# Visual-Behavior/aloception-oss

Hardware: AMD Instinct MI355X
Metric: frames/sec (whole node) DeformableDETR-R50 inference (higher is better)
Workload: dtype bf16; 1 GPU; DeformableDETR-R50 inference bf16, batch 8 synthetic 1333x800 frames per GPU, random-init weights; launch=hip-graph replay + eager inference(), per_gpu_batch=8, global_batch=8, parallelism=batch-sharded x1, no collective

## Files before the change

__graft_entry__.py:

```python
import os
import subprocess
import sys

ROOT = os.path.dirname(os.path.abspath(__file__))
PKG = os.path.join(ROOT, "aloception-oss_amd")
for p in (PKG, os.path.join(ROOT, "oracle")):
    if p not in sys.path:
        sys.path.insert(0, p)


def build():
    if os.path.exists("/opt/rocm/bin/hipcc"):
        subprocess.check_call(["make", "-C", os.path.join(PKG, "csrc"), "-j4"])
    subprocess.check_call(["make", "-C", os.path.join(ROOT, "oracle")])
    import alo_hip

    alo_hip.lib()
    alo_hip.two_stage_lib()
    from alonet.deformable_detr.ops.functions import load_MultiScaleDeformableAttention
    from alonet.raft.corr import CorrBlock

    load_MultiScaleDeformableAttention()


def smoke():
    import numpy as np
    import torch

    import alo_hip
    import oracle as O
    from alonet.deformable_detr.ops.functions import MSDeformAttnFunction
    from alonet.raft.corr import CorrBlock

    assert torch.cuda.is_available(), "smoke() needs a GPU"
    dev = "cuda:0"
    rng = np.random.default_rng(0)
    shapes = np.array([(12, 17), (6, 9), (3, 5), (2, 3)], np.int32)
    start = np.concatenate([[0], np.cumsum(shapes[:, 0] * shapes[:, 1])[:-1]]).astype(np.int32)
    N, M, D, Lq, L, P = 2, 8, 32, 40, 4, 4
    S = int((shapes[:, 0] * shapes[:, 1]).sum())
    value = rng.standard_normal((N, S, M, D)).astype(np.float32)
    loc = rng.uniform(-0.1, 1.1, (N, Lq, M, L, P, 2)).astype(np.float32)
    attn = rng.random((N, Lq, M, L, P)).astype(np.float32)
    attn /= attn.reshape(N, Lq, M, -1).sum(-1)[..., None, None]
    gout = rng.standard_normal((N, Lq, M * D)).astype(np.float32)

    tv = torch.from_numpy(value).to(dev).requires_grad_(True)
    tl = torch.from_numpy(loc).to(dev).requires_grad_(True)
    ta = torch.from_numpy(attn).to(dev).requires_grad_(True)
    out = MSDeformAttnFunction.apply(tv, torch.from_numpy(shapes).to(dev), torch.from_numpy(start).to(dev), tl, ta, 64)
    out.backward(torch.from_numpy(gout).to(dev))
    ref = O.msda_forward(value, shapes, start, loc, attn)
    rgv, rgl, rga = O.msda_backward(value, shapes, start, loc, attn, gout)
    err = {
        "msda_out": float(np.abs(out.detach().cpu().numpy() - ref).max()),
        "msda_grad_value": float(np.abs(tv.grad.cpu().numpy() - rgv).max()),
        "msda_grad_loc": float(np.abs(tl.grad.cpu().numpy() - rgl).max() / max(1.0, np.abs(rgl).max())),
        "msda_grad_attn": float(np.abs(ta.grad.cpu().numpy() - rga).max()),
    }
    refs = np.concatenate([np.stack([(np.tile(np.arange(w), h) + 0.5) / w, (np.repeat(np.arange(h), w) + 0.5) / h], -1) for h, w in shapes])
    eloc = (refs[None, :, None, None, None, :] + rng.uniform(-0.08, 0.08, (N, S, M, L, P, 2))).astype(np.float32)
    eattn = rng.random((N, S, M, L, P)).astype(np.float32)
    eattn /= eattn.reshape(N, S, M, -1).sum(-1)[..., None, None]
    egout = rng.standard_normal((N, S, M * D)).astype(np.float32)
    hint = (__import__("ctypes").c_int32 * 8)(*[int(v) for v in shapes.reshape(-1)])
    assert alo_hip.lib().alo_msda_backward_path(N, S, M, D, L, S, P, alo_hip.ALO_F32, alo_hip.ALO_F32, hint) == 2
    tsh = torch.from_numpy(shapes).to(dev)
    egv, egl, ega = alo_hip.msda_backward(torch.from_numpy(value).to(dev), tsh, torch.from_numpy(start).to(dev), torch.from_numpy(eloc).to(dev),
                                          torch.from_numpy(eattn).to(dev), torch.from_numpy(egout).to(dev))
    wgv, wgl, wga = O.msda_backward(value, shapes, start, eloc, eattn, egout)
    err["msda_wide_grad_value"] = float(np.abs(egv.cpu().numpy() - wgv).max())
    err["msda_wide_grad_loc"] = float(np.abs(egl.cpu().numpy() - wgl).max() / max(1.0, np.abs(wgl).max()))
    err["msda_wide_grad_attn"] = float(np.abs(ega.cpu().numpy() - wga).max())
    f1 = rng.standard_normal((1, 64, 16, 24)).astype(np.float32)
    f2 = rng.standard_normal((1, 64, 16, 24)).astype(np.float32)
    blk = CorrBlock(torch.from_numpy(f1).to(dev), torch.from_numpy(f2).to(dev))
    pyr = O.corr_pyramid(f1, f2)
    err["corr_pyramid"] = max(float(np.abs(blk.corr_pyramid[i].cpu().numpy() - pyr[i]).max()) for i in range(4))
    ys, xs = np.meshgrid(np.arange(16), np.arange(24), indexing="ij")
    coords = (np.stack([xs, ys])[None] + rng.standard_normal((1, 2, 16, 24)) * 2).astype(np.float32)
    got = blk(torch.from_numpy(coords).to(dev)).cpu().numpy()
    err["corr_lookup"] = float(np.abs(got - O.corr_lookup(pyr, coords)).max())
    print("smoke max-abs errors vs oracle:", err)
    assert all(v <= 1e-4 for v in err.values()), err
    assert "libalo_hotpath.so" in open("/proc/self/maps").read()


if __name__ == "__main__":
    build()
    if len(sys.argv) > 1 and sys.argv[1] == "smoke":
        smoke()
```

aloception-oss_amd/alo_hip/__init__.py:

```python
import ctypes
import warnings
import os
import subprocess

import torch

_PKG_ROOT = os.path.dirname(os.path.dirname(os.path.abspath(__file__)))
LIB_PATH = os.path.join(_PKG_ROOT, "libalo_hotpath.so")
CSRC_DIR = os.path.join(_PKG_ROOT, "csrc")

ALO_F32, ALO_F64, ALO_BF16 = 0, 1, 2
RESIDENT_AUTO, RESIDENT_ALWAYS = 0, 1
_DTYPE_CODE = {torch.float32: ALO_F32, torch.float64: ALO_F64, torch.bfloat16: ALO_BF16}

_lib = None
_warned_inference_tensor = False


def tensor_version(t):
    if t.is_inference():
        global _warned_inference_tensor
        if not _warned_inference_tensor:
            _warned_inference_tensor = True
            warnings.warn("alo_hip: a parameter / shape tensor created under torch.inference_mode() carries no version counter, so what is "
                          "derived from it (packed MFMA weights, folded convolutions, the host copy of spatial_shapes) is re-derived on "
                          "every call instead of being cached — results are right, the forward is slower.  Build / load the model outside "
                          "inference_mode() (torch.no_grad() is enough for inference).", RuntimeWarning, stacklevel=3)
        return object()
    return t._version


_DERIVED = "_alo_derived"
_EPOCH = "_alo_cache_epoch"


def derived(owner, name, sources, build, no_grad=True):
    entries = owner.__dict__.setdefault(_DERIVED, {}) if hasattr(owner, "__dict__") else {}
    key = tuple([None if t is None else (tensor_version(t), t.data_ptr(), t.dtype, t.device) for t in sources])
    hit = entries.get(name)
    if hit is None or hit[0] != key:
        with torch.set_grad_enabled(torch.is_grad_enabled() and not no_grad):
            hit = entries[name] = (key, build())
    return hit[1]


class HotpathUnavailable(RuntimeError):
    """libalo_hotpath.so cannot be loaded (not built, or built for another ABI)."""


def build(force=False):
    cmd = ["make", "-C", CSRC_DIR, "-j4"] + (["-B"] if force else [])
    subprocess.check_call(cmd, stdout=subprocess.DEVNULL)
    return LIB_PATH


def _declare(lib):
    c = ctypes
    vp, ip, sz = c.c_void_p, c.c_int, c.c_size_t
    lib.alo_abi_version.restype = ip
    lib.alo_abi_version.argtypes = []
    lib.alo_last_error.restype = c.c_char_p
    lib.alo_last_error.argtypes = []
    lib.alo_msda_forward.restype = ip
    lib.alo_msda_forward.argtypes = [vp] * 6 + [ip] * 9 + [vp]
    lib.alo_msda_forward_fused.restype = ip
    lib.alo_msda_forward_fused.argtypes = [vp] * 7 + [ip] * 9 + [vp]
    lib.alo_msda_backward.restype = ip
    lib.alo_msda_backward.argtypes = [vp] * 9 + [ip] * 9 + [vp]
    lib.alo_msda_backward_hinted.restype = ip
    lib.alo_msda_backward_hinted.argtypes = [vp] * 9 + [ip] * 9 + [c.POINTER(c.c_int32), vp]
    lib.alo_msda_backward_path.restype = ip
    lib.alo_msda_backward_path.argtypes = [ip] * 9 + [c.POINTER(c.c_int32)]
    lib.alo_corr_level_shape.restype = None
    lib.alo_corr_level_shape.argtypes = [ip, ip, ip, c.POINTER(ip), c.POINTER(ip)]
    lib.alo_corr_build_workspace_bytes.restype = sz
    lib.alo_corr_build_workspace_bytes.argtypes = [ip] * 5
    lib.alo_corr_build.restype = ip
    lib.alo_corr_build.argtypes = [vp, vp, c.POINTER(vp), vp, sz] + [ip] * 5 + [vp]
    lib.alo_corr_lookup.restype = ip
    lib.alo_corr_lookup.argtypes = [c.POINTER(vp), vp, vp] + [ip] * 5 + [vp]
    lib.alo_corr_lookup_backward.restype = ip
    lib.alo_corr_lookup_backward.argtypes = [c.POINTER(vp), vp, vp] + [ip] * 5 + [vp]
    lib.alo_corr_lookup_backward_coords.restype = ip
    lib.alo_corr_lookup_backward_coords.argtypes = [c.POINTER(vp), vp, vp, vp] + [ip] * 5 + [vp]
    lib.alo_corr_alt_workspace_bytes.restype = sz
    lib.alo_corr_alt_workspace_bytes.argtypes = [ip] * 5
    lib.alo_corr_alt_prepare.restype = ip
    lib.alo_corr_alt_prepare.argtypes = [vp, c.POINTER(vp), vp, sz] + [ip] * 5 + [vp]
    lib.alo_corr_alt_lookup.restype = ip
    lib.alo_corr_alt_lookup.argtypes = [vp, sz, vp, vp] + [ip] * 6 + [vp]
    lib.alo_msda_forward_fused_hm.restype = ip
    lib.alo_msda_forward_fused_hm_rows.restype = ip
    lib.alo_msda_forward_fused_hm_rows.argtypes = [vp] * 5 + [c.c_long, c.c_long, vp, vp] + [ip] * 9 + [vp]
    lib.alo_msda_forward_fused_hm.argtypes = [vp] * 7 + [ip] * 9 + [vp]
    lib.alo_msda_forward_fused_hm_resident.restype = ip
    lib.alo_msda_forward_fused_hm_resident.argtypes = [vp] * 5 + [c.c_long, c.c_long, vp, vp] + [ip] * 9 + [c.POINTER(c.c_int32), ip, vp]
    lib.alo_msda_resident_levels.restype = ip
    lib.alo_msda_resident_levels.argtypes = [c.POINTER(c.c_int32)] + [ip] * 6
    lib.alo_value_head_major.restype = ip
    lib.alo_value_head_major.argtypes = [vp] * 3 + [ip] * 5 + [vp]
    lib.alo_bias_act_nchw.restype = ip
    lib.alo_bias_act_nchw.argtypes = [vp] * 3 + [ip] * 4 + [vp]
    lib.alo_gru_gate.restype = ip
    lib.alo_gru_gate.argtypes = [vp] * 4 + [ip] * 3 + [c.c_long, c.c_long, vp]
    lib.alo_gru_update.restype = ip
    lib.alo_gru_update.argtypes = [vp] * 5 + [ip] * 3 + [c.c_long, vp]
    lib.alo_pack_mfma_b.restype = ip
    lib.alo_pack_mfma_b.argtypes = [vp, vp, ip, ip, ip, vp]
    lib.alo_value_proj_head_major.restype = ip
    lib.alo_value_proj_head_major.argtypes = [vp] * 5 + [ip] * 5 + [vp]
    lib.alo_conv3x3_nhwc.restype = ip
    lib.alo_conv3x3_nhwc.argtypes = [vp] * 5 + [ip] * 8 + [vp]
    lib.alo_conv3x3_workspace_bytes.restype = c.c_size_t
    lib.alo_conv3x3_workspace_bytes.argtypes = [ip] * 6
    lib.alo_stem_conv_pool.restype = ip
    lib.alo_stem_conv_pool.argtypes = [vp] * 4 + [ip] * 3 + [c.c_long] * 4 + [ip, vp]
    lib.alo_groupnorm_rows_workspace_bytes.restype = c.c_size_t
    lib.alo_groupnorm_rows_workspace_bytes.argtypes = [ip, ip, ip]
    lib.alo_groupnorm_rows.restype = ip
    lib.alo_groupnorm_rows.argtypes = [vp] * 5 + [ip] * 4 + [c.c_float, c.c_long, ip, vp]
    lib.alo_groupnorm_rows_act.restype = ip
    lib.alo_groupnorm_rows_act.argtypes = [vp] * 5 + [ip] * 4 + [c.c_float, c.c_long, ip, ip, vp]
    lib.alo_conv3x3_small_nhwc.restype = ip
    lib.alo_conv3x3_small_nhwc.argtypes = [vp] * 4 + [ip] * 6 + [vp]
    lib.alo_upsample_add_nhwc.restype = ip
    lib.alo_upsample_add_nhwc.argtypes = [vp] * 3 + [ip] * 8 + [vp]
    lib.alo_linear_packed.restype = ip
    lib.alo_linear_packed.argtypes = [vp] * 5 + [c.c_long, ip, ip, ip, ip, vp]
    lib.alo_mask_pyramid.restype = ip
    lib.alo_mask_pyramid.argtypes = [vp, ip, vp, vp, ip, ip, ip, ip, c.POINTER(c.c_int), c.c_uint, vp]
    lib.alo_encoder_reference_points.restype = ip
    lib.alo_encoder_reference_points.argtypes = [vp, vp, ip, ip, c.POINTER(c.c_int), vp]
    lib.alo_conv1x1_nhwc.restype = ip
    lib.alo_conv1x1_nhwc.argtypes = [vp, vp, ip, vp, vp, vp] + [ip] * 8 + [vp]
    lib.alo_panoptic_onehot.restype = ip
    lib.alo_panoptic_onehot.argtypes = [vp, vp] + [ip] * 6 + [c.c_float, vp]
    lib.alo_ffn256.restype = ip
    lib.alo_ffn256.argtypes = [vp] * 6 + [c.c_long, ip, ip, vp]
    lib.alo_linear_shortk.restype = ip
    lib.alo_linear_shortk.argtypes = [vp] * 5 + [c.c_long, ip, ip, ip, ip, vp]
    lib.alo_pos_sine_flat.restype = ip
    lib.alo_pos_sine_flat.argtypes = [vp] * 7 + [ip] * 6 + [c.c_float, c.c_float, ip, vp]
    lib.alo_add_layernorm.restype = ip
    lib.alo_add_layernorm.argtypes = [vp] * 7 + [c.c_long, ip, c.c_float, ip, vp]
    lib.alo_bias_act.restype = ip
    lib.alo_bias_act.argtypes = [vp] * 4 + [c.c_long, ip, ip, ip, vp]


def lib():
    global _lib
    if _lib is None:
        if not os.path.exists(LIB_PATH):
            raise HotpathUnavailable(
                f"{LIB_PATH} is missing: build it with `python -c 'import __graft_entry__ as g; g.build()'` "
                f"or `make -C {CSRC_DIR}` (hipcc, --offload-arch=gfx950). There is no CPU fallback for this path."
            )
        try:
            handle = ctypes.CDLL(LIB_PATH)
        except OSError as e:
            raise HotpathUnavailable(f"cannot load {LIB_PATH}: {e}") from e
        _declare(handle)
        if handle.alo_abi_version() != 2:
            raise HotpathUnavailable(f"{LIB_PATH} has ABI version {handle.alo_abi_version()}, expected 2")
        _lib = handle
    return _lib


def is_available():
    try:
        lib()
        return True
    except HotpathUnavailable:
        return False


def _check(rc):
    if rc != 0:
        raise RuntimeError(lib().alo_last_error().decode() or f"alo_hotpath error {rc}")


def _stream(device):
    return ctypes.c_void_p(torch.cuda.current_stream(device).cuda_stream)


def _ptr(t):
    return ctypes.c_void_p(t.data_ptr())


def _require_cuda_contiguous(named):
    for name, t in named:
        if not t.is_contiguous():
            raise RuntimeError(f"{name} tensor has to be contiguous")
    for name, t in named:
        if not t.is_cuda:
            raise RuntimeError(f"{name} must be a CUDA tensor")


class LaunchTimer:

    def __init__(self, only=None):
        self.records = []
        self.relaunch = {}
        self.only = only

    def __enter__(self):
        global _timer
        self._prev, _timer = _timer, self
        return self

    def __exit__(self, *exc):
        global _timer
        _timer = self._prev

    def replay_ms(self, tag, reps=20):
        fn = self.relaunch[tag]
        fn()
        torch.cuda.synchronize()
        start, stop = torch.cuda.Event(enable_timing=True), torch.cuda.Event(enable_timing=True)
        start.record()
        for _ in range(reps):
            fn()
        stop.record()
        torch.cuda.synchronize()
        return start.elapsed_time(stop) / reps

    def replay_samples(self, tag, reps=7):
        fn = self.relaunch[tag]
        fn()
        torch.cuda.synchronize()
        events = [torch.cuda.Event(enable_timing=True) for _ in range(reps + 1)]
        events[0].record()
        for i in range(reps):
            fn()
            events[i + 1].record()
        torch.cuda.synchronize()
        return [events[i].elapsed_time(events[i + 1]) for i in range(reps)]

    def summary(self):
        torch.cuda.synchronize()
        out = {}
        for tag, start, stop, nbytes, flops in self.records:
            d = out.setdefault(tag, dict(calls=0, ms_total=0.0, alg_bytes_avg=0.0, alg_flops_avg=0.0))
            d["calls"] += 1
            d["ms_total"] += start.elapsed_time(stop)
            d["alg_bytes_avg"] += nbytes
            d["alg_flops_avg"] += flops
        for d in out.values():
            d["ms_avg"] = d["ms_total"] / d["calls"]
            d["alg_bytes_avg"] /= d["calls"]
            d["alg_flops_avg"] /= d["calls"]
        return out


_timer = None


class _timed:
    def __init__(self, tag, nbytes=0.0, flops=0.0, relaunch=None):
        self.tag, self.nbytes, self.flops, self.relaunch = tag, nbytes, flops, relaunch

    def __enter__(self):
        self.on = _timer is not None and (_timer.only is None or self.tag.startswith(_timer.only))
        if self.on:
            self.start = torch.cuda.Event(enable_timing=True)
            self.stop = torch.cuda.Event(enable_timing=True)
            self.start.record()
        return self

    def __exit__(self, *exc):
        if self.on:
            self.stop.record()
            _timer.records.append((self.tag, self.start, self.stop, self.nbytes, self.flops))
            if self.relaunch is not None:
                _timer.relaunch[self.tag] = self.relaunch


def msda_forward_bytes(N, S, M, D, L, Lq, P, elem, loc_elem=4):
    return elem * (N * S * M * D + N * Lq * M * D) + loc_elem * (N * Lq * M * L * P * 3)


def msda_backward_bytes(N, S, M, D, L, Lq, P, elem, loc_elem=4):
    return elem * (2 * N * S * M * D + N * Lq * M * D) + loc_elem * (N * Lq * M * L * P * 3 * 2)


def _msda_prepare(value, spatial_shapes, level_start_index, sampling_loc, attn_weight, im2col_step, extra=()):
    if not value.is_cuda:
        raise RuntimeError("Not implemented on the CPU")
    _require_cuda_contiguous(
        [("value", value), ("spatial_shapes", spatial_shapes), ("level_start_index", level_start_index),
         ("sampling_loc", sampling_loc), ("attn_weight", attn_weight)] + list(extra)
    )
    if value.dim() != 4 or sampling_loc.dim() != 6 or attn_weight.dim() != 5:
        raise RuntimeError("value must be (N,S,M,D), sampling_loc (N,Lq,M,L,P,2), attn_weight (N,Lq,M,L,P)")
    if spatial_shapes.dtype != torch.int32 or level_start_index.dtype != torch.int32:
        raise RuntimeError("spatial_shapes and level_start_index must be int32 tensors")
    N, S, M, D = value.shape
    _, Lq, M2, L, P, two = sampling_loc.shape
    if (M2, two) != (M, 2) or tuple(attn_weight.shape) != (N, Lq, M, L, P) or sampling_loc.shape[0] != N:
        raise RuntimeError("sampling_loc / attn_weight shapes do not match value")
    if tuple(spatial_shapes.shape) != (L, 2) or tuple(level_start_index.shape) != (L,):
        raise RuntimeError("spatial_shapes must be (L,2) and level_start_index (L,)")
    step = min(N, int(im2col_step))
    if step <= 0 or N % step != 0:
        raise RuntimeError(f"batch({N}) must divide im2col_step({step})")
    vdt = _DTYPE_CODE.get(value.dtype)
    if vdt is None:
        raise RuntimeError(f"ms_deform_attn: unsupported value dtype {value.dtype}")
    if value.dtype == torch.bfloat16:
        sampling_loc, attn_weight = sampling_loc.float(), attn_weight.float()
    elif sampling_loc.dtype != value.dtype or attn_weight.dtype != value.dtype:
        raise RuntimeError("sampling_loc and attn_weight must have the dtype of value")
    ldt = _DTYPE_CODE[sampling_loc.dtype]
    return (N, S, M, D, L, Lq, P), vdt, ldt, sampling_loc.contiguous(), attn_weight.contiguous()


def msda_forward(value, spatial_shapes, level_start_index, sampling_loc, attn_weight, im2col_step=64):
    dims, vdt, ldt, loc, attn = _msda_prepare(value, spatial_shapes, level_start_index, sampling_loc, attn_weight, im2col_step)
    N, S, M, D, L, Lq, P = dims
    out = torch.empty((N, Lq, M * D), dtype=value.dtype, device=value.device)
    nbytes = msda_forward_bytes(N, S, M, D, L, Lq, P, value.element_size(), loc.element_size())
    with torch.cuda.device(value.device), _timed(f"msda_fwd/Lq={Lq}", nbytes):
        _check(lib().alo_msda_forward(_ptr(value), _ptr(spatial_shapes), _ptr(level_start_index), _ptr(loc), _ptr(attn),
                                      _ptr(out), N, S, M, D, L, Lq, P, vdt, ldt, _stream(value.device)))
    return out


def _check_fused_operands(value, spatial_shapes, level_start_index, sampling_offsets, attn_logits, reference_points, dims):
    N, Lq, M, L, P = dims
    if sampling_offsets.dtype != value.dtype or attn_logits.dtype != value.dtype:
        raise RuntimeError("sampling_offsets and attn_logits must have the dtype of value")
    if spatial_shapes.dtype != torch.int32 or level_start_index.dtype != torch.int32:
        raise RuntimeError("spatial_shapes and level_start_index must be int32 tensors")
    ref_dim = reference_points.shape[-1]
    if tuple(reference_points.shape) != (N, Lq, L, ref_dim) or attn_logits.numel() != N * Lq * M * L * P:
        raise RuntimeError("reference_points must be (N,Lq,L,2|4) and attn_logits (N,Lq,M,L*P)")
    return ref_dim


def msda_forward_fused(value, spatial_shapes, level_start_index, sampling_offsets, attn_logits, reference_points):
    if not value.is_cuda:
        raise RuntimeError("Not implemented on the CPU")
    N, S, M, D = value.shape
    _, Lq, _, L, P, _ = sampling_offsets.shape
    geo = torch.float64 if value.dtype == torch.float64 else torch.float32
    reference_points = reference_points.to(geo).contiguous()
    _require_cuda_contiguous([("value", value), ("spatial_shapes", spatial_shapes), ("level_start_index", level_start_index),
                              ("sampling_offsets", sampling_offsets), ("attn_logits", attn_logits),
                              ("reference_points", reference_points)])
    ref_dim = _check_fused_operands(value, spatial_shapes, level_start_index, sampling_offsets, attn_logits, reference_points,
                                    (N, Lq, M, L, P))
    vdt = _DTYPE_CODE.get(value.dtype)
    if vdt is None:
        raise RuntimeError(f"ms_deform_attn: unsupported value dtype {value.dtype}")
    out = torch.empty((N, Lq, M * D), dtype=value.dtype, device=value.device)
    e = value.element_size()
    nbytes = e * (N * S * M * D + N * Lq * M * D + N * Lq * M * L * P * 3) + reference_points.element_size() * reference_points.numel()
    with torch.cuda.device(value.device), _timed(f"msda_fwd_fused/Lq={Lq}", nbytes):
        _check(lib().alo_msda_forward_fused(_ptr(value), _ptr(spatial_shapes), _ptr(level_start_index),
                                            _ptr(sampling_offsets), _ptr(attn_logits), _ptr(reference_points), _ptr(out),
                                            N, S, M, D, L, Lq, P, ref_dim, vdt, _stream(value.device)))
    return out


def head_major_supported(value, L, P):
    return (value.is_cuda and value.dtype == torch.bfloat16 and L == 4 and P == 4 and value.shape[-1] % 8 == 0
            and value.shape[-1] <= 32)


def value_head_major(value, padding_mask=None):
    _require_cuda_contiguous([("value", value)])
    N, S, M, D = value.shape
    if padding_mask is not None:
        if padding_mask.dtype != torch.bool or tuple(padding_mask.shape) != (N, S) or not padding_mask.is_cuda:
            raise RuntimeError("padding_mask must be a (N, S) bool CUDA tensor")
        padding_mask = padding_mask.contiguous()
    out = torch.empty((N, M, S, D), dtype=value.dtype, device=value.device)
    with torch.cuda.device(value.device), _timed(f"value_head_major/S={S}", 2 * value.element_size() * value.numel()):
        _check(lib().alo_value_head_major(_ptr(value), None if padding_mask is None else _ptr(padding_mask), _ptr(out),
                                          N, S, M, D, _DTYPE_CODE[value.dtype], _stream(value.device)))
    return out


def _query_rows(t, inner):
    if t.dim() < 3 or t.shape[0] == 0 or t.shape[1] == 0:
        return None
    expect = 1
    for size, stride in zip(reversed(t.shape[2:]), reversed(t.stride()[2:])):
        if size != 1 and stride != expect:
            return None
        expect *= size
    if expect != inner:
        return None
    rs = t.stride(1) if t.shape[1] > 1 else inner
    if rs < inner or (t.shape[0] > 1 and t.stride(0) != rs * t.shape[1]):
        return None
    return rs


def msda_forward_fused_hm(value_hm, spatial_shapes, level_start_index, sampling_offsets, attn_logits, reference_points,
                          resident=True):
    if not value_hm.is_cuda:
        raise RuntimeError("Not implemented on the CPU")
    N, M, S, D = value_hm.shape
    _, Lq, _, L, P, _ = sampling_offsets.shape
    reference_points = reference_points.float().contiguous()
    _require_cuda_contiguous([("value", value_hm), ("spatial_shapes", spatial_shapes), ("level_start_index", level_start_index)])
    ref_dim = _check_fused_operands(value_hm, spatial_shapes, level_start_index, sampling_offsets, attn_logits, reference_points,
                                    (N, Lq, M, L, P))
    off_rs, log_rs = _query_rows(sampling_offsets, M * L * P * 2), _query_rows(attn_logits, M * L * P)
    if off_rs is None or log_rs is None or off_rs % 8 or log_rs % 8 or not sampling_offsets.is_cuda or not attn_logits.is_cuda:
        sampling_offsets, attn_logits = sampling_offsets.contiguous(), attn_logits.contiguous()
        off_rs, log_rs = M * L * P * 2, M * L * P
    out = torch.empty((N, Lq, M * D), dtype=value_hm.dtype, device=value_hm.device)
    e = value_hm.element_size()
    nbytes = e * (N * S * M * D + N * Lq * M * D + N * Lq * M * L * P * 3) + 4 * reference_points.numel()
    host = _host_spatial_shapes(spatial_shapes, read=False) if resident else None
    starts = None
    if host is not None and D == 32 and len(host) == L and sum(int(h) * int(w) for h, w in host) == S:
        starts = (ctypes.c_int32 * (2 * L))(*[int(v) for hw in host for v in hw])

    policy = RESIDENT_ALWAYS if resident == "always" else RESIDENT_AUTO

    def launch():
        if starts is not None:
            _check(lib().alo_msda_forward_fused_hm_resident(_ptr(value_hm), _ptr(spatial_shapes), _ptr(level_start_index),
                                                            _ptr(sampling_offsets), _ptr(attn_logits), off_rs, log_rs,
                                                            _ptr(reference_points), _ptr(out), N, S, M, D, L, Lq, P, ref_dim,
                                                            _DTYPE_CODE[value_hm.dtype], starts, policy, _stream(value_hm.device)))
            return
        _check(lib().alo_msda_forward_fused_hm_rows(_ptr(value_hm), _ptr(spatial_shapes), _ptr(level_start_index),
                                                    _ptr(sampling_offsets), _ptr(attn_logits), off_rs, log_rs,
                                                    _ptr(reference_points), _ptr(out), N, S, M, D, L, Lq, P, ref_dim,
                                                    _DTYPE_CODE[value_hm.dtype], _stream(value_hm.device)))

    tag = "msda_fwd_fused_resident" if starts is not None and lib().alo_msda_resident_levels(starts, N, S, M, L, Lq, policy) else "msda_fwd_fused"
    with torch.cuda.device(value_hm.device), _timed(f"{tag}/Lq={Lq}", nbytes, relaunch=launch if _timer else None):
        launch()
    return out


def _host_spatial_shapes(spatial_shapes, read=True):
    host = getattr(spatial_shapes, "_alo_shapes", None)
    if host is not None:
        return host
    hit = getattr(spatial_shapes, "_alo_shapes_read", None)
    if hit is not None and hit[0] == tensor_version(spatial_shapes):
        return hit[1]
    if not read:
        return None
    host = [tuple(int(v) for v in hw) for hw in spatial_shapes.tolist()]
    spatial_shapes._alo_shapes_read = (tensor_version(spatial_shapes), host)
    return host


def _wide_backward_wants_host_shapes(value, dims, ldt):
    N, S, M, D, L, Lq, P = dims
    return value.dtype in (torch.float32, torch.bfloat16) and ldt == ALO_F32 and D in (32, 64) and L == 4 and P == 4 and Lq == S


_tiled_backward_eligible = _wide_backward_wants_host_shapes


def msda_backward(value, spatial_shapes, level_start_index, sampling_loc, attn_weight, grad_output, im2col_step=64):
    dims, vdt, ldt, loc, attn = _msda_prepare(value, spatial_shapes, level_start_index, sampling_loc, attn_weight,
                                              im2col_step, extra=[("grad_output", grad_output)])
    N, S, M, D, L, Lq, P = dims
    if grad_output.dtype != value.dtype or grad_output.numel() != N * Lq * M * D:
        raise RuntimeError("grad_output must be (N, Lq, M*D) with the dtype of value")
    gdt = torch.float64 if value.dtype == torch.float64 else torch.float32
    grad_value = torch.empty(value.shape, dtype=gdt, device=value.device)
    grad_loc = torch.empty(loc.shape, dtype=gdt, device=value.device)
    grad_attn = torch.empty(attn.shape, dtype=gdt, device=value.device)
    nbytes = msda_backward_bytes(N, S, M, D, L, Lq, P, value.element_size(), loc.element_size())
    host = _host_spatial_shapes(spatial_shapes) if _wide_backward_wants_host_shapes(value, dims, ldt) else None
    hint = None if host is None else (ctypes.c_int32 * (2 * L))(*[int(v) for hw in host for v in hw])

    def launch():
        _check(lib().alo_msda_backward_hinted(_ptr(value), _ptr(spatial_shapes), _ptr(level_start_index), _ptr(loc), _ptr(attn),
                                              _ptr(grad_output), _ptr(grad_value), _ptr(grad_loc), _ptr(grad_attn),
                                              N, S, M, D, L, Lq, P, vdt, ldt, hint, _stream(value.device)))

    with torch.cuda.device(value.device), _timed(f"msda_bwd/Lq={Lq}", nbytes, relaunch=launch if _timer else None):
        launch()
    return [grad_value.to(value.dtype), grad_loc.to(sampling_loc.dtype), grad_attn.to(attn_weight.dtype)]


def corr_level_shapes(H, W, num_levels):
    out = []
    h, w = ctypes.c_int(), ctypes.c_int()
    for lvl in range(num_levels):
        lib().alo_corr_level_shape(H, W, lvl, ctypes.byref(h), ctypes.byref(w))
        out.append((h.value, w.value))
    return out


def _require_f32_cuda(name, t, ndim):
    if not t.is_cuda:
        raise RuntimeError(f"{name} must be a CUDA tensor (the correlation path has no CPU implementation here)")
    if t.dtype != torch.float32 or t.dim() != ndim:
        raise RuntimeError(f"{name} must be a {ndim}-d float32 tensor, got {tuple(t.shape)} {t.dtype}")


def corr_build(fmap1, fmap2, num_levels=4):
    _require_f32_cuda("fmap1", fmap1, 4)
    _require_f32_cuda("fmap2", fmap2, 4)
    if fmap1.shape != fmap2.shape:
        raise RuntimeError("fmap1 and fmap2 must have the same shape")
    fmap1, fmap2 = fmap1.contiguous(), fmap2.contiguous()
    B, C, H, W = fmap1.shape
    shapes = corr_level_shapes(H, W, num_levels)
    levels = [torch.empty((B * H * W, 1, h, w), dtype=torch.float32, device=fmap1.device) for h, w in shapes]
    nbytes = lib().alo_corr_build_workspace_bytes(B, C, H, W, num_levels)
    ws = torch.empty((max(nbytes, 4) // 4,), dtype=torch.float32, device=fmap1.device)
    ptrs = (ctypes.c_void_p * num_levels)(*[t.data_ptr() for t in levels])
    ncols = sum(h * w for h, w in shapes)
    def launch():
        _check(lib().alo_corr_build(_ptr(fmap1), _ptr(fmap2), ptrs, _ptr(ws), nbytes, B, C, H, W, num_levels,
                                    _stream(fmap1.device)))

    with torch.cuda.device(fmap1.device), _timed("corr_build", 4.0 * (2 * B * C * H * W + B * H * W * ncols),
                                                 2.0 * B * (H * W) * (H * W) * C, relaunch=launch if _timer else None):
        launch()
    return levels


def _corr_lookup_args(levels, levels_name, coords, radius, grad_out=None, fn=None):
    _require_f32_cuda("coords", coords, 4)
    coords = coords.contiguous()
    B, two, H, W = coords.shape
    L = len(levels)
    if grad_out is None:
        if two != 2:
            raise RuntimeError("coords must be (B,2,H,W)")
    else:
        _require_f32_cuda("grad_out", grad_out, 4)
        grad_out = grad_out.contiguous()
        if two != 2 or tuple(grad_out.shape) != (B, L * (2 * radius + 1) ** 2, H, W):
            raise RuntimeError(f"{fn}: coords must be (B,2,H,W) and grad_out (B, L*(2r+1)^2, H, W)")
    for lvl, t in enumerate(levels):
        _require_f32_cuda(f"{levels_name}[{lvl}]", t, 4)
        if not t.is_contiguous() or t.shape[0] != B * H * W:
            raise RuntimeError(f"{levels_name}[{lvl}] must be a contiguous (B*H*W,1,h,w) tensor")
    return coords, grad_out, (ctypes.c_void_p * L)(*[t.data_ptr() for t in levels]), (B, H, W, L)


def corr_lookup(levels, coords, radius=4):
    coords, _, ptrs, (B, H, W, L) = _corr_lookup_args(levels, "corr_pyramid", coords, radius)
    out = torch.empty((B, L * (2 * radius + 1) ** 2, H, W), dtype=torch.float32, device=coords.device)
    taps = (2 * radius + 2) ** 2
    nbytes = 4.0 * B * H * W * (L * (2 * radius + 1) ** 2 + L * taps + 2)
    with torch.cuda.device(coords.device), _timed("corr_lookup", nbytes):
        _check(lib().alo_corr_lookup(ptrs, _ptr(coords), _ptr(out), B, H, W, radius, L, _stream(coords.device)))
    return out


def corr_lookup_backward(grad_levels, coords, grad_out, radius=4):
    coords, grad_out, ptrs, (B, H, W, L) = _corr_lookup_args(grad_levels, "grad_levels", coords, radius, grad_out,
                                                             "corr_lookup_backward")
    taps = (2 * radius + 2) ** 2
    nbytes = 4.0 * B * H * W * (L * (2 * radius + 1) ** 2 + 2 * L * taps + 2)
    with torch.cuda.device(coords.device), _timed("corr_lookup_backward", nbytes):
        _check(lib().alo_corr_lookup_backward(ptrs, _ptr(coords), _ptr(grad_out), B, H, W, radius, L, _stream(coords.device)))
    return grad_levels


def corr_lookup_backward_coords(levels, coords, grad_out, radius=4):
    coords, grad_out, ptrs, (B, H, W, L) = _corr_lookup_args(levels, "corr_pyramid", coords, radius, grad_out,
                                                             "corr_lookup_backward_coords")
    per_level = torch.empty((B, L, 2, H, W), dtype=torch.float32, device=coords.device)
    taps = (2 * radius + 2) ** 2
    nbytes = 4.0 * B * H * W * (L * (2 * radius + 1) ** 2 + L * taps + 2 + 2 * L)
    with torch.cuda.device(coords.device), _timed("corr_lookup_backward_coords", nbytes):
        _check(lib().alo_corr_lookup_backward_coords(ptrs, _ptr(coords), _ptr(grad_out), _ptr(per_level), B, H, W, radius, L,
                                                     _stream(coords.device)))
    return per_level.sum(1)


def corr_alt_prepare(fmap1, fmap2_levels):
    _require_f32_cuda("fmap1", fmap1, 4)
    for lvl, t in enumerate(fmap2_levels):
        _require_f32_cuda(f"fmap2_levels[{lvl}]", t, 4)
    B, C, H, W = fmap1.shape
    L = len(fmap2_levels)
    for lvl, ((h, w), t) in enumerate(zip(corr_level_shapes(H, W, L), fmap2_levels)):
        if tuple(t.shape) != (B, C, h, w) or t.device != fmap1.device:
            raise RuntimeError(f"fmap2_levels[{lvl}] must be ({B}, {C}, {h}, {w}) on {fmap1.device}, got {tuple(t.shape)} on {t.device}")
    fmap1 = fmap1.contiguous()
    levels = [t.contiguous() for t in fmap2_levels]
    nbytes = lib().alo_corr_alt_workspace_bytes(B, C, H, W, L)
    ws = torch.empty((max(nbytes, 16),), dtype=torch.uint8, device=fmap1.device)
    ptrs = (ctypes.c_void_p * L)(*[t.data_ptr() for t in levels])
    moved = 4.0 * 2 * (fmap1.numel() + sum(t.numel() for t in levels))
    with torch.cuda.device(fmap1.device), _timed("corr_alt_prepare", moved):
        _check(lib().alo_corr_alt_prepare(_ptr(fmap1), ptrs, _ptr(ws), nbytes, B, C, H, W, L, _stream(fmap1.device)))
    return ws


def corr_alt_lookup(workspace, coords, channels, num_levels, radius=4):
    _require_f32_cuda("coords", coords, 4)
    if not workspace.is_cuda or workspace.dtype != torch.uint8 or workspace.device != coords.device:
        raise RuntimeError("workspace must be the uint8 CUDA tensor corr_alt_prepare returned, on the device of coords")
    coords = coords.contiguous()
    B, two, H, W = coords.shape
    if two != 2:
        raise RuntimeError("coords must be (B,2,H,W)")
    L, C, win = num_levels, channels, (2 * radius + 1) ** 2
    out = torch.empty((B, L * win, H, W), dtype=torch.float32, device=coords.device)
    flops = 2.0 * B * H * W * L * (2 * radius + 2) ** 2 * C
    nbytes = 4.0 * B * H * W * (L * win + 2 + L * C)
    with torch.cuda.device(coords.device), _timed("corr_alt_lookup", nbytes, flops):
        _check(lib().alo_corr_alt_lookup(_ptr(workspace), workspace.numel(), _ptr(coords), _ptr(out), B, C, H, W, radius, L,
                                         _stream(coords.device)))
    return out


def fusable(*tensors):
    if torch.is_grad_enabled() and any(t is not None and t.requires_grad for t in tensors):
        return False
    first = tensors[0]
    return first.is_cuda and first.dtype in (torch.float32, torch.bfloat16)


def add_layernorm_supported(x):
    C = x.shape[-1]
    return C % 4 == 0 and 0 < C <= 1024 and (C * x.element_size()) % 16 == 0 and x.data_ptr() % 16 == 0


def invalidate_caches(module):
    module.__dict__[_EPOCH] = cache_epoch(module) + 1
    for owner in (*module.modules(), *module.parameters(), *module.buffers()):
        owner.__dict__.pop(_DERIVED, None)


def cache_epoch(module):
    return module.__dict__.get(_EPOCH, 0)


def add_layernorm(x, residual, weight, bias, eps=1e-5, pos=None):
    C = x.shape[-1]
    rows = x.numel() // C
    x = x.contiguous()
    residual = None if residual is None else residual.contiguous()
    pos = None if pos is None else pos.contiguous()
    for name, t in (("residual", residual), ("pos", pos)):
        if t is not None and (t.shape != x.shape or t.dtype != x.dtype):
            raise RuntimeError(f"add_layernorm: {name} must have the shape and dtype of x")
    weight, bias = weight.to(x.dtype).contiguous(), bias.to(x.dtype).contiguous()
    out = torch.empty_like(x)
    out_pos = None if pos is None else torch.empty_like(x)
    nbytes = x.element_size() * x.numel() * (2 + (residual is not None) + 2 * (pos is not None))
    with torch.cuda.device(x.device), _timed(f"add_layernorm/rows={rows}", nbytes):
        _check(lib().alo_add_layernorm(_ptr(x), None if residual is None else _ptr(residual), _ptr(weight), _ptr(bias),
                                       _ptr(out), None if pos is None else _ptr(pos),
                                       None if pos is None else _ptr(out_pos), rows, C, float(eps),
                                       _DTYPE_CODE[x.dtype], _stream(x.device)))
    return out if pos is None else (out, out_pos)


def bias_act_(x, bias, residual=None, relu=True):
    if x.dim() == 4:
        if not x.is_contiguous(memory_format=torch.channels_last):
            raise RuntimeError("bias_act_: 4-D input must be channels_last")
        C = x.shape[1]
        if residual is not None and not (residual.shape == x.shape and residual.is_contiguous(memory_format=torch.channels_last)):
            raise RuntimeError("bias_act_: residual must be channels_last with the shape of x")
    else:
        if not x.is_contiguous():
            raise RuntimeError("bias_act_: matrix input must be contiguous")
        C = x.shape[-1]
        if residual is not None and not (residual.shape == x.shape and residual.is_contiguous()):
            raise RuntimeError("bias_act_: residual must be contiguous with the shape of x")
    if residual is not None and residual.dtype != x.dtype:
        raise RuntimeError("bias_act_: residual must have the dtype of x")
    bias = bias.to(x.dtype).contiguous()
    nbytes = x.element_size() * x.numel() * (2 + (residual is not None))
    with torch.cuda.device(x.device), _timed(f"bias_act/C={C}", nbytes):
        _check(lib().alo_bias_act(_ptr(x), _ptr(bias), None if residual is None else _ptr(residual), _ptr(x),
                                  x.numel() // C, C, 1 if relu else 0, _DTYPE_CODE[x.dtype], _stream(x.device)))
    return x


def _require_f32_nchw(name, t):
    if not (t.is_cuda and t.dtype == torch.float32 and t.dim() == 4 and t.is_contiguous()):
        raise RuntimeError(f"{name} must be a contiguous float32 CUDA tensor (B, C, H, W)")


def bias_act_nchw_(x, bias, relu=True):
    _require_f32_nchw("x", x)
    B, C, H, W = x.shape
    with torch.cuda.device(x.device), _timed(f"bias_act_nchw/C={C}", 8.0 * x.numel()):
        _check(lib().alo_bias_act_nchw(_ptr(x), _ptr(bias.float().contiguous()), _ptr(x), B, C, H * W, 1 if relu else 0,
                                       _stream(x.device)))
    return x


def gru_gate_(zr, bias_zr, hx, rhx, C):
    _require_f32_nchw("zr", zr); _require_f32_nchw("hx", hx); _require_f32_nchw("rhx", rhx)
    B, C2, H, W = zr.shape
    if C2 != 2 * C or hx.shape != rhx.shape or hx.shape[0] != B or hx.shape[2:] != zr.shape[2:] or hx.shape[1] < C:
        raise RuntimeError("gru_gate_: zr must be (B,2C,H,W) and hx / rhx (B,C+Cx,H,W)")
    with torch.cuda.device(zr.device), _timed(f"gru_gate/C={C}", 4.0 * B * C * H * W * 5):
        _check(lib().alo_gru_gate(_ptr(zr), _ptr(bias_zr), _ptr(hx), _ptr(rhx), B, C, H * W, hx.stride(0), rhx.stride(0),
                                  _stream(zr.device)))


def gru_update_(q, bias_q, zr, hx, C, net=None):
    _require_f32_nchw("q", q); _require_f32_nchw("zr", zr); _require_f32_nchw("hx", hx)
    B, Cq, H, W = q.shape
    if Cq != C or zr.shape != (B, 2 * C, H, W) or hx.shape[0] != B or hx.shape[2:] != q.shape[2:]:
        raise RuntimeError("gru_update_: q must be (B,C,H,W), zr (B,2C,H,W), hx (B,C+Cx,H,W)")
    if net is not None:
        _require_f32_nchw("net", net)
    with torch.cuda.device(q.device), _timed(f"gru_update/C={C}", 4.0 * B * C * H * W * (4 + (net is not None))):
        _check(lib().alo_gru_update(_ptr(q), _ptr(bias_q), _ptr(zr), _ptr(hx), None if net is None else _ptr(net), B, C,
                                    H * W, hx.stride(0), _stream(q.device)))


def pos_sine_flat(mask_flatten, spatial_shapes, level_start_index, dim_t, level_embed, normalize, center, scale, dtype,
                  eps=1e-6):
    B, S = mask_flatten.shape
    L, F = spatial_shapes.shape[0], dim_t.numel()
    if mask_flatten.dtype != torch.bool or dim_t.dtype != torch.float32:
        raise RuntimeError("pos_sine_flat: mask must be bool and dim_t float32")
    mask_flatten, dim_t = mask_flatten.contiguous(), dim_t.contiguous()
    if level_embed is not None:
        level_embed = level_embed.to(dtype).contiguous()
        if tuple(level_embed.shape) != (L, 2 * F):
            raise RuntimeError("pos_sine_flat: level_embed must be (L, 2 * num_pos_feats)")
    out = torch.empty((B, S, 2 * F), dtype=dtype, device=mask_flatten.device)
    work = torch.empty((B, S, 2), dtype=torch.float32, device=mask_flatten.device)
    with torch.cuda.device(out.device), _timed(f"pos_sine_flat/S={S}", out.element_size() * out.numel()):
        _check(lib().alo_pos_sine_flat(_ptr(mask_flatten), _ptr(spatial_shapes), _ptr(level_start_index), _ptr(dim_t),
                                       None if level_embed is None else _ptr(level_embed), _ptr(out), _ptr(work), B, S, L, F,
                                       1 if normalize else 0, 1 if center else 0, float(scale), float(eps),
                                       _DTYPE_CODE[dtype], _stream(out.device)))
    return out


def linear_shortk_supported(x, weight):
    return (x.is_cuda and x.dtype == torch.bfloat16 and weight.dtype == torch.bfloat16 and x.shape[-1] in (64, 128, 256)
            and weight.dim() == 2 and weight.shape[1] == x.shape[-1] and weight.shape[0] % 64 == 0)


def linear_shortk(x, weight, bias=None, relu=False, residual=None):
    if not linear_shortk_supported(x, weight):
        raise RuntimeError("linear_shortk: needs bf16 CUDA tensors, K in (64, 128, 256) and N % 64 == 0")
    N, K = weight.shape
    x2 = x.reshape(-1, K)
    if not x2.is_contiguous():
        x2 = x2.contiguous()
    y = torch.empty((x2.shape[0], N), dtype=x.dtype, device=x.device)
    M = x2.shape[0]
    if residual is not None:
        residual = residual.reshape(-1, N)
        if residual.shape[0] != M or residual.dtype != x.dtype or not residual.is_contiguous():
            raise RuntimeError("linear_shortk: residual must be a contiguous (M, N) tensor of x's dtype")
    if M:
        nbytes = 2.0 * (x2.numel() + y.numel() * (2 if residual is not None else 1))
        with torch.cuda.device(x.device), _timed(f"linear_shortk/N={N},K={K}", nbytes, 2.0 * M * N * K):
            _check(lib().alo_linear_shortk(_ptr(x2), _ptr(weight.contiguous()), None if bias is None else _ptr(bias.contiguous()),
                                           None if residual is None else _ptr(residual), _ptr(y), M, N, K, 1 if relu else 0,
                                           ALO_BF16, _stream(x.device)))
    return y.view(*x.shape[:-1], N)


def linear_packed_supported(x, weight):
    return (x.is_cuda and x.dtype == torch.bfloat16 and weight.dtype == torch.bfloat16 and weight.dim() == 2
            and x.shape[-1] == weight.shape[1] and weight.shape[1] % 256 == 0 and weight.shape[1] >= 512
            and weight.shape[0] % 128 == 0 and not torch.is_grad_enabled())


def linear_packed(x, weight, bias=None, relu=False, residual=None):
    if not linear_packed_supported(x, weight):
        raise RuntimeError("linear_packed: needs bf16 CUDA tensors, K % 256 == 0, K >= 512, N % 128 == 0, no autograd")
    x2 = x.reshape(-1, x.shape[-1])
    if not x2.is_contiguous():
        x2 = x2.contiguous()
    M, K = x2.shape
    N = weight.shape[0]
    y = torch.empty((M, N), dtype=x.dtype, device=x.device)
    if residual is not None:
        residual = residual.reshape(M, N)
        if residual.dtype != x.dtype or not residual.is_contiguous():
            raise RuntimeError("linear_packed: residual must be a contiguous (M, N) tensor of the input's dtype")
    if M:
        packed = pack_mfma_b(weight)
        bias_c = None if bias is None else bias.to(x.dtype).contiguous()
        with torch.cuda.device(x.device), _timed(f"linear_packed/K={K}/N={N}", 2.0 * (M * K + M * N * (2 if residual is not None else 1)),
                                                 2.0 * M * N * K):
            _check(lib().alo_linear_packed(_ptr(x2), _ptr(packed), None if bias_c is None else _ptr(bias_c),
                                           None if residual is None else _ptr(residual), _ptr(y), M, N, K, 1 if relu else 0,
                                           ALO_BF16, _stream(x.device)))
    return y.view(*x.shape[:-1], N)


def conv1x1_strided_supported(x, weight2d):
    if not (x.dim() == 4 and x.is_cuda and x.is_contiguous(memory_format=torch.channels_last)):
        return False
    if os.environ.get("ALO_CONV1X1_GATHER") == "0":
        return False
    rows = x.permute(0, 2, 3, 1)
    if linear_shortk_supported(rows, weight2d):
        return True
    return linear_packed_supported(rows, weight2d) and (weight2d.shape[0] >= 1024 or tuple(weight2d.shape) == (128, 512))


def conv1x1_strided(x, weight2d, bias, stride, relu=False):
    if not conv1x1_strided_supported(x, weight2d):
        raise RuntimeError("conv1x1_strided: unsupported dtype / layout / shape")
    n, cin, h, w_ = x.shape
    cout = weight2d.shape[0]
    ho, wo = (h - 1) // stride + 1, (w_ - 1) // stride + 1
    y = torch.empty((n, cout, ho, wo), dtype=x.dtype, device=x.device, memory_format=torch.channels_last)
    packed = not linear_shortk_supported(x.permute(0, 2, 3, 1), weight2d)
    wt = pack_mfma_b(weight2d) if packed else weight2d.contiguous()
    bias_c = None if bias is None else bias.to(x.dtype).contiguous()
    with torch.cuda.device(x.device), _timed(f"conv1x1_strided/K={cin}/N={cout}", 2.0 * (y.numel() // cout * cin + y.numel()),
                                             2.0 * y.numel() * cin):
        _check(lib().alo_conv1x1_nhwc(_ptr(x), _ptr(wt), 1 if packed else 0, None if bias_c is None else _ptr(bias_c), None, _ptr(y),
                                      n, h, w_, cin, cout, stride, 1 if relu else 0, ALO_BF16, _stream(x.device)))
    return y


def linear_auto(x, weight, bias=None, relu=False, residual=None):
    if linear_shortk_supported(x, weight) and (bias is None or bias.dtype == x.dtype):
        return linear_shortk(x, weight, bias, relu, residual=residual)
    if linear_packed_supported(x, weight) and (bias is None or bias.dtype == x.dtype) and (
            residual is not None or weight.shape[0] >= 1024 or tuple(weight.shape) == (128, 512)):
        return linear_packed(x, weight, bias, relu, residual=residual)
    x2 = x.reshape(-1, x.shape[-1])
    fused_act = relu and residual is None
    if bias is not None:
        y = torch._addmm_activation(bias, x2, weight.t(), use_gelu=False) if fused_act else torch.addmm(bias, x2, weight.t())
    else:
        y = torch.mm(x2, weight.t())
        y = torch.relu_(y) if fused_act else y
    if residual is not None:
        y = y + residual.reshape(y.shape)
        y = torch.relu_(y) if relu else y
    return y.view(*x.shape[:-1], weight.shape[0])


def ffn256_supported(x, w1, w2):
    return (x.is_cuda and x.dtype == torch.bfloat16 and x.shape[-1] == 256 and w1.dtype == torch.bfloat16
            and w2.dtype == torch.bfloat16 and w1.dim() == 2 and w1.shape[1] == 256 and w1.shape[0] % 256 == 0
            and tuple(w2.shape) == (256, w1.shape[0]))


def pack_mfma_b(weight):
    return derived(weight, "mfma_b", (weight,), lambda: _pack_mfma_b(weight.contiguous()))


def _pack_mfma_b(w):
    packed = torch.empty_like(w)
    with torch.cuda.device(w.device):
        _check(lib().alo_pack_mfma_b(_ptr(w), _ptr(packed), w.shape[0], w.shape[1], ALO_BF16, _stream(w.device)))
    return packed


def ffn256(x, w1, b1, w2, b2):
    if not ffn256_supported(x, w1, w2):
        raise RuntimeError("ffn256: needs bf16 CUDA tensors, d_model = 256 and a hidden width that is a multiple of 256")
    x2 = x.reshape(-1, 256)
    if not x2.is_contiguous():
        x2 = x2.contiguous()
    y = torch.empty_like(x2)
    M, Fh = x2.shape[0], w1.shape[0]
    if M:
        p1, p2 = pack_mfma_b(w1), pack_mfma_b(w2)
        with torch.cuda.device(x.device), _timed(f"ffn256/F={Fh}", 4.0 * x2.numel(), 4.0 * M * 256 * Fh):
            _check(lib().alo_ffn256(_ptr(x2), _ptr(p1), None if b1 is None else _ptr(b1.contiguous()),
                                    _ptr(p2), None if b2 is None else _ptr(b2.contiguous()), _ptr(y), M, Fh,
                                    ALO_BF16, _stream(x.device)))
    return y.view(x.shape)


def conv3x3_supported(x, weight, stride=(1, 1), padding=(1, 1), dilation=(1, 1), groups=1):
    return (x.is_cuda and x.dtype == torch.bfloat16 and weight.dtype == torch.bfloat16 and x.dim() == 4 and weight.dim() == 4
            and tuple(weight.shape[2:]) == (3, 3) and tuple(stride) in ((1, 1), (2, 2)) and tuple(padding) == (1, 1)
            and tuple(dilation) == (1, 1) and groups == 1 and weight.shape[1] == x.shape[1] and x.shape[1] % 64 == 0
            and weight.shape[0] % 64 == 0 and x.is_contiguous(memory_format=torch.channels_last)
            and not torch.is_grad_enabled())


def conv3x3(x, weight, bias=None, relu=False, stride=1):
    stride = stride[0] if isinstance(stride, (tuple, list)) else stride
    if not conv3x3_supported(x, weight, (stride, stride)):
        raise RuntimeError("conv3x3: needs a channels-last bf16 CUDA activation, a (Cout, Cin, 3, 3) weight, Cin % 64 == 0, "
                           "Cout % 64 == 0, stride 1 or 2, no autograd")
    n, cin, h, w_ = x.shape
    cout = weight.shape[0]
    packed = derived(weight, "conv3x3_b", (weight,),
                     lambda: _pack_mfma_b(weight.permute(0, 2, 3, 1).reshape(cout, 9 * cin).contiguous()))
    ho, wo = (h - 1) // stride + 1, (w_ - 1) // stride + 1
    y = torch.empty((n, cout, ho, wo), dtype=x.dtype, device=x.device, memory_format=torch.channels_last)
    bias_c = None if bias is None else bias.contiguous()
    ws_bytes = lib().alo_conv3x3_workspace_bytes(n, h, w_, cin, cout, stride)
    ws = torch.empty(ws_bytes // 4, dtype=torch.float32, device=x.device) if ws_bytes else None
    with torch.cuda.device(x.device), _timed(f"conv3x3/C={cin}/s={stride}", 2.0 * (x.numel() + y.numel()), 2.0 * 9 * cin * y.numel()):
        _check(lib().alo_conv3x3_nhwc(_ptr(x), _ptr(packed), None if bias_c is None else _ptr(bias_c), _ptr(y),
                                      None if ws is None else _ptr(ws), n, h, w_, cin, cout, stride, 1 if relu else 0, ALO_BF16,
                                      _stream(x.device)))
    return y


def stem_conv_pool_supported(x, weight):
    return (x.is_cuda and x.dtype == torch.bfloat16 and weight.dtype == torch.bfloat16 and x.dim() == 4 and x.shape[1] == 3
            and tuple(weight.shape) == (64, 3, 7, 7) and not torch.is_grad_enabled())


def stem_conv_pool(x, weight, bias=None):
    if not stem_conv_pool_supported(x, weight):
        raise RuntimeError("stem_conv_pool: needs a bf16 CUDA (N, 3, H, W) image, a (64, 3, 7, 7) bf16 weight, no autograd")
    n, _, h, w_ = x.shape

    def pack():
        wm = torch.zeros((64, 8, 24), dtype=weight.dtype, device=weight.device)
        wm[:, :7, :21] = weight.permute(0, 2, 3, 1).reshape(64, 7, 21)
        return _pack_mfma_b(wm.reshape(64, 192)[:, :176].contiguous())

    packed = derived(weight, "stem_b", (weight,), pack)
    hc, wc = (h - 1) // 2 + 1, (w_ - 1) // 2 + 1
    hp, wp = (hc - 1) // 2 + 1, (wc - 1) // 2 + 1
    y = torch.empty((n, 64, hp, wp), dtype=x.dtype, device=x.device, memory_format=torch.channels_last)
    bias_c = None if bias is None else bias.contiguous()
    sn, sc, sh, sw = x.stride()
    with torch.cuda.device(x.device), _timed("stem_conv_pool", 2.0 * (x.numel() + y.numel()), 2.0 * 147 * 64 * n * hc * wc):
        _check(lib().alo_stem_conv_pool(_ptr(x), _ptr(packed), None if bias_c is None else _ptr(bias_c), _ptr(y), n, h, w_,
                                        sn, sc, sh, sw, ALO_BF16, _stream(x.device)))
    return y


def groupnorm_rows_supported(x, weight, groups, narrow=False):
    c_ = x.shape[-1]
    cpg = c_ // groups if groups and c_ % groups == 0 else 0
    return (x.is_cuda and x.dtype == torch.bfloat16 and x.dim() == 3 and weight is not None and weight.dtype == torch.bfloat16
            and c_ % 8 == 0 and 256 % (c_ // 8) == 0 and cpg > 0 and (cpg % 8 == 0 or (narrow and cpg in (2, 4))) and 256 % groups == 0
            and not torch.is_grad_enabled())


def groupnorm_nhwc_supported(x, norm):
    return (x.dim() == 4 and x.is_cuda and x.is_contiguous(memory_format=torch.channels_last) and norm.affine
            and groupnorm_rows_supported(x.new_empty((1, 1, x.shape[1])), norm.weight, norm.num_groups, narrow=True))


def groupnorm_nhwc(x, norm, relu=False):
    if not groupnorm_nhwc_supported(x, norm):
        raise RuntimeError("groupnorm_nhwc: needs a channels-last bf16 CUDA map and 2, 4 or 8k channels per group, no autograd")
    n, c_, h, w_ = x.shape
    rows = x.permute(0, 2, 3, 1)
    out = torch.empty_like(x)
    if n and h * w_:
        nbytes = lib().alo_groupnorm_rows_workspace_bytes(n, h * w_, norm.num_groups)
        ws = torch.empty(max(nbytes, 4) // 4, dtype=torch.float32, device=x.device)
        with torch.cuda.device(x.device), _timed(f"groupnorm_nhwc/C={c_}", 6.0 * x.numel()):
            _check(lib().alo_groupnorm_rows_act(_ptr(rows), _ptr(norm.weight.contiguous()), _ptr(norm.bias.contiguous()), _ptr(out),
                                                _ptr(ws), n, h * w_, c_, norm.num_groups, float(norm.eps), h * w_ * c_,
                                                1 if relu else 0, ALO_BF16, _stream(x.device)))
    return out


def conv3x3_small_supported(x, conv):
    w = conv.weight
    return (isinstance(conv, torch.nn.Conv2d) and x.dim() == 4 and x.is_cuda and x.dtype == torch.bfloat16 and w.dtype == torch.bfloat16
            and conv.kernel_size == (3, 3) and conv.stride == (1, 1) and conv.padding == (1, 1) and conv.dilation == (1, 1)
            and conv.groups == 1 and conv.padding_mode == "zeros" and w.shape[1] == x.shape[1] and x.shape[1] in (16, 32, 64)
            and (w.shape[0] == 1 or (w.shape[0] % 4 == 0 and w.shape[0] <= 32))
            and x.is_contiguous(memory_format=torch.channels_last) and not torch.is_grad_enabled())


def _small_conv_operands(conv):
    w, b = conv.weight, conv.bias

    def build():
        cout, cin = w.shape[:2]
        full = torch.zeros((32, 3, 3, cin), dtype=w.dtype, device=w.device)
        full[:cout] = w.permute(0, 2, 3, 1)
        frag = full.view(32, 9, cin // 16, 2, 8).permute(1, 2, 3, 0, 4).contiguous()
        bias32 = torch.zeros(32, dtype=torch.float32, device=w.device)
        if b is not None:
            bias32[:cout] = b.float()
        return frag, bias32

    return derived(conv, "small_frag", (w, b), build)


def conv3x3_small(x, conv):
    if not conv3x3_small_supported(x, conv):
        raise RuntimeError("conv3x3_small: needs a channels-last bf16 CUDA map, a 3x3 / stride 1 / padding 1 convolution with Cin in "
                           "(16, 32, 64) and Cout = 1 or 4k <= 32, no autograd")
    n, cin, h, w_ = x.shape
    cout = conv.weight.shape[0]
    frag, bias32 = _small_conv_operands(conv)
    y = torch.empty((n, cout, h, w_), dtype=x.dtype, device=x.device, memory_format=torch.channels_last)
    if y.numel():
        with torch.cuda.device(x.device), _timed(f"conv3x3_small/C={cin}->{cout}", 2.0 * (x.numel() + y.numel()), 2.0 * 9 * cin * cout * n * h * w_):
            _check(lib().alo_conv3x3_small_nhwc(_ptr(x), _ptr(frag), _ptr(bias32), _ptr(y), n, h, w_, cin, cout, ALO_BF16, _stream(x.device)))
    return y


def upsample_add_supported(x_low, fpn):
    return (x_low.dim() == 4 and fpn.dim() == 4 and x_low.is_cuda and x_low.dtype == torch.bfloat16 and fpn.dtype == torch.bfloat16
            and x_low.shape[1] == fpn.shape[1] and x_low.shape[1] % 8 == 0 and fpn.shape[0] > 0 and x_low.shape[0] % fpn.shape[0] == 0
            and x_low.is_contiguous(memory_format=torch.channels_last) and fpn.is_contiguous(memory_format=torch.channels_last)
            and not torch.is_grad_enabled())


def upsample_add(x_low, fpn):
    if not upsample_add_supported(x_low, fpn):
        raise RuntimeError("upsample_add: needs channels-last bf16 CUDA maps with C % 8 == 0 and x_low.shape[0] a multiple of fpn.shape[0]")
    bq, c_, h, w_ = x_low.shape
    b_, _, H, W = fpn.shape
    out = torch.empty((bq, c_, H, W), dtype=x_low.dtype, device=x_low.device, memory_format=torch.channels_last)
    if out.numel():
        with torch.cuda.device(x_low.device), _timed(f"upsample_add/C={c_}", 2.0 * (out.numel() + x_low.numel() + fpn.numel())):
            _check(lib().alo_upsample_add_nhwc(_ptr(x_low), _ptr(fpn), _ptr(out), bq, bq // b_, c_, h, w_, H, W, ALO_BF16, _stream(x_low.device)))
    return out


def groupnorm_rows(x, weight, bias, groups, eps=1e-5, out=None):
    if not groupnorm_rows_supported(x, weight, groups):
        raise RuntimeError("groupnorm_rows: needs bf16 CUDA rows (B, HW, C) with C / 8 and groups dividing 256, no autograd")
    x = x.contiguous()
    b_, hw, c_ = x.shape
    if out is None:
        out = torch.empty_like(x)
    if tuple(out.shape) != (b_, hw, c_) or out.dtype != x.dtype or out.stride(2) != 1 or out.stride(1) != c_:
        raise RuntimeError("groupnorm_rows: out must be (B, HW, C) of the input's dtype with contiguous rows")
    if b_ and hw:
        nbytes = lib().alo_groupnorm_rows_workspace_bytes(b_, hw, groups)
        ws = torch.empty(nbytes // 4, dtype=torch.float32, device=x.device)
        with torch.cuda.device(x.device), _timed(f"groupnorm_rows/HW={hw}", 6.0 * x.numel()):
            _check(lib().alo_groupnorm_rows(_ptr(x), _ptr(weight.contiguous()), _ptr(bias.contiguous()), _ptr(out), _ptr(ws), b_, hw,
                                            c_, groups, float(eps), out.stride(0) if b_ > 1 else hw * c_, ALO_BF16,
                                            _stream(x.device)))
    return out


def _host_shapes(shapes):
    flat = [int(v) for hw in shapes for v in hw]
    return (ctypes.c_int * len(flat))(*flat), len(flat) // 2


def mask_pyramid(frame_mask, shapes, nearest_levels=()):
    if frame_mask.dim() == 4:
        frame_mask = frame_mask[:, 0]
    if not frame_mask.is_cuda or frame_mask.dim() != 3:
        raise RuntimeError("mask_pyramid: needs a CUDA (B, H, W) or (B, 1, H, W) mask")
    if frame_mask.dtype not in (torch.float32, torch.bool, torch.uint8):
        frame_mask = frame_mask != 0
    frame_mask = frame_mask.contiguous()
    b_, h, w_ = frame_mask.shape
    arr, L = _host_shapes(shapes)
    S = sum(int(a) * int(b) for a, b in shapes)
    mask_flat = torch.empty((b_, S), dtype=torch.uint8, device=frame_mask.device)
    ratios = torch.empty((b_, L, 2), dtype=torch.float32, device=frame_mask.device)
    bits = 0
    for l in nearest_levels:
        bits |= 1 << int(l)
    with torch.cuda.device(frame_mask.device), _timed("mask_pyramid", float(frame_mask.numel() + mask_flat.numel())):
        _check(lib().alo_mask_pyramid(_ptr(frame_mask), 1 if frame_mask.dtype == torch.float32 else 0, _ptr(mask_flat), _ptr(ratios),
                                      b_, h, w_, L, arr, bits, _stream(frame_mask.device)))
    return mask_flat.view(torch.bool), ratios


def encoder_reference_points(valid_ratios, shapes):
    if not valid_ratios.is_cuda or valid_ratios.dtype != torch.float32 or valid_ratios.dim() != 3 or valid_ratios.shape[2] != 2:
        raise RuntimeError("encoder_reference_points: needs CUDA float32 valid ratios of shape (B, L, 2)")
    valid_ratios = valid_ratios.contiguous()
    arr, L = _host_shapes(shapes)
    if L != valid_ratios.shape[1]:
        raise RuntimeError("encoder_reference_points: one (h, w) per level of valid_ratios")
    S = sum(int(a) * int(b) for a, b in shapes)
    out = torch.empty((valid_ratios.shape[0], S, L, 2), dtype=torch.float32, device=valid_ratios.device)
    with torch.cuda.device(valid_ratios.device), _timed("encoder_reference_points", 4.0 * out.numel()):
        _check(lib().alo_encoder_reference_points(_ptr(valid_ratios), _ptr(out), valid_ratios.shape[0], L, arr,
                                                  _stream(valid_ratios.device)))
    return out


def value_proj_head_major_supported(x, weight, heads):
    return (linear_shortk_supported(x, weight) and heads % 2 == 0 and weight.shape[0] == heads * 32 and x.dim() == 3)


def value_proj_head_major(x, weight, bias, padding_mask, heads):
    if not value_proj_head_major_supported(x, weight, heads):
        raise RuntimeError("value_proj_head_major: needs bf16 (N, S, K) input, K in (64, 128, 256), head dimension 32")
    N, S, K = x.shape
    x = x if x.is_contiguous() else x.contiguous()
    if padding_mask is not None:
        if padding_mask.dtype != torch.bool or tuple(padding_mask.shape) != (N, S):
            raise RuntimeError("padding_mask must be a (N, S) bool tensor")
        padding_mask = padding_mask.contiguous()
    out = torch.empty((N, heads, S, 32), dtype=x.dtype, device=x.device)
    with torch.cuda.device(x.device), _timed(f"value_proj_hm/S={S}", 2.0 * (x.numel() + out.numel()), 2.0 * N * S * heads * 32 * K):
        _check(lib().alo_value_proj_head_major(_ptr(x), _ptr(weight.contiguous()), None if bias is None else _ptr(bias.contiguous()),
                                               None if padding_mask is None else _ptr(padding_mask), _ptr(out), N, S, heads, K,
                                               ALO_BF16, _stream(x.device)))
    return out



def panoptic_onehot(mask_logits, frame_size, threshold=0.5):
    if not mask_logits.is_cuda or mask_logits.dim() != 4:
        raise RuntimeError("panoptic_onehot: needs CUDA (B, Q, h, w) logits")
    x = mask_logits.float().contiguous()
    b_, q, h, w_ = x.shape
    H, W = int(frame_size[0]), int(frame_size[1])
    out = torch.empty((b_, q, H, W), dtype=torch.long, device=x.device)
    if out.numel():
        with torch.cuda.device(x.device), _timed("panoptic_onehot", 8.0 * out.numel()):
            _check(lib().alo_panoptic_onehot(_ptr(x), _ptr(out), b_, q, h, w_, H, W, float(threshold), _stream(x.device)))
    return out


TWO_STAGE_LIB_PATH = os.path.join(_PKG_ROOT, "libalo_two_stage.so")
_two_stage_lib = None


def two_stage_lib():
    global _two_stage_lib
    if _two_stage_lib is None:
        lib()
        if not os.path.exists(TWO_STAGE_LIB_PATH):
            raise HotpathUnavailable(f"{TWO_STAGE_LIB_PATH} is missing: build it with `make -C {CSRC_DIR}` (hipcc, --offload-arch=gfx950)")
        try:
            handle = ctypes.CDLL(TWO_STAGE_LIB_PATH)
        except OSError as e:
            raise HotpathUnavailable(f"cannot load {TWO_STAGE_LIB_PATH}: {e}") from e
        c = ctypes
        vp, ip = c.c_void_p, c.c_int
        handle.alo_two_stage_abi_version.restype = ip
        handle.alo_two_stage_abi_version.argtypes = []
        handle.alo_encoder_proposals.restype = ip
        handle.alo_encoder_proposals.argtypes = [vp, vp, vp, ip, ip, c.POINTER(c.c_int), vp]
        handle.alo_encoder_proposals_masked.restype = ip
        handle.alo_encoder_proposals_masked.argtypes = [vp, vp, vp, vp, vp, ip, ip, c.POINTER(c.c_int), ip, ip, vp]
        handle.alo_mask_rows.restype = ip
        handle.alo_mask_rows.argtypes = [vp, vp, vp, c.c_long, ip, ip, vp]
        handle.alo_proposal_queries.restype = ip
        handle.alo_proposal_queries.argtypes = [vp, vp, vp, vp, vp, ip, ip, ip, ip, vp]
        if handle.alo_two_stage_abi_version() != 1:
            raise HotpathUnavailable(f"{TWO_STAGE_LIB_PATH} has ABI version {handle.alo_two_stage_abi_version()}, expected 1")
        _two_stage_lib = handle
    return _two_stage_lib


def encoder_proposals_supported(mask_flatten, shapes):
    return (mask_flatten.is_cuda and mask_flatten.dim() == 2 and mask_flatten.dtype in (torch.bool, torch.uint8)
            and mask_flatten.is_contiguous() and 0 < len(shapes) <= 8 and mask_flatten.shape[0] > 0 and mask_flatten.numel() < 2 ** 31
            and all(int(h) > 0 and int(w) > 0 for h, w in shapes)
            and sum(int(h) * int(w) for h, w in shapes) == mask_flatten.shape[1])


def encoder_proposals(mask_flatten, shapes):
    if not encoder_proposals_supported(mask_flatten, shapes):
        raise RuntimeError("encoder_proposals: needs a contiguous CUDA (B, S) bool / uint8 mask and 1..8 non-empty levels whose sizes sum to S")
    B, S = mask_flatten.shape
    arr, L = _host_shapes(shapes)
    proposals = torch.empty((B, S, 4), dtype=torch.float32, device=mask_flatten.device)
    keep = torch.empty((B, S), dtype=torch.uint8, device=mask_flatten.device)
    with torch.cuda.device(mask_flatten.device), _timed(f"encoder_proposals/S={S}", 18.0 * B * S):
        _check(two_stage_lib().alo_encoder_proposals(_ptr(mask_flatten), _ptr(proposals), _ptr(keep), B, L, arr,
                                                     _stream(mask_flatten.device)))
    return proposals, keep.view(torch.bool)


def encoder_proposals_masked_supported(mask_flatten, shapes, memory):
    return (encoder_proposals_supported(mask_flatten, shapes) and memory.dim() == 3 and memory.device == mask_flatten.device
            and tuple(memory.shape[:2]) == tuple(mask_flatten.shape) and mask_rows_supported(memory, mask_flatten))


def encoder_proposals_masked(mask_flatten, shapes, memory):
    if not encoder_proposals_masked_supported(mask_flatten, shapes, memory):
        raise RuntimeError("encoder_proposals_masked: needs what encoder_proposals and mask_rows need, memory (B, S, C) on the mask's device")
    B, S = mask_flatten.shape
    arr, L = _host_shapes(shapes)
    proposals = torch.empty((B, S, 4), dtype=torch.float32, device=mask_flatten.device)
    keep = torch.empty((B, S), dtype=torch.uint8, device=mask_flatten.device)
    out = torch.empty_like(memory)
    with torch.cuda.device(memory.device), _timed(f"encoder_proposals_masked/S={S}", 2.0 * memory.element_size() * memory.numel() + 18.0 * B * S):
        _check(two_stage_lib().alo_encoder_proposals_masked(_ptr(mask_flatten), _ptr(proposals), _ptr(keep), _ptr(memory), _ptr(out), B, L,
                                                            arr, memory.shape[-1], _DTYPE_CODE[memory.dtype], _stream(memory.device)))
    return proposals, keep.view(torch.bool), out


def mask_rows_supported(memory, keep):
    return (memory.is_cuda and memory.dtype in (torch.float32, torch.bfloat16) and memory.is_contiguous() and memory.dim() >= 2
            and memory.shape[-1] % 8 == 0 and memory.numel() > 0 and memory.data_ptr() % 16 == 0
            and keep.is_cuda and keep.dtype in (torch.bool, torch.uint8) and keep.is_contiguous()
            and tuple(keep.shape) == tuple(memory.shape[:-1]))


def mask_rows(memory, keep):
    if not mask_rows_supported(memory, keep):
        raise RuntimeError("mask_rows: needs contiguous CUDA fp32 / bf16 rows with C % 8 == 0 and one bool / uint8 `keep` per row")
    C = memory.shape[-1]
    rows = memory.numel() // C
    out = torch.empty_like(memory)
    with torch.cuda.device(memory.device), _timed(f"mask_rows/rows={rows}", 2.0 * memory.element_size() * memory.numel() + rows):
        _check(two_stage_lib().alo_mask_rows(_ptr(memory), _ptr(keep), _ptr(out), rows, C, _DTYPE_CODE[memory.dtype],
                                             _stream(memory.device)))
    return out


def proposal_queries_supported(coords_unact, topk, dtype):
    return (coords_unact.is_cuda and coords_unact.dtype == torch.float32 and coords_unact.dim() == 3 and coords_unact.shape[2] == 4
            and coords_unact.is_contiguous() and coords_unact.numel() > 0 and coords_unact.data_ptr() % 16 == 0
            and topk.is_cuda and topk.dtype == torch.int64 and topk.dim() == 2 and topk.shape[0] == coords_unact.shape[0]
            and topk.is_contiguous() and topk.numel() > 0 and dtype in (torch.float32, torch.bfloat16))


def proposal_dim_t(device, owner=None):
    def build():
        return 10000 ** (torch.arange(64, dtype=torch.float32, device=device) / 64)
    if owner is None or owner.device != torch.device(device):
        return build()
    return derived(owner, "proposal_dim_t", (owner,), build)


def proposal_queries(coords_unact, topk, dtype, owner=None):
    if not proposal_queries_supported(coords_unact, topk, dtype):
        raise RuntimeError("proposal_queries: needs contiguous CUDA (B, S, 4) float32 coordinates, (B, K) int64 indices, fp32 / bf16 output")
    B, S, _ = coords_unact.shape
    K = topk.shape[1]
    ref = torch.empty((B, K, 4), dtype=torch.float32, device=coords_unact.device)
    embed = torch.empty((B, K, 512), dtype=dtype, device=coords_unact.device)
    dim_t = proposal_dim_t(coords_unact.device, owner)
    with torch.cuda.device(coords_unact.device), _timed(f"proposal_queries/K={K}", B * K * (8.0 + 32.0 + 512.0 * embed.element_size())):
        _check(two_stage_lib().alo_proposal_queries(_ptr(coords_unact), _ptr(topk), _ptr(dim_t), _ptr(ref), _ptr(embed), B, S, K,
                                                    _DTYPE_CODE[dtype], _stream(coords_unact.device)))
    return ref, embed
```

aloception-oss_amd/alonet/deformable_detr/deformable_transformer.py:

```python
import copy
import math

import torch
import torch.nn.functional as F
from torch import nn
from torch.nn.init import constant_, normal_, xavier_uniform_

import alo_hip

from .ops.modules import MSDeformAttn
from .utils import inverse_sigmoid


_GEOMETRY = {}


def _level_geometry(shapes, device):
    key = (shapes, str(device))
    if key not in _GEOMETRY:
        sizes = [h * w for h, w in shapes]
        with torch.inference_mode(False):
            spatial_shapes = torch.tensor(shapes, dtype=torch.int32, device=device)
            level_start_index = torch.tensor([sum(sizes[:i]) for i in range(len(sizes))], dtype=torch.int32, device=device)
        spatial_shapes._alo_total = sum(sizes)
        spatial_shapes._alo_shapes = list(shapes)
        _GEOMETRY[key] = (spatial_shapes, level_start_index)
    return _GEOMETRY[key]


def _fused_ok(module, kwargs, *tensors):
    return (not module.training and "is_tracing" not in kwargs and alo_hip.fusable(*tensors)
            and alo_hip.add_layernorm_supported(tensors[0]))


def _add_norm(norm, x, residual, pos=None):
    return alo_hip.add_layernorm(x, residual, norm.weight, norm.bias, norm.eps, pos=pos)


def _self_attention(mha, qk_in, v_in):
    B, L, E = qk_in.shape
    H = mha.num_heads
    w, b = mha.in_proj_weight, mha.in_proj_bias
    qk = alo_hip.linear_auto(qk_in, w[: 2 * E], None if b is None else b[: 2 * E])
    v = alo_hip.linear_auto(v_in, w[2 * E:], None if b is None else b[2 * E:])
    q, k = qk[..., :E], qk[..., E:]
    heads = lambda t: t.reshape(B, L, H, E // H).transpose(1, 2)
    out = F.scaled_dot_product_attention(heads(q), heads(k), heads(v))
    out = out.transpose(1, 2).reshape(B, L, E)
    return alo_hip.linear_auto(out, mha.out_proj.weight, mha.out_proj.bias)


def _ffn(linear1, activation, linear2, x):
    if activation is F.relu and alo_hip.ffn256_supported(x, linear1.weight, linear2.weight):
        return alo_hip.ffn256(x, linear1.weight, linear1.bias, linear2.weight, linear2.bias)
    if activation is F.relu and linear1.bias is not None:
        h = alo_hip.linear_auto(x, linear1.weight, linear1.bias, relu=True)
        return alo_hip.linear_auto(h, linear2.weight, linear2.bias)
    return linear2(activation(linear1(x)))


PROPOSAL_EMBED_DIM = 512


def encoder_output_proposals(mask_flatten, shapes, dtype=torch.float32):
    device = mask_flatten.device
    B = mask_flatten.shape[0]
    per_level, start = [], 0
    for lvl, (h, w) in enumerate(shapes):
        free = ~mask_flatten[:, start:start + h * w].view(B, h, w)
        valid_h = free[:, :, 0].sum(1).to(dtype).view(B, 1, 1)
        valid_w = free[:, 0, :].sum(1).to(dtype).view(B, 1, 1)
        cy = ((torch.arange(h, dtype=dtype, device=device) + 0.5).view(1, h, 1) / valid_h).expand(B, h, w)
        cx = ((torch.arange(w, dtype=dtype, device=device) + 0.5).view(1, 1, w) / valid_w).expand(B, h, w)
        side = torch.full((B, h, w), 0.05 * 2.0 ** lvl, dtype=dtype, device=device)
        per_level.append(torch.stack((cx, cy, side, side), -1).view(B, h * w, 4))
        start += h * w
    p = torch.cat(per_level, 1)
    keep = ((p > 0.01) & (p < 0.99)).all(-1) & ~mask_flatten
    proposals = torch.log(p / (1 - p)).masked_fill(~keep.unsqueeze(-1), float("inf"))
    return proposals, keep


def proposal_pos_embed(coords_unact):
    dim_t = 10000 ** (torch.arange(64, dtype=torch.float32, device=coords_unact.device) / 64)
    angle = (coords_unact.sigmoid() * (2 * math.pi)).unsqueeze(-1) / dim_t
    return torch.stack((angle.sin(), angle.cos()), -1).flatten(-3)


def _get_clones(module, n):
    return nn.ModuleList([copy.deepcopy(module) for _ in range(n)])


def _get_activation_fn(activation):
    fns = {"relu": F.relu, "gelu": F.gelu, "glu": F.glu}
    if activation not in fns:
        raise RuntimeError(f"activation should be relu/gelu, not {activation}.")
    return fns[activation]


class DeformableTransformerEncoderLayer(nn.Module):
    def __init__(self, d_model=256, d_ffn=1024, dropout=0.1, activation="relu", n_levels=4, n_heads=8, n_points=4):
        super().__init__()
        self.self_attn = MSDeformAttn(d_model, n_levels, n_heads, n_points)
        self.dropout1 = nn.Dropout(dropout)
        self.norm1 = nn.LayerNorm(d_model)
        self.linear1 = nn.Linear(d_model, d_ffn)
        self.activation = _get_activation_fn(activation)
        self.dropout2 = nn.Dropout(dropout)
        self.linear2 = nn.Linear(d_ffn, d_model)
        self.dropout3 = nn.Dropout(dropout)
        self.norm2 = nn.LayerNorm(d_model)

    @staticmethod
    def with_pos_embed(tensor, pos):
        return tensor if pos is None else tensor + pos

    def forward_ffn(self, src):
        src2 = self.linear2(self.dropout2(self.activation(self.linear1(src))))
        return self.norm2(src + self.dropout3(src2))

    def forward(self, src, pos, reference_points, spatial_shapes, level_start_index, padding_mask=None, **kwargs):
        src2 = self.self_attn(self.with_pos_embed(src, pos), reference_points, src, spatial_shapes, level_start_index,
                              padding_mask, **kwargs)
        src = self.norm1(src + self.dropout1(src2))
        return self.forward_ffn(src)

    def forward_fused(self, src, query, pos, reference_points, spatial_shapes, level_start_index, padding_mask=None,
                      next_query=True, **kwargs):
        src2 = self.self_attn(query, reference_points, src, spatial_shapes, level_start_index, padding_mask, **kwargs)
        src = _add_norm(self.norm1, src2, src)
        src2 = _ffn(self.linear1, self.activation, self.linear2, src)
        if next_query and pos is not None:
            return _add_norm(self.norm2, src2, src, pos=pos)
        return _add_norm(self.norm2, src2, src), None


class DeformableTransformerEncoder(nn.Module):
    def __init__(self, encoder_layer, num_layers):
        super().__init__()
        self.layers = _get_clones(encoder_layer, num_layers)
        self.num_layers = num_layers

    @staticmethod
    def get_reference_points(spatial_shapes, valid_ratios, device, **kwargs):
        per_level = []
        host_shapes = getattr(spatial_shapes, "_alo_shapes", None)
        if (host_shapes is not None and valid_ratios.is_cuda and valid_ratios.dtype == torch.float32
                and not (torch.is_grad_enabled() and valid_ratios.requires_grad) and "is_tracing" not in kwargs):
            return alo_hip.encoder_reference_points(valid_ratios, host_shapes)
        for lvl in range(spatial_shapes.shape[0]):
            h, w = host_shapes[lvl] if host_shapes is not None else (int(spatial_shapes[lvl, 0]), int(spatial_shapes[lvl, 1]))
            ys = torch.arange(h, dtype=torch.float32, device=device) + 0.5
            xs = torch.arange(w, dtype=torch.float32, device=device) + 0.5
            ref_y, ref_x = torch.meshgrid(ys, xs, indexing="ij")
            ref_y = ref_y.reshape(1, -1) / (valid_ratios[:, None, lvl, 1] * h)
            ref_x = ref_x.reshape(1, -1) / (valid_ratios[:, None, lvl, 0] * w)
            per_level.append(torch.stack((ref_x, ref_y), -1))
        reference_points = torch.cat(per_level, 1)
        return reference_points[:, :, None] * valid_ratios[:, None]

    def forward(self, src, spatial_shapes, level_start_index, valid_ratios, pos=None, padding_mask=None, **kwargs):
        output = src
        reference_points = self.get_reference_points(spatial_shapes, valid_ratios, device=src.device, **kwargs)
        if _fused_ok(self, kwargs, output, pos) and all(hasattr(layer, "forward_fused") for layer in self.layers):
            query = output if pos is None else output + pos
            for i, layer in enumerate(self.layers):
                output, query = layer.forward_fused(output, query, pos, reference_points, spatial_shapes, level_start_index,
                                                    padding_mask, next_query=i + 1 < len(self.layers), **kwargs)
                if query is None:
                    query = output
            return output
        for layer in self.layers:
            output = layer(output, pos, reference_points, spatial_shapes, level_start_index, padding_mask, **kwargs)
        return output


class DeformableTransformerDecoderLayer(nn.Module):
    def __init__(self, d_model=256, dim_feedforward=1024, dropout=0.1, activation="relu", n_levels=4, n_heads=8,
                 n_points=4):
        super().__init__()
        self.cross_attn = MSDeformAttn(d_model, n_levels, n_heads, n_points)
        self.dropout1 = nn.Dropout(dropout)
        self.norm1 = nn.LayerNorm(d_model)
        self.self_attn = nn.MultiheadAttention(d_model, n_heads, dropout=dropout)
        self.dropout2 = nn.Dropout(dropout)
        self.norm2 = nn.LayerNorm(d_model)
        self.linear1 = nn.Linear(d_model, dim_feedforward)
        self.activation = _get_activation_fn(activation)
        self.dropout3 = nn.Dropout(dropout)
        self.linear2 = nn.Linear(dim_feedforward, d_model)
        self.dropout4 = nn.Dropout(dropout)
        self.norm3 = nn.LayerNorm(d_model)

    @staticmethod
    def with_pos_embed(tensor, pos):
        return tensor if pos is None else tensor + pos

    def forward_ffn(self, tgt):
        tgt2 = self.linear2(self.dropout3(self.activation(self.linear1(tgt))))
        return self.norm3(tgt + self.dropout4(tgt2))

    def pre_process_tgt(self, tgt, query_pos, tgt_key_padding_mask, **kwargs):
        return tgt, query_pos, tgt_key_padding_mask

    def decoder_layer_forward(self, tgt, query_pos, reference_points, src, src_spatial_shapes, level_start_index,
                              tgt_key_padding_mask=None, src_padding_mask=None, **kwargs):
        carried = tgt.__dict__.get("_alo_with_pos")
        if carried is not None and carried[0] is query_pos:
            q = k = carried[1]
        else:
            q = k = self.with_pos_embed(tgt, query_pos)
        if _fused_ok(self, kwargs, tgt, query_pos) and tgt_key_padding_mask is None and self.self_attn._qkv_same_embed_dim:
            tgt2 = _self_attention(self.self_attn, q, tgt)
        else:
            tgt2 = self.self_attn(q.transpose(0, 1), k.transpose(0, 1), tgt.transpose(0, 1),
                                  key_padding_mask=tgt_key_padding_mask)[0].transpose(0, 1)
        if _fused_ok(self, kwargs, tgt, tgt2, query_pos):
            if query_pos is None:
                tgt = query = _add_norm(self.norm2, tgt2, tgt)
            else:
                tgt, query = _add_norm(self.norm2, tgt2, tgt, pos=query_pos.expand_as(tgt))
            tgt2 = self.cross_attn(query, reference_points, src, src_spatial_shapes, level_start_index,
                                   src_padding_mask, **kwargs)
            tgt = _add_norm(self.norm1, tgt2, tgt)
            if query_pos is None or not query_pos.is_contiguous():
                return _add_norm(self.norm3, _ffn(self.linear1, self.activation, self.linear2, tgt), tgt)
            out, out_pos = _add_norm(self.norm3, _ffn(self.linear1, self.activation, self.linear2, tgt), tgt, pos=query_pos)
            out._alo_with_pos = (query_pos, out_pos)
            return out
        tgt = self.norm2(tgt + self.dropout2(tgt2))
        tgt2 = self.cross_attn(self.with_pos_embed(tgt, query_pos), reference_points, src, src_spatial_shapes,
                               level_start_index, src_padding_mask, **kwargs)
        tgt = self.norm1(tgt + self.dropout1(tgt2))
        return self.forward_ffn(tgt)

    def forward(self, tgt, query_pos, reference_points, src, src_spatial_shapes, level_start_index,
                tgt_key_padding_mask=None, src_padding_mask=None, **kwargs):
        tgt, query_pos, tgt_key_padding_mask = self.pre_process_tgt(tgt, query_pos, tgt_key_padding_mask, **kwargs)
        return self.decoder_layer_forward(tgt, query_pos, reference_points, src, src_spatial_shapes, level_start_index,
                                          tgt_key_padding_mask, src_padding_mask, **kwargs)


class DeformableTransformerDecoder(nn.Module):
    def __init__(self, decoder_layer, num_layers, return_intermediate=False):
        super().__init__()
        self.layers = _get_clones(decoder_layer, num_layers)
        self.num_layers = num_layers
        self.return_intermediate = return_intermediate
        self.bbox_embed = None
        self.class_embed = None

    def pre_process_tgt(self, tgt, query_pos, tgt_key_padding_mask, reference_points, **kwargs):
        return tgt, query_pos, tgt_key_padding_mask, reference_points

    def decoder_forward(self, tgt, reference_points, src, src_spatial_shapes, src_level_start_index, src_valid_ratios,
                        query_pos=None, src_padding_mask=None, tgt_key_padding_mask=None, **kwargs):
        output = tgt
        intermediate, intermediate_refs = [], []
        ref_input = None
        for lid, layer in enumerate(self.layers):
            if ref_input is None or self.bbox_embed is not None:
                if reference_points.shape[-1] == 4:
                    ratios = torch.cat([src_valid_ratios, src_valid_ratios], -1)
                    ref_input = reference_points[:, :, None] * ratios[:, None]
                else:
                    assert reference_points.shape[-1] == 2
                    ref_input = reference_points[:, :, None] * src_valid_ratios[:, None]
            output = layer(tgt=output, query_pos=query_pos, reference_points=ref_input, src=src,
                           src_spatial_shapes=src_spatial_shapes, level_start_index=src_level_start_index,
                           src_padding_mask=src_padding_mask, tgt_key_padding_mask=tgt_key_padding_mask, **kwargs)
            if self.bbox_embed is not None:
                tmp = self.bbox_embed[lid](output)
                if reference_points.shape[-1] == 4:
                    new_ref = (tmp + inverse_sigmoid(reference_points)).sigmoid()
                else:
                    tmp = torch.cat([tmp[..., :2] + inverse_sigmoid(reference_points), tmp[..., 2:]], -1)
                    new_ref = tmp.sigmoid()
                reference_points = new_ref.detach()
            if self.return_intermediate:
                intermediate.append(output)
                intermediate_refs.append(reference_points)
        if self.return_intermediate:
            return torch.stack(intermediate), torch.stack(intermediate_refs)
        return output, reference_points

    def forward(self, tgt, reference_points, src, src_spatial_shapes, src_level_start_index, src_valid_ratios,
                query_pos=None, src_padding_mask=None, tgt_key_padding_mask=None, decoder_outputs=None, **kwargs):
        decoder_outputs = {} if decoder_outputs is None else decoder_outputs
        tgt, query_pos, tgt_key_padding_mask, reference_points = self.pre_process_tgt(
            tgt, query_pos, tgt_key_padding_mask=tgt_key_padding_mask, reference_points=reference_points, **kwargs)
        output, inter_refs = self.decoder_forward(
            tgt=tgt, reference_points=reference_points, src=src, src_spatial_shapes=src_spatial_shapes,
            src_level_start_index=src_level_start_index, src_valid_ratios=src_valid_ratios, query_pos=query_pos,
            src_padding_mask=src_padding_mask, tgt_key_padding_mask=tgt_key_padding_mask, **kwargs)
        decoder_outputs["init_reference_out"] = reference_points
        decoder_outputs.update({"hs": output, "inter_references_out": inter_refs})
        return decoder_outputs


class DeformableTransformer(nn.Module):

    def __init__(self, d_model=256, nhead=8, num_encoder_layers=6, num_decoder_layers=6, dim_feedforward=1024,
                 encoder=None, decoder=None, decoder_layer=None, encoder_layer=None, dropout=0.1, activation="relu",
                 return_intermediate_dec=False, num_feature_levels=4, dec_n_points=4, enc_n_points=4,
                 two_stage=False, two_stage_num_proposals=300):
        super().__init__()
        if two_stage and 2 * d_model != PROPOSAL_EMBED_DIM:
            raise ValueError(f"two-stage Deformable-DETR needs d_model = {PROPOSAL_EMBED_DIM // 2}: the proposals' sine embedding is "
                             f"fixed at 4 x 128 = {PROPOSAL_EMBED_DIM} = 2 * d_model channels (got d_model = {d_model})")
        self.d_model, self.nhead = d_model, nhead
        self.two_stage, self.two_stage_num_proposals = two_stage, two_stage_num_proposals
        if encoder is None:
            encoder_layer = encoder_layer or DeformableTransformerEncoderLayer(
                d_model, dim_feedforward, dropout, activation, num_feature_levels, nhead, enc_n_points)
            encoder = DeformableTransformerEncoder(encoder_layer, num_encoder_layers)
        self.encoder = encoder
        if decoder is None:
            decoder_layer = decoder_layer or DeformableTransformerDecoderLayer(
                d_model, dim_feedforward, dropout, activation, num_feature_levels, nhead, dec_n_points)
            decoder = DeformableTransformerDecoder(decoder_layer, num_decoder_layers, return_intermediate_dec)
        self.decoder = decoder
        self.level_embed = nn.Parameter(torch.Tensor(num_feature_levels, d_model))
        if two_stage:
            self.enc_output = nn.Linear(d_model, d_model)
            self.enc_output_norm = nn.LayerNorm(d_model)
            self.pos_trans = nn.Linear(d_model * 2, d_model * 2)
            self.pos_trans_norm = nn.LayerNorm(d_model * 2)
        else:
            self.reference_points = nn.Linear(d_model, 2)
        self._reset_parameters()

    def _reset_parameters(self):
        for p in self.parameters():
            if p.dim() > 1:
                nn.init.xavier_uniform_(p)
        for m in self.modules():
            if isinstance(m, MSDeformAttn):
                m._reset_parameters()
        if not self.two_stage:
            xavier_uniform_(self.reference_points.weight.data, gain=1.0)
            constant_(self.reference_points.bias.data, 0.0)
        normal_(self.level_embed)

    def get_proposal_pos_embed(self, proposals):
        return proposal_pos_embed(proposals)

    def gen_encoder_output_proposals(self, memory, memory_padding_mask, shapes, fused=False):
        if fused and alo_hip.encoder_proposals_masked_supported(memory_padding_mask, shapes, memory):
            proposals, keep, output_memory = alo_hip.encoder_proposals_masked(memory_padding_mask, shapes, memory)
        else:
            if fused and alo_hip.encoder_proposals_supported(memory_padding_mask, shapes):
                proposals, keep = alo_hip.encoder_proposals(memory_padding_mask, shapes)
            else:
                proposals, keep = encoder_output_proposals(memory_padding_mask, shapes)
            if fused and alo_hip.mask_rows_supported(memory, keep):
                output_memory = alo_hip.mask_rows(memory, keep)
            else:
                output_memory = memory.masked_fill(~keep.unsqueeze(-1), 0.0)
        if fused and alo_hip.add_layernorm_supported(output_memory):
            output_memory = _add_norm(self.enc_output_norm,
                                      alo_hip.linear_auto(output_memory, self.enc_output.weight, self.enc_output.bias), None)
        else:
            output_memory = self.enc_output_norm(self.enc_output(output_memory))
        return output_memory, proposals

    def _proposal_heads(self):
        n = self.decoder.num_layers
        for name in ("class_embed", "bbox_embed"):
            heads = getattr(self.decoder, name, None)
            if heads is None:
                raise RuntimeError(f"two-stage DeformableTransformer: decoder.{name} is missing — attach the detection heads "
                                   f"({n + 1} of them: one per decoder layer and one for the encoder's proposals) before the forward")
            if len(heads) <= n:
                raise RuntimeError(f"two-stage DeformableTransformer: decoder.{name} holds {len(heads)} heads, the proposals "
                                   f"are scored by entry {n} (one per decoder layer and one more)")
        return self.decoder.class_embed[n], self.decoder.bbox_embed[n]

    def _two_stage_queries(self, memory, mask_flatten, shapes, kwargs):
        class_head, box_head = self._proposal_heads()
        fused = _fused_ok(self, kwargs, memory, self.enc_output.weight, self.pos_trans.weight)
        output_memory, output_proposals = self.gen_encoder_output_proposals(memory, mask_flatten, shapes, fused=fused)
        enc_outputs_class = class_head(output_memory)
        enc_outputs_coord_unact = box_head(output_memory) + output_proposals
        topk = torch.topk(enc_outputs_class[..., 0], self.two_stage_num_proposals, dim=1)[1]
        if fused and alo_hip.proposal_queries_supported(enc_outputs_coord_unact, topk, memory.dtype):
            reference_points, embed = alo_hip.proposal_queries(enc_outputs_coord_unact, topk, memory.dtype, owner=self.pos_trans.weight)
        else:
            coords = torch.gather(enc_outputs_coord_unact, 1, topk.unsqueeze(-1).expand(-1, -1, 4)).detach()
            reference_points = coords.sigmoid()
            embed = proposal_pos_embed(coords).to(memory.dtype)
        if fused and alo_hip.add_layernorm_supported(embed):
            pos_trans_out = _add_norm(self.pos_trans_norm, alo_hip.linear_auto(embed, self.pos_trans.weight, self.pos_trans.bias), None)
        else:
            pos_trans_out = self.pos_trans_norm(self.pos_trans(embed))
        query_pos, tgt = torch.split(pos_trans_out, memory.shape[-1], dim=2)
        if fused:
            query_pos, tgt = query_pos.contiguous(), tgt.contiguous()
        return query_pos, tgt, reference_points, enc_outputs_class, enc_outputs_coord_unact

    @staticmethod
    def get_valid_ratio(mask):
        _, H, W = mask.shape
        valid_h = torch.sum((~mask).float()[:, :, 0], 1, keepdim=True)
        valid_w = torch.sum((~mask).float()[:, 0, :], 1, keepdim=True)
        return torch.cat([valid_w / W, valid_h / H], 1)

    def forward(self, srcs, masks, pos_embeds, query_embed=None, **kwargs):
        assert self.two_stage or query_embed is not None
        device = srcs[0].device
        src_flatten, mask_flatten, pos_flatten, shapes = [], [], [], []
        pos_encoder = kwargs.pop("pos_encoder", None)
        ready = kwargs.pop("src_flatten", None)
        ready_mask = kwargs.pop("mask_flatten", None)
        ready_ratios = kwargs.pop("valid_ratios", None)
        for lvl, (src, mask, pos_embed) in enumerate(zip(srcs, masks, pos_embeds)):
            _, _, h, w = src.shape
            shapes.append((h, w))
            if ready is None:
                src_flatten.append(src.flatten(2).transpose(1, 2))
            if ready_mask is None:
                mask_flatten.append(mask.flatten(1))
            if pos_embed is not None:
                pos_flatten.append(pos_embed.flatten(2).transpose(1, 2) + self.level_embed[lvl].view(1, 1, -1))
        src_flatten = torch.cat(src_flatten, 1) if ready is None else ready
        mask_flatten = torch.cat(mask_flatten, 1) if ready_mask is None else ready_mask
        spatial_shapes, level_start_index = _level_geometry(tuple(shapes), device)
        sizes = [h * w for h, w in shapes]
        if pos_flatten:
            pos_flatten = torch.cat(pos_flatten, 1).to(src_flatten.dtype)
        else:
            pos_flatten = alo_hip.pos_sine_flat(mask_flatten, spatial_shapes, level_start_index, pos_encoder.dim_t(device),
                                                self.level_embed, pos_encoder.normalize, pos_encoder.center,
                                                pos_encoder.scale, src_flatten.dtype)
        valid_ratios = torch.stack([self.get_valid_ratio(m) for m in masks], 1) if ready_ratios is None else ready_ratios

        memory = self.encoder(src_flatten, spatial_shapes, level_start_index, valid_ratios, pos_flatten, mask_flatten,
                              **kwargs)

        bs, _, c = memory.shape
        enc_outputs_class = enc_outputs_coord_unact = None
        if self.two_stage:
            query_pos, tgt, reference_points, enc_outputs_class, enc_outputs_coord_unact = self._two_stage_queries(
                memory, mask_flatten, shapes, kwargs)
        else:
            query_pos, tgt = torch.split(query_embed, c, dim=1)
            query_pos = query_pos.unsqueeze(0).expand(bs, -1, -1)
            tgt = tgt.unsqueeze(0).expand(bs, -1, -1)
            if _fused_ok(self, kwargs, memory, query_embed):
                query_pos, tgt = query_pos.contiguous(), tgt.contiguous()
            reference_points = self.reference_points(query_pos).sigmoid()

        out = {}
        out.update(self.decoder(tgt, reference_points, memory, spatial_shapes, level_start_index, valid_ratios,
                                query_pos=query_pos, src_padding_mask=mask_flatten, **kwargs))
        memory_t = memory.transpose(1, 2)
        splits, start = [], 0
        for (h, w), n in zip(shapes, sizes):
            splits.append(memory_t[..., start:start + n].reshape(bs, c, h, w))
            start += n
        out["memory"] = splits
        out["enc_outputs_class"] = enc_outputs_class
        out["enc_outputs_coord_unact"] = enc_outputs_coord_unact
        return out
```

aloception-oss_amd/alonet/deformable_detr/ops/modules/ms_deform_attn.py:

```python
import math
import warnings

import torch
import torch.nn.functional as F
from torch import nn
from torch.nn.init import constant_, xavier_uniform_

import alo_hip

from ..functions import MSDeformAttnFunction, load_MultiScaleDeformableAttention, ms_deform_attn_core_pytorch


def _is_power_of_2(n):
    if not isinstance(n, int) or n < 0:
        raise ValueError("invalid input for _is_power_of_2: {} (type: {})".format(n, type(n)))
    return n != 0 and (n & (n - 1)) == 0


class MSDeformAttn(nn.Module):
    def __init__(self, d_model=256, n_levels=4, n_heads=8, n_points=4):
        super().__init__()
        if d_model % n_heads != 0:
            raise ValueError("d_model must be divisible by n_heads, but got {} and {}".format(d_model, n_heads))
        if not _is_power_of_2(d_model // n_heads):
            warnings.warn(
                "d_model // n_heads is not a power of 2: the gfx950 kernel then leaves lanes idle "
                "(channels per head are spread over a power-of-two lane group)."
            )
        self.im2col_step = 64
        self.fused_prologue = True
        self.d_model, self.n_levels, self.n_heads, self.n_points = d_model, n_levels, n_heads, n_points

        self.sampling_offsets = nn.Linear(d_model, n_heads * n_levels * n_points * 2)
        self.attention_weights = nn.Linear(d_model, n_heads * n_levels * n_points)
        self.value_proj = nn.Linear(d_model, d_model)
        self.output_proj = nn.Linear(d_model, d_model)
        self._reset_parameters()

        load_MultiScaleDeformableAttention()

    def _reset_parameters(self):
        constant_(self.sampling_offsets.weight.data, 0.0)
        angle = torch.arange(self.n_heads, dtype=torch.float32) * (2.0 * math.pi / self.n_heads)
        ring = torch.stack([angle.cos(), angle.sin()], -1)
        ring = ring / ring.abs().max(-1, keepdim=True)[0]
        ring = ring.view(self.n_heads, 1, 1, 2).repeat(1, self.n_levels, self.n_points, 1)
        ring = ring * torch.arange(1, self.n_points + 1, dtype=torch.float32).view(1, 1, self.n_points, 1)
        with torch.no_grad():
            self.sampling_offsets.bias = nn.Parameter(ring.reshape(-1))
        constant_(self.attention_weights.weight.data, 0.0)
        constant_(self.attention_weights.bias.data, 0.0)
        xavier_uniform_(self.value_proj.weight.data)
        constant_(self.value_proj.bias.data, 0.0)
        xavier_uniform_(self.output_proj.weight.data)
        constant_(self.output_proj.bias.data, 0.0)

    def _merged_query_projection(self):
        so, aw = self.sampling_offsets, self.attention_weights
        return alo_hip.derived(self, "merged", (so.weight, so.bias, aw.weight, aw.bias),
                               lambda: (torch.cat([so.weight, aw.weight], 0).contiguous(),
                                        torch.cat([so.bias, aw.bias], 0).contiguous()))

    def forward(self, query, reference_points, input_flatten, input_spatial_shapes, input_level_start_index,
                input_padding_mask=None, **kwargs):
        N, Lq, _ = query.shape
        _, S, _ = input_flatten.shape
        total = getattr(input_spatial_shapes, "_alo_total", None)
        if total is None:
            total = int((input_spatial_shapes[:, 0] * input_spatial_shapes[:, 1]).sum())
        assert total == S
        M, L, P = self.n_heads, self.n_levels, self.n_points

        if reference_points.shape[-1] not in (2, 4):
            raise ValueError(
                "Last dim of reference_points must be 2 or 4, but get {} instead.".format(reference_points.shape[-1])
            )
        needs_grad = torch.is_grad_enabled() and (
            any(t.requires_grad for t in (query, input_flatten, reference_points))
            or any(p.requires_grad for p in self.parameters()))
        fused = "is_tracing" not in kwargs and not needs_grad and self.fused_prologue and query.is_cuda
        proj = (lambda lin, t: alo_hip.linear_auto(t, lin.weight, lin.bias)) if fused else (lambda lin, t: lin(t))
        D = self.d_model // M
        hm = (fused and D == 32 and L == 4 and P == 4 and self.value_proj.bias is not None
              and alo_hip.value_proj_head_major_supported(input_flatten, self.value_proj.weight, M))
        if hm and self.sampling_offsets.bias is not None and self.attention_weights.bias is not None:
            w_cat, b_cat = self._merged_query_projection()
            both = alo_hip.linear_auto(query, w_cat, b_cat)
            offsets = both[..., :M * L * P * 2].view(N, Lq, M, L, P, 2)
            logits = both[..., M * L * P * 2:].view(N, Lq, M, L * P)
        else:
            offsets = proj(self.sampling_offsets, query).view(N, Lq, M, L, P, 2)
            logits = proj(self.attention_weights, query).view(N, Lq, M, L * P)
        if hm:
            value = alo_hip.value_proj_head_major(input_flatten, self.value_proj.weight, self.value_proj.bias,
                                                  input_padding_mask, M)
            output = alo_hip.msda_forward_fused_hm(value, input_spatial_shapes, input_level_start_index, offsets, logits,
                                                   reference_points)
            return proj(self.output_proj, output)
        value = proj(self.value_proj, input_flatten)

        if fused and alo_hip.head_major_supported(value.view(N, S, M, self.d_model // M), L, P):
            value = alo_hip.value_head_major(value.view(N, S, M, self.d_model // M), input_padding_mask)
            output = alo_hip.msda_forward_fused_hm(value, input_spatial_shapes, input_level_start_index,
                                                   offsets.contiguous(), logits.contiguous(), reference_points)
            return proj(self.output_proj, output)

        if input_padding_mask is not None:
            if needs_grad:
                value = value.masked_fill(input_padding_mask[..., None], float(0))
            else:
                value.masked_fill_(input_padding_mask[..., None], float(0))
        value = value.view(N, S, M, self.d_model // M)
        low_precision = value.dtype in (torch.bfloat16, torch.float16)
        geo = torch.float32 if low_precision else value.dtype

        if fused:
            output = alo_hip.msda_forward_fused(value.contiguous(), input_spatial_shapes, input_level_start_index,
                                                offsets.contiguous(), logits.contiguous(), reference_points)
            return proj(self.output_proj, output)

        offsets = offsets.to(geo)
        weights = F.softmax(logits.to(geo), -1).view(N, Lq, M, L, P)
        reference_points = reference_points.to(geo)
        if reference_points.shape[-1] == 2:
            normalizer = torch.stack([input_spatial_shapes[..., 1], input_spatial_shapes[..., 0]], -1)
            locations = reference_points[:, :, None, :, None, :] + offsets / normalizer[None, None, None, :, None, :]
        else:
            locations = (
                reference_points[:, :, None, :, None, :2]
                + offsets / P * reference_points[:, :, None, :, None, 2:] * 0.5
            )

        if "is_tracing" in kwargs:
            output = ms_deform_attn_core_pytorch(value.to(geo), input_spatial_shapes, locations, weights).to(value.dtype)
        else:
            output = MSDeformAttnFunction.apply(
                value, input_spatial_shapes, input_level_start_index, locations, weights, self.im2col_step
            )
        return self.output_proj(output)
```

aloception-oss_amd/csrc/common.hpp:

```cpp
#pragma once
#include <hip/hip_runtime.h>
#include <stdint.h>

#include <cstdarg>
#include <cstdio>

#include "../../include/alo_hotpath.h"

namespace alo {

char* error_buffer();
inline int fail(alo_status_t code, const char* fmt, ...) {
    va_list ap;
    va_start(ap, fmt);
    vsnprintf(error_buffer(), 512, fmt, ap);
    va_end(ap);
    return (int)code;
}
#define ALO_REQUIRE(cond, code, ...) \
    do {                             \
        if (!(cond)) return ::alo::fail(code, __VA_ARGS__); \
    } while (0)

template <typename... P>
inline bool aligned16(const P*... p) {
    return ((... | (uintptr_t)p) & 15) == 0;
}

constexpr int kLdsLimit = 160 * 1024;
template <auto kernel>
int launch(dim3 grid, dim3 block, size_t lds, hipStream_t stream, const char* what, void** args) {
    ALO_REQUIRE(lds <= (size_t)kLdsLimit, ALO_ERR_UNSUPPORTED, "%s: %zu bytes of dynamic LDS, the limit is %d", what, lds, kLdsLimit);
    const void* fn = reinterpret_cast<const void*>(kernel);
    hipError_t e = hipSuccess;
    if (lds > 48 * 1024) {
        static unsigned long long done = 0;
        int dev = 0;
        e = hipGetDevice(&dev);
        const unsigned long long bit = 1ull << (dev & 63);
        if (e == hipSuccess && !(__atomic_load_n(&done, __ATOMIC_ACQUIRE) & bit)) {
            e = hipFuncSetAttribute(fn, hipFuncAttributeMaxDynamicSharedMemorySize, kLdsLimit);
            if (e == hipSuccess) __atomic_fetch_or(&done, bit, __ATOMIC_RELEASE);
        }
    }
    if (e == hipSuccess) e = hipLaunchKernel(fn, grid, block, args, lds, stream);
    if (e == hipSuccess) e = hipGetLastError();
    if (e != hipSuccess) return fail(ALO_ERR_LAUNCH, "%s: %s", what, hipGetErrorString(e));
    return ALO_OK;
}

constexpr int kNumXcd = 8;

__device__ __forceinline__ unsigned xcd_contiguous_block(unsigned bid, unsigned nblocks) {
    const unsigned q = nblocks / kNumXcd, r = nblocks % kNumXcd;
    const unsigned xcd = bid % kNumXcd, k = bid / kNumXcd;
    const unsigned start = xcd < r ? xcd * (q + 1) : r * (q + 1) + (xcd - r) * q;
    return start + k;
}

int msda_backward_wide(const void* value, const int32_t* shapes, const int32_t* lstart, const void* loc, const void* attn,
                       const void* grad_out, void* grad_value, void* grad_loc, void* grad_attn, int N, int S, int M, int D, int Lq,
                       int value_dtype, const int32_t* host_shapes, hipStream_t stream, bool plan_only = false);

struct RowGather {
    int s, Wo, HoWo, W, HW;
};
inline RowGather row_gather(int stride = 1, int Ho = 1, int Wo = 1, int H = 1, int W = 1) { return {stride, Wo, Ho * Wo, W, H * W}; }

int linear_shortk_gather(const void* x, const void* weight, const void* bias, const void* residual, void* y, long M, int N, int K,
                         int relu, const RowGather& gather, hipStream_t stream);

#define ALO_RELU_RES(fn, first, relu, residual, ...)                                                                          \
    ((residual) ? ((relu) ? fn<first, true, true>(__VA_ARGS__) : fn<first, false, true>(__VA_ARGS__))                          \
                : ((relu) ? fn<first, true, false>(__VA_ARGS__) : fn<first, false, false>(__VA_ARGS__)))

typedef __attribute__((ext_vector_type(4))) unsigned int u32x4;
typedef __attribute__((ext_vector_type(2))) unsigned int u32x2;
typedef __attribute__((ext_vector_type(4))) float f32x4;
typedef __attribute__((ext_vector_type(16))) float f32x16;

struct bf16_t {
    uint16_t bits;
};

__device__ __forceinline__ float relu_keep_nan(float v) { return (v > 0.f || v != v) ? v : 0.f; }

__device__ __forceinline__ float bf16_to_f32(uint16_t b) { return __uint_as_float(((unsigned)b) << 16); }
__device__ __forceinline__ uint16_t f32_to_bf16(float f) {
    const __bf16 b = static_cast<__bf16>(f);
    return __builtin_bit_cast(uint16_t, b);
}
__device__ __forceinline__ unsigned pack_bf16x2(float lo, float hi) {
    typedef __bf16 bf16x2_hw __attribute__((ext_vector_type(2)));
    typedef float f32x2_hw __attribute__((ext_vector_type(2)));
    const bf16x2_hw r = __builtin_convertvector(f32x2_hw{lo, hi}, bf16x2_hw);
    return __builtin_bit_cast(unsigned, r);
}

typedef __attribute__((ext_vector_type(8))) __bf16 bf16x8_t;
__device__ __forceinline__ bf16x8_t as_bf16x8(const u32x4& v) {
    union { u32x4 u; bf16x8_t b; } x;
    x.u = v;
    return x.b;
}

template <bool RELU>
__device__ __forceinline__ u32x4 add_residual_bf16x8(const u32x4& v, const u32x4& rv) {
    const unsigned a4[4] = {v.x, v.y, v.z, v.w}, r4[4] = {rv.x, rv.y, rv.z, rv.w};
    unsigned o4[4];
#pragma unroll
    for (int i = 0; i < 4; ++i) {
        float lo = __uint_as_float(a4[i] << 16) + __uint_as_float(r4[i] << 16);
        float hi = __uint_as_float(a4[i] & 0xffff0000u) + __uint_as_float(r4[i] & 0xffff0000u);
        if (RELU) { lo = relu_keep_nan(lo); hi = relu_keep_nan(hi); }
        o4[i] = pack_bf16x2(lo, hi);
    }
    return u32x4{o4[0], o4[1], o4[2], o4[3]};
}

__device__ __forceinline__ long gather_row(const RowGather& g, long row) {
    if (g.s <= 1) return row;
    const long n = row / g.HoWo;
    const int rem = (int)(row - n * g.HoWo);
    const int yo = rem / g.Wo, xo = rem - yo * g.Wo;
    return n * g.HW + (long)(yo * g.s) * g.W + xo * g.s;
}

__device__ __forceinline__ __amdgpu_buffer_rsrc_t make_rsrc(const void* base, unsigned bytes) {
    return __builtin_amdgcn_make_buffer_rsrc(const_cast<void*>(base), 0, (int)bytes, 0x00020000);
}
constexpr unsigned kOutOfRange = 0xC0000000u;

template <typename T, typename CT, int VEC>
struct Loader;

template <>
struct Loader<float, float, 4> {
    using raw_t = u32x4;
    static __device__ __forceinline__ raw_t load(__amdgpu_buffer_rsrc_t r, unsigned off) {
        return __builtin_amdgcn_raw_buffer_load_b128(r, off, 0, 0);
    }
    static __device__ __forceinline__ void widen(const raw_t& x, float (&v)[4]) {
        v[0] = __uint_as_float(x.x); v[1] = __uint_as_float(x.y); v[2] = __uint_as_float(x.z); v[3] = __uint_as_float(x.w);
    }
};
template <>
struct Loader<float, float, 1> {
    using raw_t = unsigned;
    static __device__ __forceinline__ raw_t load(__amdgpu_buffer_rsrc_t r, unsigned off) {
        return __builtin_amdgcn_raw_buffer_load_b32(r, off, 0, 0);
    }
    static __device__ __forceinline__ void widen(const raw_t& x, float (&v)[1]) { v[0] = __uint_as_float(x); }
};
template <>
struct Loader<double, double, 2> {
    using raw_t = u32x4;
    static __device__ __forceinline__ raw_t load(__amdgpu_buffer_rsrc_t r, unsigned off) {
        return __builtin_amdgcn_raw_buffer_load_b128(r, off, 0, 0);
    }
    static __device__ __forceinline__ void widen(const raw_t& x, double (&v)[2]) {
        v[0] = __hiloint2double((int)x.y, (int)x.x);
        v[1] = __hiloint2double((int)x.w, (int)x.z);
    }
};
template <>
struct Loader<double, double, 1> {
    using raw_t = u32x2;
    static __device__ __forceinline__ raw_t load(__amdgpu_buffer_rsrc_t r, unsigned off) {
        return __builtin_amdgcn_raw_buffer_load_b64(r, off, 0, 0);
    }
    static __device__ __forceinline__ void widen(const raw_t& x, double (&v)[1]) {
        v[0] = __hiloint2double((int)x.y, (int)x.x);
    }
};
template <>
struct Loader<bf16_t, float, 8> {
    using raw_t = u32x4;
    static __device__ __forceinline__ raw_t load(__amdgpu_buffer_rsrc_t r, unsigned off) {
        return __builtin_amdgcn_raw_buffer_load_b128(r, off, 0, 0);
    }
    static __device__ __forceinline__ void widen(const raw_t& x, float (&v)[8]) {
        const unsigned w[4] = {x.x, x.y, x.z, x.w};
#pragma unroll
        for (int i = 0; i < 4; ++i) {
            v[2 * i] = __uint_as_float(w[i] << 16);
            v[2 * i + 1] = __uint_as_float(w[i] & 0xffff0000u);
        }
    }
};
template <>
struct Loader<bf16_t, float, 1> {
    using raw_t = unsigned short;
    static __device__ __forceinline__ raw_t load(__amdgpu_buffer_rsrc_t r, unsigned off) {
        return __builtin_amdgcn_raw_buffer_load_b16(r, off, 0, 0);
    }
    static __device__ __forceinline__ void widen(const raw_t& x, float (&v)[1]) { v[0] = bf16_to_f32(x); }
};

__device__ __forceinline__ float ld(const float* p) { return *p; }
__device__ __forceinline__ double ld(const double* p) { return *p; }
__device__ __forceinline__ float ld(const bf16_t* p) { return bf16_to_f32(p->bits); }
__device__ __forceinline__ void st(float* p, float v) { *p = v; }
__device__ __forceinline__ void st(double* p, double v) { *p = v; }
__device__ __forceinline__ void st(bf16_t* p, float v) { p->bits = f32_to_bf16(v); }

template <typename T, typename CT, int VEC>
__device__ __forceinline__ void store_vec(T* p, const CT (&v)[VEC]) {
    if constexpr (sizeof(T) == 4 && VEC == 4) {
        *reinterpret_cast<f32x4*>(p) = f32x4{(float)v[0], (float)v[1], (float)v[2], (float)v[3]};
    } else if constexpr (sizeof(T) == 8 && VEC == 2) {
        *reinterpret_cast<double2*>(p) = double2{(double)v[0], (double)v[1]};
    } else if constexpr (sizeof(T) == 2 && VEC == 8) {
        u32x4 o;
        o.x = pack_bf16x2(v[0], v[1]);
        o.y = pack_bf16x2(v[2], v[3]);
        o.z = pack_bf16x2(v[4], v[5]);
        o.w = pack_bf16x2(v[6], v[7]);
        *reinterpret_cast<u32x4*>(p) = o;
    } else {
#pragma unroll
        for (int i = 0; i < VEC; ++i) st(p + i, v[i]);
    }
}

}
```

aloception-oss_amd/csrc/fused.hip:

```cpp
#include "common.hpp"

namespace alo {
namespace {

constexpr int kThreads = 256;
constexpr int kMaxChunks = 4;

__device__ __forceinline__ float wave_sum(float v) {
#pragma unroll
    for (int o = 32; o > 0; o >>= 1) v += __shfl_xor(v, o, 64);
    return v;
}

__device__ __forceinline__ void load4(const float* p, float (&v)[4]) {
    const f32x4 x = *reinterpret_cast<const f32x4*>(p);
    v[0] = x[0]; v[1] = x[1]; v[2] = x[2]; v[3] = x[3];
}
__device__ __forceinline__ void load4(const bf16_t* p, float (&v)[4]) {
    const u32x2 x = *reinterpret_cast<const u32x2*>(p);
    v[0] = __uint_as_float(x.x << 16); v[1] = __uint_as_float(x.x & 0xffff0000u);
    v[2] = __uint_as_float(x.y << 16); v[3] = __uint_as_float(x.y & 0xffff0000u);
}
__device__ __forceinline__ void store4(float* p, const float (&v)[4]) {
    *reinterpret_cast<f32x4*>(p) = f32x4{v[0], v[1], v[2], v[3]};
}
__device__ __forceinline__ void store4(bf16_t* p, const float (&v)[4]) {
    u32x2 o;
    o.x = pack_bf16x2(v[0], v[1]);
    o.y = pack_bf16x2(v[2], v[3]);
    *reinterpret_cast<u32x2*>(p) = o;
}

template <typename T, int CHUNKS, bool HAS_RES, bool HAS_POS>
__global__ void __launch_bounds__(kThreads)
add_layernorm_kernel(const T* x, const T* res, const T* __restrict__ gamma, const T* __restrict__ beta, T* out,
                     const T* pos, T* out_pos, long rows, int C, float eps) {
    const int lane = threadIdx.x & 63;
    const long wave = (long)blockIdx.x * (kThreads / 64) + (threadIdx.x >> 6);
    const long nwaves = (long)gridDim.x * (kThreads / 64);
    float g[CHUNKS][4], b[CHUNKS][4];
#pragma unroll
    for (int k = 0; k < CHUNKS; ++k) {
        const int c = 256 * k + 4 * lane;
        if (c < C) { load4(gamma + c, g[k]); load4(beta + c, b[k]); }
    }
    const float inv_c = 1.0f / (float)C;
    for (long r = wave; r < rows; r += nwaves) {
        const long base = r * C;
        float v[CHUNKS][4];
        float s = 0.f;
#pragma unroll
        for (int k = 0; k < CHUNKS; ++k) {
            const int c = 256 * k + 4 * lane;
#pragma unroll
            for (int i = 0; i < 4; ++i) v[k][i] = 0.f;
            if (c < C) {
                load4(x + base + c, v[k]);
                if constexpr (HAS_RES) {
                    float t[4];
                    load4(res + base + c, t);
#pragma unroll
                    for (int i = 0; i < 4; ++i) v[k][i] += t[i];
                }
#pragma unroll
                for (int i = 0; i < 4; ++i) s += v[k][i];
            }
        }
        const float mean = wave_sum(s) * inv_c;
        float q = 0.f;
#pragma unroll
        for (int k = 0; k < CHUNKS; ++k) {
            const int c = 256 * k + 4 * lane;
            if (c < C) {
#pragma unroll
                for (int i = 0; i < 4; ++i) { const float d = v[k][i] - mean; q += d * d; }
            }
        }
        const float rstd = rsqrtf(wave_sum(q) * inv_c + eps);
#pragma unroll
        for (int k = 0; k < CHUNKS; ++k) {
            const int c = 256 * k + 4 * lane;
            if (c < C) {
                float y[4];
#pragma unroll
                for (int i = 0; i < 4; ++i) y[i] = (v[k][i] - mean) * rstd * g[k][i] + b[k][i];
                store4(out + base + c, y);
                if constexpr (HAS_POS) {
                    float p[4];
                    load4(pos + base + c, p);
                    if constexpr (sizeof(T) == 2) {
#pragma unroll
                        for (int i = 0; i < 4; ++i) y[i] = bf16_to_f32(f32_to_bf16(y[i]));
                    }
#pragma unroll
                    for (int i = 0; i < 4; ++i) y[i] += p[i];
                    store4(out_pos + base + c, y);
                }
            }
        }
    }
}

template <typename T, bool HAS_RES, bool RELU>
__global__ void __launch_bounds__(kThreads)
bias_act_kernel(const T* x, const T* __restrict__ bias, const T* res, T* y,
                long n4, int C) {
    const long stride = (long)gridDim.x * kThreads;
    for (long i = (long)blockIdx.x * kThreads + threadIdx.x; i < n4; i += stride) {
        const long e = i * 4;
        const int c = (int)(e % C);
        float v[4], bb[4];
        load4(x + e, v);
        load4(bias + c, bb);
#pragma unroll
        for (int k = 0; k < 4; ++k) v[k] += bb[k];
        if constexpr (HAS_RES) {
            float t[4];
            load4(res + e, t);
#pragma unroll
            for (int k = 0; k < 4; ++k) v[k] += t[k];
        }
        if constexpr (RELU) {
#pragma unroll
            for (int k = 0; k < 4; ++k) v[k] = relu_keep_nan(v[k]);
        }
        store4(y + e, v);
    }
}

__global__ void __launch_bounds__(kThreads)
value_head_major_kernel(const bf16_t* __restrict__ value, const unsigned char* __restrict__ mask,
                        bf16_t* __restrict__ out, int S, int M, int D) {
    const int n = blockIdx.y;
    const int s0 = blockIdx.x * 64;
    const int vec_per_row = M * D / 8;
    const int vec_per_head = D / 8;
    const int total = 64 * vec_per_row;
    for (int i = threadIdx.x; i < total; i += kThreads) {
        const int m = i / (64 * vec_per_head);
        const int rem = i - m * 64 * vec_per_head;
        const int sp = rem / vec_per_head, v = rem - sp * vec_per_head;
        const int s = s0 + sp;
        if (s >= S) continue;
        u32x4 x = *reinterpret_cast<const u32x4*>(value + ((size_t)n * S + s) * M * D + m * D + v * 8);
        if (mask != nullptr && mask[(size_t)n * S + s]) x = u32x4{0u, 0u, 0u, 0u};
        *reinterpret_cast<u32x4*>(out + (((size_t)n * M + m) * S + s) * D + v * 8) = x;
    }
}

template <bool RELU>
__global__ void __launch_bounds__(kThreads)
bias_act_nchw_kernel(const float* x, const float* __restrict__ bias, float* y, long n4, int C, int HW4) {
    const long stride = (long)gridDim.x * kThreads;
    for (long i = (long)blockIdx.x * kThreads + threadIdx.x; i < n4; i += stride) {
        const int c = (int)((i / HW4) % C);
        float v[4];
        load4(x + i * 4, v);
        const float b = bias[c];
#pragma unroll
        for (int k = 0; k < 4; ++k) { v[k] += b; if (RELU) v[k] = relu_keep_nan(v[k]); }
        store4(y + i * 4, v);
    }
}

__device__ __forceinline__ float sigmoidf_(float v) { return 1.0f / (1.0f + expf(-v)); }

__global__ void __launch_bounds__(kThreads)
gru_gate_kernel(float* zr, const float* __restrict__ bias_zr, const float* h, float* rh, long n4, int C, int HW4,
                long hb, long rb) {
    const long stride = (long)gridDim.x * kThreads;
    for (long i = (long)blockIdx.x * kThreads + threadIdx.x; i < n4; i += stride) {
        const long plane = i / HW4;
        const int p4 = (int)(i - plane * HW4);
        const int b = (int)(plane / C), c = (int)(plane - (long)b * C);
        const long zoff = (((long)b * 2 * C + c) * HW4 + p4) * 4;
        const long roff = zoff + (long)C * HW4 * 4;
        const long hoff = (long)b * hb + ((long)c * HW4 + p4) * 4;
        const long rhoff = (long)b * rb + ((long)c * HW4 + p4) * 4;
        float z[4], r[4], hv[4];
        load4(zr + zoff, z);
        load4(zr + roff, r);
        load4(h + hoff, hv);
        const float bz = bias_zr[c], br = bias_zr[C + c];
#pragma unroll
        for (int k = 0; k < 4; ++k) {
            z[k] = sigmoidf_(z[k] + bz);
            r[k] = sigmoidf_(r[k] + br) * hv[k];
        }
        store4(zr + zoff, z);
        store4(rh + rhoff, r);
    }
}

__global__ void __launch_bounds__(kThreads)
gru_update_kernel(const float* q, const float* __restrict__ bias_q, const float* zr, float* h, float* net, long n4, int C,
                  int HW4, long hb) {
    const long stride = (long)gridDim.x * kThreads;
    for (long i = (long)blockIdx.x * kThreads + threadIdx.x; i < n4; i += stride) {
        const long plane = i / HW4;
        const int p4 = (int)(i - plane * HW4);
        const int b = (int)(plane / C), c = (int)(plane - (long)b * C);
        const long zoff = (((long)b * 2 * C + c) * HW4 + p4) * 4;
        const long hoff = (long)b * hb + ((long)c * HW4 + p4) * 4;
        float qv[4], z[4], hv[4];
        load4(q + i * 4, qv);
        load4(zr + zoff, z);
        load4(h + hoff, hv);
        const float bq = bias_q[c];
#pragma unroll
        for (int k = 0; k < 4; ++k) hv[k] = (1.0f - z[k]) * hv[k] + z[k] * tanhf(qv[k] + bq);
        store4(h + hoff, hv);
        if (net != nullptr) store4(net + i * 4, hv);
    }
}

__global__ void __launch_bounds__(kThreads)
pos_prefix_kernel(const unsigned char* __restrict__ mask, const int32_t* __restrict__ shapes,
                  const int32_t* __restrict__ lstart, float* __restrict__ emb, int S, int normalize, int center,
                  float scale, float eps) {
    const int l = blockIdx.y, b = blockIdx.z;
    const int H = shapes[2 * l], W = shapes[2 * l + 1], start = lstart[l];
    const unsigned char* mk = mask + (size_t)b * S + start;
    float* e = emb + ((size_t)b * S + start) * 2;
    const float shift = (normalize && center) ? 0.5f : 0.0f;
    const int lane = threadIdx.x & 63, wave = threadIdx.x >> 6;
    const int col_items = (W + 63) / 64, items = col_items + H;
    for (int item = blockIdx.x * (kThreads / 64) + wave; item < items; item += gridDim.x * (kThreads / 64)) {
        if (item < col_items) {
            const int x = item * 64 + lane;
            if (x < W) {
                float cum = 0.f;
#pragma unroll 4
                for (int y = 0; y < H; ++y) cum += mk[y * W + x] ? 0.f : 1.f;
                const float denom = (cum - shift) + eps;
                float run = 0.f;
#pragma unroll 4
                for (int y = 0; y < H; ++y) {
                    run += mk[y * W + x] ? 0.f : 1.f;
                    e[(y * W + x) * 2] = normalize ? (run - shift) / denom * scale : run;
                }
            }
        } else {
            const int y = item - col_items;
            const int per = (W + 63) / 64, x0 = lane * per, x1 = min(W, x0 + per);
            float mine = 0.f;
            for (int x = x0; x < x1; ++x) mine += mk[y * W + x] ? 0.f : 1.f;
            float incl = mine;
#pragma unroll
            for (int o = 1; o < 64; o <<= 1) {
                const float up = __shfl_up(incl, o, 64);
                if (lane >= o) incl += up;
            }
            const float total = __shfl(incl, 63, 64);
            const float denom = (total - shift) + eps;
            float run = incl - mine;
            for (int x = x0; x < x1; ++x) {
                run += mk[y * W + x] ? 0.f : 1.f;
                e[(y * W + x) * 2 + 1] = normalize ? (run - shift) / denom * scale : run;
            }
        }
    }
}

template <typename T>
__global__ void __launch_bounds__(kThreads)
pos_generate_kernel(const float* __restrict__ emb, const float* __restrict__ dim_t, const T* __restrict__ level_embed,
                    const int32_t* __restrict__ lstart, T* __restrict__ out, long n4, int S, int L, int F) {
    const int C = 2 * F, c4 = C / 4;
    const long stride = (long)gridDim.x * kThreads;
    for (long i = (long)blockIdx.x * kThreads + threadIdx.x; i < n4; i += stride) {
        const long pix = i / c4;
        const int c0 = (int)(i - pix * c4) * 4;
        const int s = (int)(pix % S);
        int l = 0;
        while (l + 1 < L && s >= lstart[l + 1]) ++l;
        const float e = emb[pix * 2 + (c0 < F ? 0 : 1)];
        float le[4] = {0.f, 0.f, 0.f, 0.f}, v[4];
        if (level_embed != nullptr) load4(level_embed + (size_t)l * C + c0, le);
#pragma unroll
        for (int k = 0; k < 4; k += 2) {
            const int f = (c0 + k) % F;
            const float p = e / dim_t[f];
            float sn, cs;
            sincosf(p, &sn, &cs);
            v[k] = sn + le[k];
            v[k + 1] = (dim_t[f + 1] == dim_t[f] ? cs : cosf(e / dim_t[f + 1])) + le[k + 1];
        }
        store4(out + pix * C + c0, v);
    }
}

template <typename T>
int add_layernorm_t(const void* x, const void* res, const void* gamma, const void* beta, void* out, const void* pos,
                    void* out_pos, long rows, int C, float eps, hipStream_t stream) {
    const int chunks = (C + 255) / 256;
    long blocks = (rows + 3) / 4;
    if (blocks > 256L * 32) blocks = 256L * 32;
    void* args[] = {&x, &res, &gamma, &beta, &out, &pos, &out_pos, &rows, &C, &eps};
    const char* what = "alo_add_layernorm";
#define ALO_LN_CASE(CH)                                                                                            \
    if (chunks == CH) {                                                                                            \
        if (res && pos) return launch<add_layernorm_kernel<T, CH, true, true>>((unsigned)blocks, kThreads, 0, stream, what, args);   \
        if (res) return launch<add_layernorm_kernel<T, CH, true, false>>((unsigned)blocks, kThreads, 0, stream, what, args);         \
        if (pos) return launch<add_layernorm_kernel<T, CH, false, true>>((unsigned)blocks, kThreads, 0, stream, what, args);         \
        return launch<add_layernorm_kernel<T, CH, false, false>>((unsigned)blocks, kThreads, 0, stream, what, args);                 \
    }
    ALO_LN_CASE(1) ALO_LN_CASE(2) ALO_LN_CASE(3) ALO_LN_CASE(4)
#undef ALO_LN_CASE
    return fail(ALO_ERR_UNSUPPORTED, "alo_add_layernorm: C = %d is above %d", C, 256 * kMaxChunks);
}

template <typename T>
int bias_act_t(const void* x, const void* bias, const void* res, void* y, long rows, int C, int relu, hipStream_t stream) {
    long n4 = rows * C / 4;
    long blocks = (n4 + kThreads - 1) / kThreads;
    if (blocks > 256L * 64) blocks = 256L * 64;
    void* args[] = {&x, &bias, &res, &y, &n4, &C};
    const char* what = "alo_bias_act";
    if (res) {
        if (relu) return launch<bias_act_kernel<T, true, true>>((unsigned)blocks, kThreads, 0, stream, what, args);
        return launch<bias_act_kernel<T, true, false>>((unsigned)blocks, kThreads, 0, stream, what, args);
    }
    if (relu) return launch<bias_act_kernel<T, false, true>>((unsigned)blocks, kThreads, 0, stream, what, args);
    return launch<bias_act_kernel<T, false, false>>((unsigned)blocks, kThreads, 0, stream, what, args);
}

}
}

using namespace alo;

extern "C" int alo_add_layernorm(const void* x, const void* residual, const void* gamma, const void* beta, void* out,
                                 const void* pos, void* out_pos, long rows, int C, float eps, int dtype, void* stream) {
    ALO_REQUIRE(x && gamma && beta && out, ALO_ERR_INVALID_ARGUMENT, "alo_add_layernorm: null pointer argument");
    ALO_REQUIRE((pos == nullptr) == (out_pos == nullptr), ALO_ERR_INVALID_ARGUMENT,
                "alo_add_layernorm: pos and out_pos go together");
    ALO_REQUIRE(rows > 0 && C > 0 && C % 4 == 0, ALO_ERR_INVALID_ARGUMENT,
                "alo_add_layernorm: rows must be positive and C a positive multiple of 4 (rows=%ld C=%d)", rows, C);
    ALO_REQUIRE(aligned16(x, residual, gamma, beta, out, pos, out_pos), ALO_ERR_INVALID_ARGUMENT,
                "alo_add_layernorm: pointers must be 16-byte aligned");
    hipStream_t s = static_cast<hipStream_t>(stream);
    if (dtype == ALO_F32) return add_layernorm_t<float>(x, residual, gamma, beta, out, pos, out_pos, rows, C, eps, s);
    if (dtype == ALO_BF16) return add_layernorm_t<bf16_t>(x, residual, gamma, beta, out, pos, out_pos, rows, C, eps, s);
    return fail(ALO_ERR_UNSUPPORTED, "alo_add_layernorm: dtype %d (F32 and BF16 are supported)", dtype);
}

extern "C" int alo_bias_act(const void* x, const void* bias, const void* residual, void* y, long rows, int C, int relu,
                            int dtype, void* stream) {
    ALO_REQUIRE(x && bias && y, ALO_ERR_INVALID_ARGUMENT, "alo_bias_act: null pointer argument");
    ALO_REQUIRE(rows > 0 && C > 0 && C % 4 == 0, ALO_ERR_INVALID_ARGUMENT,
                "alo_bias_act: rows must be positive and C a positive multiple of 4 (rows=%ld C=%d)", rows, C);
    ALO_REQUIRE(aligned16(x, bias, residual, y), ALO_ERR_INVALID_ARGUMENT, "alo_bias_act: pointers must be 16-byte aligned");
    hipStream_t s = static_cast<hipStream_t>(stream);
    if (dtype == ALO_F32) return bias_act_t<float>(x, bias, residual, y, rows, C, relu, s);
    if (dtype == ALO_BF16) return bias_act_t<bf16_t>(x, bias, residual, y, rows, C, relu, s);
    return fail(ALO_ERR_UNSUPPORTED, "alo_bias_act: dtype %d (F32 and BF16 are supported)", dtype);
}

extern "C" int alo_value_head_major(const void* value, const void* padding_mask, void* out, int N, int S, int M, int D,
                                    int dtype, void* stream) {
    ALO_REQUIRE(value && out, ALO_ERR_INVALID_ARGUMENT, "alo_value_head_major: null pointer argument");
    ALO_REQUIRE(N > 0 && S > 0 && M > 0 && D > 0 && D % 8 == 0, ALO_ERR_INVALID_ARGUMENT,
                "alo_value_head_major: dimensions must be positive and D a multiple of 8 (N=%d S=%d M=%d D=%d)", N, S, M, D);
    ALO_REQUIRE(dtype == ALO_BF16, ALO_ERR_UNSUPPORTED, "alo_value_head_major: bf16 only (dtype %d)", dtype);
    ALO_REQUIRE(aligned16(value, out), ALO_ERR_INVALID_ARGUMENT, "alo_value_head_major: pointers must be 16-byte aligned");
    void* args[] = {&value, &padding_mask, &out, &S, &M, &D};
    return launch<value_head_major_kernel>(dim3((S + 63) / 64, N), kThreads, 0, static_cast<hipStream_t>(stream), "alo_value_head_major", args);
}

static unsigned stream_blocks(long n4) {
    long blocks = (n4 + kThreads - 1) / kThreads;
    return (unsigned)(blocks > 256L * 64 ? 256L * 64 : blocks);
}

extern "C" int alo_bias_act_nchw(const float* x, const float* bias, float* y, int B, int C, int HW, int relu, void* stream) {
    ALO_REQUIRE(x && bias && y, ALO_ERR_INVALID_ARGUMENT, "alo_bias_act_nchw: null pointer argument");
    ALO_REQUIRE(B > 0 && C > 0 && HW > 0 && HW % 4 == 0, ALO_ERR_INVALID_ARGUMENT,
                "alo_bias_act_nchw: dimensions must be positive and H*W a multiple of 4 (B=%d C=%d HW=%d)", B, C, HW);
    ALO_REQUIRE(aligned16(x, y), ALO_ERR_INVALID_ARGUMENT, "alo_bias_act_nchw: pointers must be 16-byte aligned");
    long n4 = (long)B * C * HW / 4;
    int hw4 = HW / 4;
    void* args[] = {&x, &bias, &y, &n4, &C, &hw4};
    hipStream_t s = static_cast<hipStream_t>(stream);
    if (relu) return launch<bias_act_nchw_kernel<true>>(stream_blocks(n4), kThreads, 0, s, "alo_bias_act_nchw", args);
    return launch<bias_act_nchw_kernel<false>>(stream_blocks(n4), kThreads, 0, s, "alo_bias_act_nchw", args);
}

extern "C" int alo_gru_gate(float* zr, const float* bias_zr, const float* h, float* rh, int B, int C, int HW,
                            long h_batch_stride, long rh_batch_stride, void* stream) {
    ALO_REQUIRE(zr && bias_zr && h && rh, ALO_ERR_INVALID_ARGUMENT, "alo_gru_gate: null pointer argument");
    ALO_REQUIRE(B > 0 && C > 0 && HW > 0 && HW % 4 == 0 && h_batch_stride % 4 == 0 && rh_batch_stride % 4 == 0,
                ALO_ERR_INVALID_ARGUMENT, "alo_gru_gate: H*W and the batch strides must be multiples of 4 (B=%d C=%d HW=%d)",
                B, C, HW);
    ALO_REQUIRE(aligned16(zr, h, rh), ALO_ERR_INVALID_ARGUMENT, "alo_gru_gate: pointers must be 16-byte aligned");
    long n4 = (long)B * C * HW / 4;
    int hw4 = HW / 4;
    void* args[] = {&zr, &bias_zr, &h, &rh, &n4, &C, &hw4, &h_batch_stride, &rh_batch_stride};
    return launch<gru_gate_kernel>(stream_blocks(n4), kThreads, 0, static_cast<hipStream_t>(stream), "alo_gru_gate", args);
}

extern "C" int alo_gru_update(const float* q, const float* bias_q, const float* zr, float* h, float* net, int B, int C,
                              int HW, long h_batch_stride, void* stream) {
    ALO_REQUIRE(q && bias_q && zr && h, ALO_ERR_INVALID_ARGUMENT, "alo_gru_update: null pointer argument");
    ALO_REQUIRE(B > 0 && C > 0 && HW > 0 && HW % 4 == 0 && h_batch_stride % 4 == 0, ALO_ERR_INVALID_ARGUMENT,
                "alo_gru_update: H*W and the batch stride must be multiples of 4 (B=%d C=%d HW=%d)", B, C, HW);
    ALO_REQUIRE(aligned16(q, zr, h, net), ALO_ERR_INVALID_ARGUMENT, "alo_gru_update: pointers must be 16-byte aligned");
    long n4 = (long)B * C * HW / 4;
    int hw4 = HW / 4;
    void* args[] = {&q, &bias_q, &zr, &h, &net, &n4, &C, &hw4, &h_batch_stride};
    return launch<gru_update_kernel>(stream_blocks(n4), kThreads, 0, static_cast<hipStream_t>(stream), "alo_gru_update", args);
}

extern "C" int alo_pos_sine_flat(const void* padding_mask, const int32_t* spatial_shapes, const int32_t* level_start_index,
                                 const float* dim_t, const void* level_embed, void* out, float* workspace, int B, int S,
                                 int L, int num_pos_feats, int normalize, int center, float scale, float eps, int dtype,
                                 void* stream) {
    ALO_REQUIRE(padding_mask && spatial_shapes && level_start_index && dim_t && out && workspace, ALO_ERR_INVALID_ARGUMENT,
                "alo_pos_sine_flat: null pointer argument");
    ALO_REQUIRE(B > 0 && S > 0 && L > 0 && num_pos_feats > 0 && num_pos_feats % 4 == 0, ALO_ERR_INVALID_ARGUMENT,
                "alo_pos_sine_flat: sizes must be positive and num_pos_feats a multiple of 4 (B=%d S=%d L=%d F=%d)", B, S, L,
                num_pos_feats);
    ALO_REQUIRE(dtype == ALO_F32 || dtype == ALO_BF16, ALO_ERR_UNSUPPORTED, "alo_pos_sine_flat: dtype %d", dtype);
    ALO_REQUIRE(aligned16(out, level_embed), ALO_ERR_INVALID_ARGUMENT, "alo_pos_sine_flat: out / level_embed must be 16-byte aligned");
    hipStream_t st = static_cast<hipStream_t>(stream);
    {
        void* args[] = {&padding_mask, &spatial_shapes, &level_start_index, &workspace, &S, &normalize, &center, &scale, &eps};
        if (int rc = launch<pos_prefix_kernel>(dim3(32, L, B), kThreads, 0, st, "alo_pos_sine_flat", args)) return rc;
    }
    long n4 = (long)B * S * (2 * num_pos_feats) / 4;
    void* args[] = {&workspace, &dim_t, &level_embed, &level_start_index, &out, &n4, &S, &L, &num_pos_feats};
    if (dtype == ALO_F32) return launch<pos_generate_kernel<float>>(stream_blocks(n4), kThreads, 0, st, "alo_pos_sine_flat", args);
    return launch<pos_generate_kernel<bf16_t>>(stream_blocks(n4), kThreads, 0, st, "alo_pos_sine_flat", args);
}
```

aloception-oss_amd/csrc/gemm.hip:

```cpp
#include "common.hpp"

namespace alo {
namespace {

constexpr int kRows = 64;
constexpr int kOutStride = 64 * 2 + 16;

struct GemmDims {
    long M;
    int N;
    int tiles;
    int S;
    RowGather g;
};

template <int kK, bool RELU, bool HAS_RES, bool HM>
__global__ void __launch_bounds__(256, 2)
linear_shortk_kernel(const bf16_t* __restrict__ X, const bf16_t* __restrict__ W, const bf16_t* __restrict__ bias,
                     const bf16_t* __restrict__ R, bf16_t* __restrict__ Y, const GemmDims dm) {
    constexpr int kRowBytes = kK * 2 + 16;
    constexpr int kSteps = kK / 16;
    constexpr int kPieces = kK / 8;
    constexpr int kLoads = kRows * kPieces / 256;
    static_assert(kRows * kPieces % 256 == 0, "the tile loader gives every thread the same number of pieces");
    extern __shared__ __attribute__((aligned(16))) unsigned char smem[];
    unsigned char* const xbuf = smem;
    const int tid = threadIdx.x, wave = tid >> 6, lane = tid & 63;
    unsigned char* obuf = smem + kRows * kRowBytes + wave * (kRows * kOutStride);

    const int col0 = blockIdx.y * 256 + wave * 64;
    const bool has_cols = col0 < dm.N;
    const int nl = lane & 31, kg = lane >> 5;

    u32x4 wreg[2][kSteps];
    float* const bias_tab = reinterpret_cast<float*>(smem + kRows * kRowBytes + 4 * (kRows * kOutStride)) + wave * 64;
    if (has_cols) {
#pragma unroll
        for (int t = 0; t < 2; ++t) {
            const bf16_t* wr = W + (size_t)(col0 + 32 * t + nl) * kK + 8 * kg;
#pragma unroll
            for (int s = 0; s < kSteps; ++s) wreg[t][s] = *reinterpret_cast<const u32x4*>(wr + 16 * s);
        }
        const int r = lane & 15, t = (lane >> 4) & 1, k2 = lane >> 5;
        bias_tab[lane] = bias != nullptr ? bf16_to_f32(bias[col0 + 32 * t + (r & 3) + 8 * (r >> 2) + 4 * k2].bits) : 0.f;
    }

    auto fetch = [&](int tile, u32x4 (&r)[kLoads]) {
#pragma unroll
        for (int j = 0; j < kLoads; ++j) {
            const int p = tid + 256 * j;
            long row = (long)tile * kRows + p / kPieces;
            row = gather_row(dm.g, row < dm.M ? row : dm.M - 1);
            r[j] = *reinterpret_cast<const u32x4*>(X + row * kK + (p % kPieces) * 8);
        }
    };
    auto park = [&](const u32x4 (&r)[kLoads]) {
#pragma unroll
        for (int j = 0; j < kLoads; ++j) {
            const int p = tid + 256 * j;
            *reinterpret_cast<u32x4*>(xbuf + (p / kPieces) * kRowBytes + (p % kPieces) * 16) = r[j];
        }
    };

    int tile = blockIdx.x;
    if (tile >= dm.tiles) return;
    u32x4 stage[kLoads];
    fetch(tile, stage);

    for (;;) {
        park(stage);
        __syncthreads();
        const int next = tile + gridDim.x;
        const bool more = next < dm.tiles;
        if (more) fetch(next, stage);

        if (has_cols) {
#pragma unroll
            for (int half = 0; half < kRows / 32; ++half) {
                f32x16 acc[2];
#pragma unroll
                for (int t = 0; t < 2; ++t)
#pragma unroll
                    for (int q = 0; q < 4; ++q) {
                        const f32x4 b4 = *reinterpret_cast<const f32x4*>(bias_tab + (kg * 2 + t) * 16 + 4 * q);
#pragma unroll
                        for (int i = 0; i < 4; ++i) acc[t][4 * q + i] = b4[i];
                    }
#pragma unroll
                for (int s = 0; s < kSteps; ++s) {
                    const u32x4 a = *reinterpret_cast<const u32x4*>(xbuf + (32 * half + nl) * kRowBytes + (16 * s + 8 * kg) * 2);
                    acc[0] = __builtin_amdgcn_mfma_f32_32x32x16_bf16(as_bf16x8(wreg[0][s]), as_bf16x8(a), acc[0], 0, 0, 0);
                    acc[1] = __builtin_amdgcn_mfma_f32_32x32x16_bf16(as_bf16x8(wreg[1][s]), as_bf16x8(a), acc[1], 0, 0, 0);
                }
#pragma unroll
                for (int t = 0; t < 2; ++t)
#pragma unroll
                    for (int q = 0; q < 4; ++q) {
                        float v0 = acc[t][4 * q], v1 = acc[t][4 * q + 1], v2 = acc[t][4 * q + 2], v3 = acc[t][4 * q + 3];
                        if (RELU && !HAS_RES) { v0 = relu_keep_nan(v0); v1 = relu_keep_nan(v1); v2 = relu_keep_nan(v2); v3 = relu_keep_nan(v3); }
                        *reinterpret_cast<u32x2*>(obuf + (32 * half + nl) * kOutStride + (32 * t + 8 * q + 4 * kg) * 2) =
                            u32x2{pack_bf16x2(v0, v1), pack_bf16x2(v2, v3)};
                    }
            }
            __builtin_amdgcn_fence(__ATOMIC_RELEASE, "wavefront");
            __builtin_amdgcn_wave_barrier();
            __builtin_amdgcn_fence(__ATOMIC_ACQUIRE, "wavefront");
            if constexpr (HM) {
                const unsigned char* mask = reinterpret_cast<const unsigned char*>(R);
                const int heads = dm.N / 32;
#pragma unroll
                for (int hh = 0; hh < 2; ++hh) {
#pragma unroll
                    for (int pass = 0; pass < kRows / 16; ++pass) {
                        const int row = pass * 16 + (lane >> 2);
                        const long grow = (long)tile * kRows + row;
                        if (grow < dm.M) {
                            u32x4 v = *reinterpret_cast<const u32x4*>(obuf + row * kOutStride + hh * 64 + (lane & 3) * 16);
                            if (mask != nullptr && mask[grow]) v = u32x4{0u, 0u, 0u, 0u};
                            const long nb = grow / dm.S, sp = grow - nb * dm.S;
                            const int head = col0 / 32 + hh;
                            *reinterpret_cast<u32x4*>(Y + ((nb * heads + head) * dm.S + sp) * 32 + (lane & 3) * 8) = v;
                        }
                    }
                }
            } else
#pragma unroll
            for (int pass = 0; pass < kRows / 8; ++pass) {
                const int row = pass * 8 + (lane >> 3);
                const long grow = (long)tile * kRows + row;
                u32x4 v = *reinterpret_cast<const u32x4*>(obuf + row * kOutStride + (lane & 7) * 16);
                if (grow < dm.M) {
                    if constexpr (HAS_RES) {
                        v = add_residual_bf16x8<RELU>(v, *reinterpret_cast<const u32x4*>(R + grow * dm.N + col0 + (lane & 7) * 8));
                    }
                    *reinterpret_cast<u32x4*>(Y + grow * dm.N + col0 + (lane & 7) * 8) = v;
                }
            }
        }
        if (!more) break;
        __syncthreads();
        tile = next;
    }
}

}
}

using namespace alo;

namespace {
template <int K, bool RELU, bool HAS_RES, bool HM = false>
int launch_shortk(const void* x, const void* weight, const void* bias, const void* residual, void* y, long M, int N,
                  hipStream_t stream, int S = 0, const RowGather& gather = row_gather()) {
    GemmDims dm;
    dm.M = M; dm.N = N; dm.tiles = (int)((M + kRows - 1) / kRows); dm.S = S; dm.g = gather;
    const size_t lds = kRows * (K * 2 + 16) + 4 * kRows * kOutStride + 4 * 64 * sizeof(float);
    const int cols = (N + 255) / 256;
    int gx = 512 / cols;
    if (gx > dm.tiles) gx = dm.tiles;
    if (gx < 1) gx = 1;
    void* args[] = {&x, &weight, &bias, &residual, &y, &dm};
    return launch<linear_shortk_kernel<K, RELU, HAS_RES, HM>>(dim3(gx, cols), 256, lds, stream, "alo_linear_shortk", args);
}
}

extern "C" int alo_linear_shortk(const void* x, const void* weight, const void* bias, const void* residual, void* y, long M,
                                 int N, int K, int relu, int dtype, void* stream) {
    ALO_REQUIRE(x && weight && y, ALO_ERR_INVALID_ARGUMENT, "alo_linear_shortk: null pointer argument");
    ALO_REQUIRE(M > 0 && N > 0 && N % 64 == 0, ALO_ERR_INVALID_ARGUMENT,
                "alo_linear_shortk: M must be positive and N a positive multiple of 64 (M=%ld N=%d)", M, N);
    ALO_REQUIRE(K == 64 || K == 128 || K == 256, ALO_ERR_UNSUPPORTED, "alo_linear_shortk: K must be 64, 128 or 256, got %d", K);
    ALO_REQUIRE(dtype == ALO_BF16, ALO_ERR_UNSUPPORTED, "alo_linear_shortk: bf16 only (dtype %d)", dtype);
    ALO_REQUIRE(aligned16(x, weight, y, residual), ALO_ERR_INVALID_ARGUMENT, "alo_linear_shortk: pointers must be 16-byte aligned");
    return linear_shortk_gather(x, weight, bias, residual, y, M, N, K, relu, row_gather(), static_cast<hipStream_t>(stream));
}

int alo::linear_shortk_gather(const void* x, const void* weight, const void* bias, const void* residual, void* y, long M, int N, int K,
                              int relu, const RowGather& gather, hipStream_t stream) {
    if (K == 64) return ALO_RELU_RES(launch_shortk, 64, relu, residual, x, weight, bias, residual, y, M, N, stream, 0, gather);
    if (K == 128) return ALO_RELU_RES(launch_shortk, 128, relu, residual, x, weight, bias, residual, y, M, N, stream, 0, gather);
    if (K == 256) return ALO_RELU_RES(launch_shortk, 256, relu, residual, x, weight, bias, residual, y, M, N, stream, 0, gather);
    return fail(ALO_ERR_UNSUPPORTED, "alo_conv1x1_nhwc: the resident-weight kernel needs Cin in (64, 128, 256), got %d", K);
}

namespace alo {
namespace {

constexpr int kFfnRows = 64;
constexpr int kFfnStride = 256 * 2 + 16;

struct FfnDims {
    long M;
    int F;
    int tiles;
};

__global__ void __launch_bounds__(256, 2)
ffn256_kernel(const bf16_t* __restrict__ X, const bf16_t* __restrict__ W1, const bf16_t* __restrict__ B1,
              const bf16_t* __restrict__ W2, const bf16_t* __restrict__ B2, bf16_t* __restrict__ Y, const FfnDims dm) {
    extern __shared__ __attribute__((aligned(16))) unsigned char smem[];
    unsigned char* const xs = smem;
    unsigned char* const hs = smem + kFfnRows * kFfnStride;
    const int tid = threadIdx.x, wave = tid >> 6, lane = tid & 63;
    const int nl = lane & 31, kg = lane >> 5;
    const int F = dm.F;

    float* const b1s = reinterpret_cast<float*>(smem + 2 * kFfnRows * kFfnStride);
    float* const b2s = b1s + F;
    for (int i = tid; i < F; i += 256) b1s[i] = B1 ? bf16_to_f32(B1[i].bits) : 0.f;
    b2s[tid] = B2 ? bf16_to_f32(B2[tid].bits) : 0.f;

    constexpr int KB = 2;
    constexpr int NBATCH = 16 / KB;
    auto load_batch = [&](u32x4 (&buf)[2][KB], const bf16_t* frag0, size_t tile_stride, int batch) {
#pragma unroll
        for (int t = 0; t < 2; ++t)
#pragma unroll
            for (int j = 0; j < KB; ++j)
                buf[t][j] = *reinterpret_cast<const u32x4*>(frag0 + t * tile_stride + (size_t)(KB * batch + j) * 512);
        __builtin_amdgcn_sched_barrier(0);
    };
    auto mma_batch = [&](f32x16 (&acc)[2][2], const unsigned char* a_lds, const u32x4 (&buf)[2][KB], int batch) {
        u32x4 af[2][KB];
#pragma unroll
        for (int j = 0; j < KB; ++j) {
            const int s = KB * batch + j;
            af[0][j] = *reinterpret_cast<const u32x4*>(a_lds + nl * kFfnStride + (16 * s + 8 * kg) * 2);
            af[1][j] = *reinterpret_cast<const u32x4*>(a_lds + (32 + nl) * kFfnStride + (16 * s + 8 * kg) * 2);
        }
#pragma unroll
        for (int j = 0; j < KB; ++j) {
            const u32x4 a0 = af[0][j], a1 = af[1][j];
            acc[0][0] = __builtin_amdgcn_mfma_f32_32x32x16_bf16(as_bf16x8(buf[0][j]), as_bf16x8(a0), acc[0][0], 0, 0, 0);
            acc[0][1] = __builtin_amdgcn_mfma_f32_32x32x16_bf16(as_bf16x8(buf[1][j]), as_bf16x8(a0), acc[0][1], 0, 0, 0);
            acc[1][0] = __builtin_amdgcn_mfma_f32_32x32x16_bf16(as_bf16x8(buf[0][j]), as_bf16x8(a1), acc[1][0], 0, 0, 0);
            acc[1][1] = __builtin_amdgcn_mfma_f32_32x32x16_bf16(as_bf16x8(buf[1][j]), as_bf16x8(a1), acc[1][1], 0, 0, 0);
        }
        __builtin_amdgcn_sched_barrier(0);
    };
    const int fs = F / 16;
    auto w1_frag = [&](int r0) { return W1 + ((size_t)((r0 + 64 * wave) / 32) * 16 * 64 + lane) * 8; };
    auto w2_frag = [&](int r0) { return W2 + (((size_t)(2 * wave) * fs + r0 / 16) * 64 + lane) * 8; };

    for (int tile = blockIdx.x; tile < dm.tiles; tile += gridDim.x) {
        {
            u32x4 xv[8];
#pragma unroll
            for (int j = 0; j < 8; ++j) {
                const int p = tid + 256 * j;
                long row = (long)tile * kFfnRows + (p >> 5);
                row = row < dm.M ? row : dm.M - 1;
                xv[j] = *reinterpret_cast<const u32x4*>(X + row * 256 + (p & 31) * 8);
            }
#pragma unroll
            for (int j = 0; j < 8; ++j) {
                const int p = tid + 256 * j;
                *reinterpret_cast<u32x4*>(xs + (p >> 5) * kFfnStride + (p & 31) * 16) = xv[j];
            }
        }
        u32x4 bufa[2][KB], bufb[2][KB];
        load_batch(bufa, w1_frag(0), (size_t)16 * 512, 0);
        __syncthreads();

        f32x16 acc2[2][2];
#pragma unroll
        for (int a = 0; a < 2; ++a)
#pragma unroll
            for (int t = 0; t < 2; ++t)
#pragma unroll
                for (int i = 0; i < 16; ++i) acc2[a][t][i] = 0.f;

        for (int r0 = 0; r0 < F; r0 += 256) {
            f32x16 acc1[2][2];
#pragma unroll
            for (int a = 0; a < 2; ++a)
#pragma unroll
                for (int t = 0; t < 2; ++t)
#pragma unroll
                    for (int i = 0; i < 16; ++i) acc1[a][t][i] = 0.f;
            const bf16_t* w1p = w1_frag(r0);
            const bf16_t* w2p = w2_frag(r0);
#pragma unroll
            for (int bt = 0; bt < NBATCH; bt += 2) {
                load_batch(bufb, w1p, (size_t)16 * 512, bt + 1);
                mma_batch(acc1, xs, bufa, bt);
                if (bt + 2 < NBATCH) load_batch(bufa, w1p, (size_t)16 * 512, bt + 2);
                else load_batch(bufa, w2p, (size_t)fs * 512, 0);
                mma_batch(acc1, xs, bufb, bt + 1);
            }
#pragma unroll
            for (int t = 0; t < 2; ++t)
#pragma unroll
                for (int q = 0; q < 4; ++q) {
                    const int col = 64 * wave + 32 * t + 8 * q + 4 * kg;
                    const f32x4 bb = *reinterpret_cast<const f32x4*>(b1s + r0 + col);
#pragma unroll
                    for (int a = 0; a < 2; ++a) {
                        const float v0 = relu_keep_nan(acc1[a][t][4 * q] + bb[0]), v1 = relu_keep_nan(acc1[a][t][4 * q + 1] + bb[1]);
                        const float v2 = relu_keep_nan(acc1[a][t][4 * q + 2] + bb[2]), v3 = relu_keep_nan(acc1[a][t][4 * q + 3] + bb[3]);
                        *reinterpret_cast<u32x2*>(hs + (32 * a + nl) * kFfnStride + col * 2) = u32x2{pack_bf16x2(v0, v1), pack_bf16x2(v2, v3)};
                    }
                }
            __syncthreads();

#pragma unroll
            for (int bt = 0; bt < NBATCH; bt += 2) {
                load_batch(bufb, w2p, (size_t)fs * 512, bt + 1);
                mma_batch(acc2, hs, bufa, bt);
                if (bt + 2 < NBATCH) load_batch(bufa, w2p, (size_t)fs * 512, bt + 2);
                else if (r0 + 256 < F) load_batch(bufa, w1_frag(r0 + 256), (size_t)16 * 512, 0);
                mma_batch(acc2, hs, bufb, bt + 1);
            }
            __syncthreads();
        }

#pragma unroll
        for (int t = 0; t < 2; ++t)
#pragma unroll
            for (int q = 0; q < 4; ++q) {
                const int col = 64 * wave + 32 * t + 8 * q + 4 * kg;
                const f32x4 bb = *reinterpret_cast<const f32x4*>(b2s + col);
#pragma unroll
                for (int a = 0; a < 2; ++a)
                    *reinterpret_cast<u32x2*>(hs + (32 * a + nl) * kFfnStride + col * 2) =
                        u32x2{pack_bf16x2(acc2[a][t][4 * q] + bb[0], acc2[a][t][4 * q + 1] + bb[1]),
                              pack_bf16x2(acc2[a][t][4 * q + 2] + bb[2], acc2[a][t][4 * q + 3] + bb[3])};
            }
        __syncthreads();
#pragma unroll
        for (int j = 0; j < 8; ++j) {
            const int p = tid + 256 * j;
            const long row = (long)tile * kFfnRows + (p >> 5);
            if (row < dm.M)
                *reinterpret_cast<u32x4*>(Y + row * 256 + (p & 31) * 8) =
                    *reinterpret_cast<const u32x4*>(hs + (p >> 5) * kFfnStride + (p & 31) * 16);
        }
        __syncthreads();
    }
}

}
}

namespace alo {
namespace {
__global__ void __launch_bounds__(256)
pack_mfma_b_kernel(const bf16_t* __restrict__ W, bf16_t* __restrict__ P, int N, int K) {
    const long total = (long)N * K / 8;
    for (long i = (long)blockIdx.x * 256 + threadIdx.x; i < total; i += (long)gridDim.x * 256) {
        const int lane = (int)(i % 64);
        const long frag = i / 64;
        const int s = (int)(frag % (K / 16)), t = (int)(frag / (K / 16));
        const int n = 32 * t + (lane & 31), k = 16 * s + 8 * (lane >> 5);
        *reinterpret_cast<u32x4*>(P + i * 8) = *reinterpret_cast<const u32x4*>(W + (size_t)n * K + k);
    }
}
}
}

extern "C" int alo_pack_mfma_b(const void* w, void* packed, int N, int K, int dtype, void* stream) {
    ALO_REQUIRE(w && packed, ALO_ERR_INVALID_ARGUMENT, "alo_pack_mfma_b: null pointer argument");
    ALO_REQUIRE(N > 0 && K > 0 && N % 32 == 0 && K % 16 == 0, ALO_ERR_INVALID_ARGUMENT,
                "alo_pack_mfma_b: N must be a multiple of 32 and K a multiple of 16 (N=%d K=%d)", N, K);
    ALO_REQUIRE(dtype == ALO_BF16, ALO_ERR_UNSUPPORTED, "alo_pack_mfma_b: bf16 only (dtype %d)", dtype);
    long total = (long)N * K / 8;
    unsigned blocks = (unsigned)((total + 255) / 256 > 4096 ? 4096 : (total + 255) / 256);
    void* args[] = {&w, &packed, &N, &K};
    return launch<pack_mfma_b_kernel>(blocks, 256, 0, static_cast<hipStream_t>(stream), "alo_pack_mfma_b", args);
}

extern "C" int alo_ffn256(const void* x, const void* w1, const void* b1, const void* w2, const void* b2, void* y, long M,
                          int F, int dtype, void* stream) {
    ALO_REQUIRE(x && w1 && w2 && y, ALO_ERR_INVALID_ARGUMENT, "alo_ffn256: null pointer argument");
    ALO_REQUIRE(M > 0 && F > 0 && F % 256 == 0, ALO_ERR_INVALID_ARGUMENT,
                "alo_ffn256: M must be positive and the hidden width a positive multiple of 256 (M=%ld F=%d)", M, F);
    ALO_REQUIRE(dtype == ALO_BF16, ALO_ERR_UNSUPPORTED, "alo_ffn256: bf16 only (dtype %d)", dtype);
    ALO_REQUIRE(aligned16(x, w1, w2, y), ALO_ERR_INVALID_ARGUMENT, "alo_ffn256: pointers must be 16-byte aligned");
    FfnDims dm;
    dm.M = M; dm.F = F; dm.tiles = (int)((M + kFfnRows - 1) / kFfnRows);
    const size_t lds = 2 * kFfnRows * kFfnStride + ((size_t)F + 256) * sizeof(float);
    int gx = dm.tiles < 512 ? dm.tiles : 512;
    void* args[] = {&x, &w1, &b1, &w2, &b2, &y, &dm};
    if (lds > (size_t)kLdsLimit) return fail(ALO_ERR_UNSUPPORTED, "alo_ffn256: hidden width %d needs %zu bytes of LDS", F, lds);
    return launch<ffn256_kernel>(gx, 256, lds, static_cast<hipStream_t>(stream), "alo_ffn256", args);
}

extern "C" int alo_value_proj_head_major(const void* x, const void* weight, const void* bias, const void* padding_mask,
                                         void* value_hm, int batch, int S, int heads, int K, int dtype, void* stream) {
    ALO_REQUIRE(x && weight && value_hm, ALO_ERR_INVALID_ARGUMENT, "alo_value_proj_head_major: null pointer argument");
    ALO_REQUIRE(batch > 0 && S > 0 && heads > 0 && heads % 2 == 0, ALO_ERR_INVALID_ARGUMENT,
                "alo_value_proj_head_major: batch, S must be positive and the head count even (batch=%d S=%d heads=%d)", batch, S,
                heads);
    ALO_REQUIRE(K == 64 || K == 128 || K == 256, ALO_ERR_UNSUPPORTED, "alo_value_proj_head_major: K must be 64, 128 or 256, got %d", K);
    ALO_REQUIRE(dtype == ALO_BF16, ALO_ERR_UNSUPPORTED, "alo_value_proj_head_major: bf16 only (dtype %d)", dtype);
    ALO_REQUIRE(aligned16(x, weight, value_hm), ALO_ERR_INVALID_ARGUMENT, "alo_value_proj_head_major: pointers must be 16-byte aligned");
    hipStream_t st = static_cast<hipStream_t>(stream);
    const long M = (long)batch * S;
    const int N = heads * 32;
    if (K == 64) return launch_shortk<64, false, false, true>(x, weight, bias, padding_mask, value_hm, M, N, st, S);
    if (K == 128) return launch_shortk<128, false, false, true>(x, weight, bias, padding_mask, value_hm, M, N, st, S);
    return launch_shortk<256, false, false, true>(x, weight, bias, padding_mask, value_hm, M, N, st, S);
}
```

Baseline: 856.5 frames/s.

## Fuse encoder layer tail, FFN and next-layer projections into one block kernel

Adds a persistent encoder-block kernel that, per 64-row tile, runs the attention output projection with residual and LayerNorm1, then the FFN with residual and LayerNorm2. It also computes the next layer's head-major value projection and merged offset/logit projection, so intermediate activations stay in LDS instead of going through global memory across several kernels. The encoder loop is rewired to chain these blocks, and the shared MFMA tile helpers are moved from the FFN kernel into common.hpp. The cost is higher LDS use per block and a large, specialised kernel that only applies to 8 heads, 4 levels, 4 points and d_model 256.

Result: faster. 902.8 frames/s (median of 6 runs) (+5.4%).

```diff
diff --git a/__graft_entry__.py b/__graft_entry__.py
--- a/__graft_entry__.py
+++ b/__graft_entry__.py
@@ -17,6 +17,7 @@
 
     alo_hip.lib()
     alo_hip.two_stage_lib()
+    alo_hip.encoder_block_lib()
     from alonet.deformable_detr.ops.functions import load_MultiScaleDeformableAttention
     from alonet.raft.corr import CorrBlock
 
diff --git a/aloception-oss_amd/alo_hip/__init__.py b/aloception-oss_amd/alo_hip/__init__.py
--- a/aloception-oss_amd/alo_hip/__init__.py
+++ b/aloception-oss_amd/alo_hip/__init__.py
@@ -1100,6 +1100,94 @@
     return out
 
 
+ENCODER_BLOCK_LIB_PATH = os.path.join(_PKG_ROOT, "libalo_encoder_block.so")
+_encoder_block_lib = None
+
+
+def encoder_block_lib():
+    global _encoder_block_lib
+    if _encoder_block_lib is None:
+        lib()
+        if not os.path.exists(ENCODER_BLOCK_LIB_PATH):
+            raise HotpathUnavailable(f"{ENCODER_BLOCK_LIB_PATH} is missing: build it with `make -C {CSRC_DIR}` (hipcc, --offload-arch=gfx950)")
+        try:
+            handle = ctypes.CDLL(ENCODER_BLOCK_LIB_PATH)
+        except OSError as e:
+            raise HotpathUnavailable(f"cannot load {ENCODER_BLOCK_LIB_PATH}: {e}") from e
+        vp, ip = ctypes.c_void_p, ctypes.c_int
+        handle.alo_encoder_block_abi_version.restype = ip
+        handle.alo_encoder_block_abi_version.argtypes = []
+        handle.alo_encoder_block.restype = ip
+        handle.alo_encoder_block.argtypes = [vp] * 21 + [ip] * 3 + [ctypes.c_float] * 2 + [ip, vp]
+        if handle.alo_encoder_block_abi_version() != 1:
+            raise HotpathUnavailable(f"{ENCODER_BLOCK_LIB_PATH} has ABI version {handle.alo_encoder_block_abi_version()}, expected 1")
+        _encoder_block_lib = handle
+    return _encoder_block_lib
+
+
+def encoder_block_enabled():
+    return os.environ.get("ALO_ENC_BLOCK", "on").lower() not in ("off", "0")
+
+
+def encoder_block_supported(src, w1, w2, *vectors, heads=8, levels=4, points=4, value_weight=None):
+    if not (fusable(src, w1, w2, value_weight, *vectors) and src.dtype == torch.bfloat16 and src.dim() == 3 and src.shape[-1] == 256
+            and src.numel() > 0 and ffn256_supported(src, w1, w2) and heads == 8 and levels == 4 and points == 4
+            and all(v is not None for v in vectors)):
+        return False
+    return value_weight is None or value_proj_head_major_supported(src, value_weight, heads)
+
+
+def _vec(t, dtype):
+    return t.to(dtype).contiguous()
+
+
+def encoder_block(src, w1, b1, w2, b2, norm2, tail=None, nxt=None):
+    if not encoder_block_supported(src, w1, w2, b1, b2, norm2[0], norm2[1]):
+        raise RuntimeError("encoder_block: needs a bf16 CUDA (N, S, 256) src outside autograd, bf16 FFN weights with a hidden width "
+                           "that is a multiple of 256, and every bias")
+    N, S, C = src.shape
+    dt, dev = src.dtype, src.device
+    src = src.contiguous()
+    Fh = w1.shape[0]
+    out = torch.empty_like(src)
+    named = [("w1", w1, (Fh, 256)), ("w2", w2, (256, Fh))]
+    t_args = [None] * 5
+    eps1 = 0.0
+    if tail is not None:
+        attn_out, wo, bo, g1, e1, eps1 = tail
+        if attn_out.shape != src.shape or attn_out.dtype != dt or attn_out.device != dev:
+            raise RuntimeError("encoder_block: attn_out must have the shape, dtype and device of src")
+        named.append(("wo", wo, (256, 256)))
+        attn_out = attn_out.contiguous()
+        t_args = [attn_out, pack_mfma_b(wo), _vec(bo, dt), _vec(g1, dt), _vec(e1, dt)]
+    n_args = [None] * 8
+    value = both = None
+    if nxt is not None:
+        pos, padding_mask, wv, bv, wq, bq = nxt
+        if pos.shape != src.shape or pos.dtype != dt or pos.device != dev:
+            raise RuntimeError("encoder_block: pos must have the shape, dtype and device of src")
+        if padding_mask is not None:
+            if padding_mask.dtype != torch.bool or tuple(padding_mask.shape) != (N, S) or padding_mask.device != dev:
+                raise RuntimeError("padding_mask must be a (N, S) bool tensor on src's device")
+            padding_mask = padding_mask.contiguous()
+        named += [("wv", wv, (256, 256)), ("wq", wq, (384, 256))]
+        value = torch.empty((N, 8, S, 32), dtype=dt, device=dev)
+        both = torch.empty((N, S, 384), dtype=dt, device=dev)
+        n_args = [pos.contiguous(), padding_mask, pack_mfma_b(wv), _vec(bv, dt), pack_mfma_b(wq), _vec(bq, dt), value, both]
+    for name, w, shape in named:
+        if tuple(w.shape) != shape or w.dtype != dt or w.device != dev:
+            raise RuntimeError(f"encoder_block: {name} must be a {shape} tensor of src's dtype on its device")
+    f_args = [src, pack_mfma_b(w1), _vec(b1, dt), pack_mfma_b(w2), _vec(b2, dt), _vec(norm2[0], dt), _vec(norm2[1], dt), out]
+    ptr = lambda t: None if t is None else _ptr(t)
+    rows = N * S
+    nbytes = 2.0 * rows * (256 * (2 + (tail is not None) + 2 * (nxt is not None)) + 384 * (nxt is not None)) + rows * (nxt is not None)
+    flops = 2.0 * rows * 256 * (2 * Fh + 256 * (tail is not None) + (256 + 384) * (nxt is not None))
+    tag = f"encoder_block/{'tail+' if tail is not None else ''}ffn{'+proj' if nxt is not None else ''}/rows={rows}"
+    with torch.cuda.device(dev), _timed(tag, nbytes, flops):
+        _check(encoder_block_lib().alo_encoder_block(*[ptr(t) for t in t_args + f_args + n_args], N, S, Fh, float(eps1), float(norm2[2]),
+                                                     ALO_BF16, _stream(dev)))
+    return out, value, both
+
 
 def panoptic_onehot(mask_logits, frame_size, threshold=0.5):
     if not mask_logits.is_cuda or mask_logits.dim() != 4:
diff --git a/aloception-oss_amd/alonet/deformable_detr/deformable_transformer.py b/aloception-oss_amd/alonet/deformable_detr/deformable_transformer.py
--- a/aloception-oss_amd/alonet/deformable_detr/deformable_transformer.py
+++ b/aloception-oss_amd/alonet/deformable_detr/deformable_transformer.py
@@ -134,6 +134,29 @@
             return _add_norm(self.norm2, src2, src, pos=pos)
         return _add_norm(self.norm2, src2, src), None
 
+    def block_supported(self, src, query):
+        attn = self.self_attn
+        return (self.activation is F.relu and attn.head_major_supported(query, src)
+                and alo_hip.encoder_block_supported(
+                    src, self.linear1.weight, self.linear2.weight, self.linear1.bias, self.linear2.bias, self.norm1.weight,
+                    self.norm1.bias, self.norm2.weight, self.norm2.bias, attn.output_proj.bias, heads=attn.n_heads,
+                    levels=attn.n_levels, points=attn.n_points, value_weight=attn.value_proj.weight))
+
+    def forward_block(self, src, value, both, pos, reference_points, spatial_shapes, level_start_index, padding_mask=None,
+                      next_layer=None):
+        attn = self.self_attn
+        out = attn.forward_head_major(value, both, reference_points, spatial_shapes, level_start_index, project=False)
+        tail = (out, attn.output_proj.weight, attn.output_proj.bias, self.norm1.weight, self.norm1.bias, self.norm1.eps)
+        nxt = None
+        if next_layer is not None:
+            n_attn = next_layer.self_attn
+            w_cat, b_cat = n_attn._merged_query_projection()
+            nxt = (pos, padding_mask, n_attn.value_proj.weight, n_attn.value_proj.bias, w_cat, b_cat)
+        return alo_hip.encoder_block(
+            src, self.linear1.weight, self.linear1.bias, self.linear2.weight, self.linear2.bias,
+            (self.norm2.weight, self.norm2.bias, self.norm2.eps),
+            tail=tail, nxt=nxt)
+
 
 class DeformableTransformerEncoder(nn.Module):
     def __init__(self, encoder_layer, num_layers):
@@ -164,6 +187,14 @@
         reference_points = self.get_reference_points(spatial_shapes, valid_ratios, device=src.device, **kwargs)
         if _fused_ok(self, kwargs, output, pos) and all(hasattr(layer, "forward_fused") for layer in self.layers):
             query = output if pos is None else output + pos
+            if (pos is not None and alo_hip.encoder_block_enabled()
+                    and all(hasattr(layer, "forward_block") and layer.block_supported(output, query) for layer in self.layers)):
+                value, both = self.layers[0].self_attn.head_major_inputs(query, output, padding_mask)
+                for i, layer in enumerate(self.layers):
+                    nxt = self.layers[i + 1] if i + 1 < len(self.layers) else None
+                    output, value, both = layer.forward_block(output, value, both, pos, reference_points, spatial_shapes,
+                                                              level_start_index, padding_mask, next_layer=nxt)
+                return output
             for i, layer in enumerate(self.layers):
                 output, query = layer.forward_fused(output, query, pos, reference_points, spatial_shapes, level_start_index,
                                                     padding_mask, next_query=i + 1 < len(self.layers), **kwargs)
diff --git a/aloception-oss_amd/alonet/deformable_detr/ops/modules/ms_deform_attn.py b/aloception-oss_amd/alonet/deformable_detr/ops/modules/ms_deform_attn.py
--- a/aloception-oss_amd/alonet/deformable_detr/ops/modules/ms_deform_attn.py
+++ b/aloception-oss_amd/alonet/deformable_detr/ops/modules/ms_deform_attn.py
@@ -61,6 +61,29 @@
                                lambda: (torch.cat([so.weight, aw.weight], 0).contiguous(),
                                         torch.cat([so.bias, aw.bias], 0).contiguous()))
 
+    def head_major_supported(self, query, input_flatten):
+        return (self.fused_prologue and query.is_cuda and self.d_model // self.n_heads == 32 and self.n_levels == 4
+                and self.n_points == 4 and self.value_proj.bias is not None and self.sampling_offsets.bias is not None
+                and self.attention_weights.bias is not None
+                and alo_hip.linear_shortk_supported(query, self.sampling_offsets.weight)
+                and alo_hip.value_proj_head_major_supported(input_flatten, self.value_proj.weight, self.n_heads))
+
+    def head_major_inputs(self, query, input_flatten, input_padding_mask=None):
+        w_cat, b_cat = self._merged_query_projection()
+        both = alo_hip.linear_auto(query, w_cat, b_cat)
+        value = alo_hip.value_proj_head_major(input_flatten, self.value_proj.weight, self.value_proj.bias, input_padding_mask,
+                                              self.n_heads)
+        return value, both
+
+    def forward_head_major(self, value, both, reference_points, input_spatial_shapes, input_level_start_index, project=True):
+        N, Lq, _ = both.shape
+        M, L, P = self.n_heads, self.n_levels, self.n_points
+        offsets = both[..., :M * L * P * 2].view(N, Lq, M, L, P, 2)
+        logits = both[..., M * L * P * 2:].view(N, Lq, M, L * P)
+        output = alo_hip.msda_forward_fused_hm(value, input_spatial_shapes, input_level_start_index, offsets, logits,
+                                               reference_points)
+        return alo_hip.linear_auto(output, self.output_proj.weight, self.output_proj.bias) if project else output
+
     def forward(self, query, reference_points, input_flatten, input_spatial_shapes, input_level_start_index,
                 input_padding_mask=None, **kwargs):
         N, Lq, _ = query.shape
@@ -84,13 +107,10 @@
         hm = (fused and D == 32 and L == 4 and P == 4 and self.value_proj.bias is not None
               and alo_hip.value_proj_head_major_supported(input_flatten, self.value_proj.weight, M))
         if hm and self.sampling_offsets.bias is not None and self.attention_weights.bias is not None:
-            w_cat, b_cat = self._merged_query_projection()
-            both = alo_hip.linear_auto(query, w_cat, b_cat)
-            offsets = both[..., :M * L * P * 2].view(N, Lq, M, L, P, 2)
-            logits = both[..., M * L * P * 2:].view(N, Lq, M, L * P)
-        else:
-            offsets = proj(self.sampling_offsets, query).view(N, Lq, M, L, P, 2)
-            logits = proj(self.attention_weights, query).view(N, Lq, M, L * P)
+            value, both = self.head_major_inputs(query, input_flatten, input_padding_mask)
+            return self.forward_head_major(value, both, reference_points, input_spatial_shapes, input_level_start_index)
+        offsets = proj(self.sampling_offsets, query).view(N, Lq, M, L, P, 2)
+        logits = proj(self.attention_weights, query).view(N, Lq, M, L * P)
         if hm:
             value = alo_hip.value_proj_head_major(input_flatten, self.value_proj.weight, self.value_proj.bias,
                                                   input_padding_mask, M)
diff --git a/aloception-oss_amd/csrc/common.hpp b/aloception-oss_amd/csrc/common.hpp
--- a/aloception-oss_amd/csrc/common.hpp
+++ b/aloception-oss_amd/csrc/common.hpp
@@ -223,4 +223,90 @@
     }
 }
 
-}
+__device__ __forceinline__ float wave_sum(float v) {
+#pragma unroll
+    for (int o = 32; o > 0; o >>= 1) v += __shfl_xor(v, o, 64);
+    return v;
+}
+
+constexpr int kTileRows = 64;
+constexpr int kTileStride = 256 * 2 + 16;
+constexpr int kTileKB = 2;
+constexpr int kTileBatches = 16 / kTileKB;
+
+__device__ __forceinline__ void load_batch(u32x4 (&buf)[2][kTileKB], const bf16_t* frag0, size_t tile_stride, int batch) {
+#pragma unroll
+    for (int t = 0; t < 2; ++t)
+#pragma unroll
+        for (int j = 0; j < kTileKB; ++j)
+            buf[t][j] = *reinterpret_cast<const u32x4*>(frag0 + t * tile_stride + (size_t)(kTileKB * batch + j) * 512);
+    __builtin_amdgcn_sched_barrier(0);
+}
+__device__ __forceinline__ void mma_batch(f32x16 (&acc)[2][2], const unsigned char* a_lds, const u32x4 (&buf)[2][kTileKB], int batch,
+                                          int nl, int kg) {
+    u32x4 af[2][kTileKB];
+#pragma unroll
+    for (int j = 0; j < kTileKB; ++j) {
+        const int s = kTileKB * batch + j;
+        af[0][j] = *reinterpret_cast<const u32x4*>(a_lds + nl * kTileStride + (16 * s + 8 * kg) * 2);
+        af[1][j] = *reinterpret_cast<const u32x4*>(a_lds + (32 + nl) * kTileStride + (16 * s + 8 * kg) * 2);
+    }
+#pragma unroll
+    for (int j = 0; j < kTileKB; ++j) {
+        const u32x4 a0 = af[0][j], a1 = af[1][j];
+        acc[0][0] = __builtin_amdgcn_mfma_f32_32x32x16_bf16(as_bf16x8(buf[0][j]), as_bf16x8(a0), acc[0][0], 0, 0, 0);
+        acc[0][1] = __builtin_amdgcn_mfma_f32_32x32x16_bf16(as_bf16x8(buf[1][j]), as_bf16x8(a0), acc[0][1], 0, 0, 0);
+        acc[1][0] = __builtin_amdgcn_mfma_f32_32x32x16_bf16(as_bf16x8(buf[0][j]), as_bf16x8(a1), acc[1][0], 0, 0, 0);
+        acc[1][1] = __builtin_amdgcn_mfma_f32_32x32x16_bf16(as_bf16x8(buf[1][j]), as_bf16x8(a1), acc[1][1], 0, 0, 0);
+    }
+    __builtin_amdgcn_sched_barrier(0);
+}
+__device__ __forceinline__ void mma_tile256(f32x16 (&acc)[2][2], const unsigned char* a_lds, u32x4 (&bufa)[2][kTileKB],
+                                            u32x4 (&bufb)[2][kTileKB], const bf16_t* w, size_t tile_stride, const bf16_t* next,
+                                            size_t next_stride, int nl, int kg) {
+#pragma unroll
+    for (int bt = 0; bt < kTileBatches; bt += 2) {
+        load_batch(bufb, w, tile_stride, bt + 1);
+        mma_batch(acc, a_lds, bufa, bt, nl, kg);
+        if (bt + 2 < kTileBatches) load_batch(bufa, w, tile_stride, bt + 2);
+        else if (next != nullptr) load_batch(bufa, next, next_stride, 0);
+        mma_batch(acc, a_lds, bufb, bt + 1, nl, kg);
+    }
+}
+
+__device__ __forceinline__ void fetch_tile256(u32x4 (&v)[8], const bf16_t* X, long row0, long M, int tid) {
+#pragma unroll
+    for (int j = 0; j < 8; ++j) {
+        const int p = tid + 256 * j;
+        long row = row0 + (p >> 5);
+        row = row < M ? row : M - 1;
+        v[j] = *reinterpret_cast<const u32x4*>(X + row * 256 + (p & 31) * 8);
+    }
+}
+__device__ __forceinline__ void park_tile256(unsigned char* lds, const u32x4 (&v)[8], int tid) {
+#pragma unroll
+    for (int j = 0; j < 8; ++j) {
+        const int p = tid + 256 * j;
+        *reinterpret_cast<u32x4*>(lds + (p >> 5) * kTileStride + (p & 31) * 16) = v[j];
+    }
+}
+template <bool ADD_BIAS, bool RELU>
+__device__ __forceinline__ void stage_tile256(unsigned char* lds, const f32x16 (&acc)[2][2], const float* bias, int wave, int nl, int kg) {
+#pragma unroll
+    for (int t = 0; t < 2; ++t)
+#pragma unroll
+        for (int q = 0; q < 4; ++q) {
+            const int col = 64 * wave + 32 * t + 8 * q + 4 * kg;
+            f32x4 bb = {0.f, 0.f, 0.f, 0.f};
+            if constexpr (ADD_BIAS) bb = *reinterpret_cast<const f32x4*>(bias + col);
+#pragma unroll
+            for (int a = 0; a < 2; ++a) {
+                float v0 = acc[a][t][4 * q], v1 = acc[a][t][4 * q + 1], v2 = acc[a][t][4 * q + 2], v3 = acc[a][t][4 * q + 3];
+                if constexpr (ADD_BIAS) { v0 += bb[0]; v1 += bb[1]; v2 += bb[2]; v3 += bb[3]; }
+                if constexpr (RELU) { v0 = relu_keep_nan(v0); v1 = relu_keep_nan(v1); v2 = relu_keep_nan(v2); v3 = relu_keep_nan(v3); }
+                *reinterpret_cast<u32x2*>(lds + (32 * a + nl) * kTileStride + col * 2) = u32x2{pack_bf16x2(v0, v1), pack_bf16x2(v2, v3)};
+            }
+        }
+}
+
+}
diff --git a/aloception-oss_amd/csrc/encoder_block.hip b/aloception-oss_amd/csrc/encoder_block.hip
--- /dev/null
+++ b/aloception-oss_amd/csrc/encoder_block.hip
@@ -0,0 +1,337 @@
+#include "common.hpp"
+
+#include "../../include/alo_encoder_block.h"
+
+namespace alo {
+namespace {
+
+constexpr int kHeads = 8;
+constexpr int kQueryCols = 384;
+constexpr int kRowsPerWave = kTileRows / 4;
+constexpr int kTables = 256 * 7 + kQueryCols;
+
+struct EncBlockArgs {
+    const bf16_t *attn, *wo, *bo, *g1, *be1;
+    const bf16_t *src, *w1, *b1, *w2, *b2, *g2, *be2;
+    bf16_t* out;
+    const bf16_t* pos;
+    const unsigned char* mask;
+    const bf16_t *wv, *bv, *wq, *bq;
+    bf16_t *value, *both;
+    long M;
+    int S, F, tiles;
+    float eps1, eps2;
+};
+
+__device__ __forceinline__ void unpack4(const u32x2& x, float (&v)[4]) {
+    v[0] = __uint_as_float(x.x << 16); v[1] = __uint_as_float(x.x & 0xffff0000u);
+    v[2] = __uint_as_float(x.y << 16); v[3] = __uint_as_float(x.y & 0xffff0000u);
+}
+__device__ __forceinline__ u32x2 pack4(const float (&v)[4]) { return u32x2{pack_bf16x2(v[0], v[1]), pack_bf16x2(v[2], v[3])}; }
+
+__device__ __forceinline__ void layernorm_row(const float (&v)[4], const f32x4& g, const f32x4& b, float eps, float (&y)[4]) {
+    const float inv_c = 1.0f / 256.f;
+    float s = 0.f;
+#pragma unroll
+    for (int i = 0; i < 4; ++i) s += v[i];
+    const float mean = wave_sum(s) * inv_c;
+    float q = 0.f;
+#pragma unroll
+    for (int i = 0; i < 4; ++i) { const float d = v[i] - mean; q += d * d; }
+    const float rstd = rsqrtf(wave_sum(q) * inv_c + eps);
+#pragma unroll
+    for (int i = 0; i < 4; ++i) y[i] = (v[i] - mean) * rstd * g[i] + b[i];
+}
+
+__device__ __forceinline__ void init_acc_bias(f32x16 (&acc)[2][2], const float* bias64, int kg) {
+#pragma unroll
+    for (int t = 0; t < 2; ++t)
+#pragma unroll
+        for (int q = 0; q < 4; ++q) {
+            const f32x4 bb = *reinterpret_cast<const f32x4*>(bias64 + 32 * t + 8 * q + 4 * kg);
+#pragma unroll
+            for (int i = 0; i < 4; ++i) { acc[0][t][4 * q + i] = bb[i]; acc[1][t][4 * q + i] = bb[i]; }
+        }
+}
+__device__ __forceinline__ void zero_acc(f32x16 (&acc)[2][2]) {
+#pragma unroll
+    for (int a = 0; a < 2; ++a)
+#pragma unroll
+        for (int t = 0; t < 2; ++t)
+#pragma unroll
+            for (int i = 0; i < 16; ++i) acc[a][t][i] = 0.f;
+}
+__device__ __forceinline__ void wave_lds_fence() {
+    __builtin_amdgcn_fence(__ATOMIC_RELEASE, "wavefront");
+    __builtin_amdgcn_wave_barrier();
+    __builtin_amdgcn_fence(__ATOMIC_ACQUIRE, "wavefront");
+}
+
+__device__ __forceinline__ const bf16_t* per_tile(const bf16_t* w) {
+    asm volatile("" : "+v"(w));
+    return w;
+}
+
+__device__ __forceinline__ unsigned warm_rows(const bf16_t* X, long first_row, long M, int lane) {
+    long row = first_row + (lane >> 2);
+    row = row < M ? row : M - 1;
+    return *reinterpret_cast<const unsigned*>(X + row * 256 + (lane & 3) * 64);
+}
+__device__ __forceinline__ void retire(unsigned v) { asm volatile("" ::"v"(v)); }
+__device__ __forceinline__ void load_rows(u32x2 (&v)[kRowsPerWave], const bf16_t* X, long first_row, long M, int lane) {
+#pragma unroll
+    for (int r = 0; r < kRowsPerWave; ++r) {
+        long row = first_row + r;
+        row = row < M ? row : M - 1;
+        v[r] = *reinterpret_cast<const u32x2*>(X + row * 256 + 4 * lane);
+    }
+}
+
+template <bool TAIL, bool PROJ>
+__global__ void __launch_bounds__(256, 2)
+encoder_block_kernel(const EncBlockArgs p) {
+    extern __shared__ __attribute__((aligned(16))) unsigned char smem[];
+    unsigned char* const A = smem;
+    unsigned char* const B = smem + kTileRows * kTileStride;
+    const int tid = threadIdx.x, lane = tid & 63;
+    const int wave = __builtin_amdgcn_readfirstlane(tid >> 6);
+    const int nl = lane & 31, kg = lane >> 5;
+    const int F = p.F;
+
+    float* const b1s = reinterpret_cast<float*>(smem + 2 * kTileRows * kTileStride);
+    float* const b2s = b1s + F;
+    float* const bos = b2s + 256;
+    float* const bvs = bos + 256;
+    float* const bqs = bvs + 256;
+    float* const g1s = bqs + kQueryCols;
+    float* const e1s = g1s + 256;
+    float* const g2s = e1s + 256;
+    float* const e2s = g2s + 256;
+    for (int i = tid; i < F; i += 256) b1s[i] = bf16_to_f32(p.b1[i].bits);
+    b2s[tid] = bf16_to_f32(p.b2[tid].bits);
+    g2s[tid] = bf16_to_f32(p.g2[tid].bits);
+    e2s[tid] = bf16_to_f32(p.be2[tid].bits);
+    if constexpr (TAIL) {
+        bos[tid] = bf16_to_f32(p.bo[tid].bits);
+        g1s[tid] = bf16_to_f32(p.g1[tid].bits);
+        e1s[tid] = bf16_to_f32(p.be1[tid].bits);
+    }
+    if constexpr (PROJ) {
+        bvs[tid] = bf16_to_f32(p.bv[tid].bits);
+        for (int i = tid; i < kQueryCols; i += 256) bqs[i] = bf16_to_f32(p.bq[i].bits);
+    }
+
+    const int fs = F / 16;
+    auto k256_frag = [&](const bf16_t* W, int col0) { return W + ((size_t)((col0 + 64 * wave) / 32) * 16 * 64 + lane) * 8; };
+    auto w2_frag = [&](int r0) { return p.w2 + (((size_t)(2 * wave) * fs + r0 / 16) * 64 + lane) * 8; };
+    constexpr size_t kStride256 = (size_t)16 * 512;
+
+    for (int tile = blockIdx.x; tile < p.tiles; tile += gridDim.x) {
+        const long row0 = (long)tile * kTileRows;
+        const int wrow = kRowsPerWave * wave;
+        const bf16_t* const wo_f = TAIL ? per_tile(k256_frag(p.wo, 0)) : nullptr;
+        const bf16_t* const wv_f = PROJ ? per_tile(k256_frag(p.wv, 0)) : nullptr;
+        const bf16_t* const wq_f = PROJ ? per_tile(k256_frag(p.wq, 0)) : nullptr;
+        u32x4 bufa[2][kTileKB], bufb[2][kTileKB];
+        {
+            u32x4 xv[8];
+            fetch_tile256(xv, TAIL ? p.attn : p.src, row0, p.M, tid);
+            park_tile256(A, xv, tid);
+        }
+
+        if constexpr (TAIL) {
+            const unsigned warm = warm_rows(p.src, row0 + wrow, p.M, lane);
+            load_batch(bufa, wo_f, kStride256, 0);
+            __syncthreads();
+            f32x16 acc[2][2];
+            init_acc_bias(acc, bos + 64 * wave, kg);
+            mma_tile256(acc, A, bufa, bufb, wo_f, kStride256, k256_frag(p.w1, 0), kStride256, nl, kg);
+            stage_tile256<false, false>(B, acc, nullptr, wave, nl, kg);
+            __syncthreads();
+            retire(warm);
+            u32x2 res[kRowsPerWave];
+            load_rows(res, p.src, row0 + wrow, p.M, lane);
+            const f32x4 g = *reinterpret_cast<const f32x4*>(g1s + 4 * lane), b = *reinterpret_cast<const f32x4*>(e1s + 4 * lane);
+#pragma unroll
+            for (int r = 0; r < kRowsPerWave; ++r) {
+                float v[4], t[4], y[4];
+                unpack4(*reinterpret_cast<const u32x2*>(B + (wrow + r) * kTileStride + lane * 8), v);
+                unpack4(res[r], t);
+#pragma unroll
+                for (int i = 0; i < 4; ++i) v[i] += t[i];
+                layernorm_row(v, g, b, p.eps1, y);
+                *reinterpret_cast<u32x2*>(A + (wrow + r) * kTileStride + lane * 8) = pack4(y);
+            }
+        } else {
+            load_batch(bufa, k256_frag(p.w1, 0), kStride256, 0);
+        }
+        __syncthreads();
+
+        {
+            f32x16 acc2[2][2];
+            zero_acc(acc2);
+            for (int r0 = 0; r0 < F; r0 += 256) {
+                f32x16 acc1[2][2];
+                zero_acc(acc1);
+                const bf16_t* w2p = w2_frag(r0);
+                mma_tile256(acc1, A, bufa, bufb, k256_frag(p.w1, r0), kStride256, w2p, (size_t)fs * 512, nl, kg);
+                stage_tile256<true, true>(B, acc1, b1s + r0, wave, nl, kg);
+                __syncthreads();
+                const bf16_t* next = r0 + 256 < F ? k256_frag(p.w1, r0 + 256) : wv_f;
+                mma_tile256(acc2, B, bufa, bufb, w2p, (size_t)fs * 512, next, kStride256, nl, kg);
+                __syncthreads();
+            }
+            stage_tile256<true, false>(B, acc2, b2s, wave, nl, kg);
+        }
+        __syncthreads();
+
+        {
+            const f32x4 g = *reinterpret_cast<const f32x4*>(g2s + 4 * lane), b = *reinterpret_cast<const f32x4*>(e2s + 4 * lane);
+#pragma unroll
+            for (int r = 0; r < kRowsPerWave; ++r) {
+                float v[4], t[4], y[4];
+                unpack4(*reinterpret_cast<const u32x2*>(B + (wrow + r) * kTileStride + lane * 8), v);
+                unpack4(*reinterpret_cast<const u32x2*>(A + (wrow + r) * kTileStride + lane * 8), t);
+#pragma unroll
+                for (int i = 0; i < 4; ++i) v[i] += t[i];
+                layernorm_row(v, g, b, p.eps2, y);
+                const u32x2 o = pack4(y);
+                *reinterpret_cast<u32x2*>(A + (wrow + r) * kTileStride + lane * 8) = o;
+                const long row = row0 + wrow + r;
+                if (row < p.M) *reinterpret_cast<u32x2*>(p.out + row * 256 + 4 * lane) = o;
+            }
+        }
+        __syncthreads();
+
+        if constexpr (PROJ) {
+            const unsigned warm = warm_rows(p.pos, row0 + wrow, p.M, lane);
+            f32x16 acc[2][2];
+            init_acc_bias(acc, bvs + 64 * wave, kg);
+            mma_tile256(acc, A, bufa, bufb, wv_f, kStride256, wq_f, kStride256, nl, kg);
+            stage_tile256<false, false>(B, acc, nullptr, wave, nl, kg);
+            __syncthreads();
+            retire(warm);
+            unsigned char masked[kTileRows / 16];
+#pragma unroll
+            for (int pass = 0; pass < kTileRows / 16; ++pass) {
+                long row = row0 + pass * 16 + (lane >> 2);
+                row = row < p.M ? row : p.M - 1;
+                masked[pass] = p.mask != nullptr ? p.mask[row] : (unsigned char)0;
+            }
+            u32x2 posr[kRowsPerWave];
+            load_rows(posr, p.pos, row0 + wrow, p.M, lane);
+            const long nb0 = row0 / p.S;
+            const int sp0 = (int)(row0 - nb0 * p.S);
+#pragma unroll
+            for (int hh = 0; hh < 2; ++hh) {
+#pragma unroll
+                for (int pass = 0; pass < kTileRows / 16; ++pass) {
+                    const int row = pass * 16 + (lane >> 2);
+                    const long grow = row0 + row;
+                    if (grow < p.M) {
+                        u32x4 v = *reinterpret_cast<const u32x4*>(B + row * kTileStride + (64 * wave + 32 * hh) * 2 + (lane & 3) * 16);
+                        if (masked[pass]) v = u32x4{0u, 0u, 0u, 0u};
+                        const unsigned over = (unsigned)(sp0 + row) / (unsigned)p.S;
+                        const long nb = nb0 + over, sp = sp0 + row - (long)over * p.S;
+                        const int head = 2 * wave + hh;
+                        *reinterpret_cast<u32x4*>(p.value + ((nb * kHeads + head) * p.S + sp) * 32 + (lane & 3) * 8) = v;
+                    }
+                }
+            }
+#pragma unroll
+            for (int r = 0; r < kRowsPerWave; ++r) {
+                float y[4], t[4];
+                unpack4(*reinterpret_cast<const u32x2*>(A + (wrow + r) * kTileStride + lane * 8), y);
+                unpack4(posr[r], t);
+#pragma unroll
+                for (int i = 0; i < 4; ++i) y[i] += t[i];
+                *reinterpret_cast<u32x2*>(A + (wrow + r) * kTileStride + lane * 8) = pack4(y);
+            }
+            __syncthreads();
+
+#pragma unroll
+            for (int pass = 0; pass < 2; ++pass) {
+                if (pass == 1 && wave >= 2) break;
+                const int col0 = 256 * pass;
+                init_acc_bias(acc, bqs + col0 + 64 * wave, kg);
+                const bf16_t* const wq_p = wq_f + (size_t)pass * 8 * kStride256;
+                const bf16_t* next = (pass == 0 && wave < 2) ? wq_f + 8 * kStride256 : nullptr;
+                mma_tile256(acc, A, bufa, bufb, wq_p, kStride256, next, kStride256, nl, kg);
+                wave_lds_fence();
+                stage_tile256<false, false>(B, acc, nullptr, wave, nl, kg);
+                wave_lds_fence();
+#pragma unroll
+                for (int k = 0; k < kTileRows / 8; ++k) {
+                    const int row = k * 8 + (lane >> 3);
+                    const long grow = row0 + row;
+                    const u32x4 v = *reinterpret_cast<const u32x4*>(B + row * kTileStride + (64 * wave) * 2 + (lane & 7) * 16);
+                    if (grow < p.M) *reinterpret_cast<u32x4*>(p.both + grow * kQueryCols + col0 + 64 * wave + (lane & 7) * 8) = v;
+                }
+            }
+            __syncthreads();
+        }
+    }
+}
+
+template <bool TAIL, bool PROJ>
+int launch_block(const EncBlockArgs& a, size_t lds, hipStream_t stream) {
+    int dev = 0, cus = 0;
+    if (hipGetDevice(&dev) != hipSuccess || hipDeviceGetAttribute(&cus, hipDeviceAttributeMultiprocessorCount, dev) != hipSuccess || cus < 1)
+        return fail(ALO_ERR_LAUNCH, "alo_encoder_block: cannot read the device's compute unit count");
+    const int gx = a.tiles < 2 * cus ? a.tiles : 2 * cus;
+    void* args[] = {const_cast<EncBlockArgs*>(&a)};
+    return launch<encoder_block_kernel<TAIL, PROJ>>(gx, 256, lds, stream, "alo_encoder_block", args);
+}
+
+}
+}
+
+using namespace alo;
+
+extern "C" int alo_encoder_block_abi_version(void) { return ALO_ENCODER_BLOCK_ABI_VERSION; }
+
+extern "C" int alo_encoder_block(const void* attn_out, const void* wo_packed, const void* bo, const void* norm1_w, const void* norm1_b,
+                                 const void* src, const void* w1_packed, const void* b1, const void* w2_packed, const void* b2,
+                                 const void* norm2_w, const void* norm2_b, void* src_out, const void* pos, const void* padding_mask,
+                                 const void* wv_packed, const void* bv, const void* wq_packed, const void* bq, void* value_hm,
+                                 void* offsets_logits, int batch, int S, int F, float eps1, float eps2, int dtype, void* stream) {
+    const char* what = "alo_encoder_block";
+    ALO_REQUIRE(src && w1_packed && b1 && w2_packed && b2 && norm2_w && norm2_b && src_out, ALO_ERR_INVALID_ARGUMENT,
+                "%s: null pointer argument", what);
+    const bool tail = attn_out || wo_packed || bo || norm1_w || norm1_b;
+    ALO_REQUIRE(!tail || (attn_out && wo_packed && bo && norm1_w && norm1_b), ALO_ERR_INVALID_ARGUMENT,
+                "%s: null pointer argument (attn_out, wo_packed, bo, norm1_w and norm1_b go together)", what);
+    const bool proj = pos || wv_packed || bv || wq_packed || bq || value_hm || offsets_logits;
+    ALO_REQUIRE(!proj || (pos && wv_packed && bv && wq_packed && bq && value_hm && offsets_logits), ALO_ERR_INVALID_ARGUMENT,
+                "%s: null pointer argument (pos, wv_packed, bv, wq_packed, bq, value_hm and offsets_logits go together)", what);
+    ALO_REQUIRE(proj || !padding_mask, ALO_ERR_INVALID_ARGUMENT, "%s: padding_mask without the projections it applies to", what);
+    ALO_REQUIRE(batch > 0 && S > 0 && F > 0 && F % 256 == 0, ALO_ERR_INVALID_ARGUMENT,
+                "%s: batch, S must be positive and the hidden width a positive multiple of 256 (batch=%d S=%d F=%d)", what, batch, S, F);
+    ALO_REQUIRE(dtype == ALO_BF16, ALO_ERR_UNSUPPORTED, "%s: bf16 only (dtype %d)", what, dtype);
+    ALO_REQUIRE(aligned16(attn_out, wo_packed, src, w1_packed, w2_packed, src_out, pos, wv_packed, wq_packed, value_hm, offsets_logits),
+                ALO_ERR_INVALID_ARGUMENT, "%s: pointers must be 16-byte aligned", what);
+    const size_t rows = (size_t)batch * S;
+    const struct { const void* p; size_t bytes; bool out; } spans[] = {
+        {attn_out, rows * 512, false}, {src, rows * 512, false}, {pos, rows * 512, false}, {padding_mask, rows, false},
+        {src_out, rows * 512, true}, {value_hm, rows * 512, true}, {offsets_logits, rows * 768, true}};
+    for (const auto& o : spans)
+        for (const auto& i : spans)
+            ALO_REQUIRE(!o.out || &o == &i || !o.p || !i.p || (const char*)o.p + o.bytes <= (const char*)i.p ||
+                            (const char*)i.p + i.bytes <= (const char*)o.p,
+                        ALO_ERR_INVALID_ARGUMENT, "%s: an output overlaps an input or another output", what);
+    EncBlockArgs a;
+    a.attn = (const bf16_t*)attn_out; a.wo = (const bf16_t*)wo_packed; a.bo = (const bf16_t*)bo;
+    a.g1 = (const bf16_t*)norm1_w; a.be1 = (const bf16_t*)norm1_b;
+    a.src = (const bf16_t*)src; a.w1 = (const bf16_t*)w1_packed; a.b1 = (const bf16_t*)b1; a.w2 = (const bf16_t*)w2_packed;
+    a.b2 = (const bf16_t*)b2; a.g2 = (const bf16_t*)norm2_w; a.be2 = (const bf16_t*)norm2_b;
+    a.out = (bf16_t*)src_out; a.pos = (const bf16_t*)pos; a.mask = (const unsigned char*)padding_mask;
+    a.wv = (const bf16_t*)wv_packed; a.bv = (const bf16_t*)bv; a.wq = (const bf16_t*)wq_packed; a.bq = (const bf16_t*)bq;
+    a.value = (bf16_t*)value_hm; a.both = (bf16_t*)offsets_logits;
+    a.M = (long)batch * S; a.S = S; a.F = F; a.tiles = (int)((a.M + kTileRows - 1) / kTileRows);
+    a.eps1 = eps1; a.eps2 = eps2;
+    const size_t lds = 2 * kTileRows * kTileStride + ((size_t)F + kTables) * sizeof(float);
+    ALO_REQUIRE(lds <= (size_t)kLdsLimit, ALO_ERR_UNSUPPORTED, "%s: hidden width %d needs %zu bytes of LDS", what, F, lds);
+    hipStream_t st = static_cast<hipStream_t>(stream);
+    if (tail) return proj ? launch_block<true, true>(a, lds, st) : launch_block<true, false>(a, lds, st);
+    return proj ? launch_block<false, true>(a, lds, st) : launch_block<false, false>(a, lds, st);
+}
diff --git a/aloception-oss_amd/csrc/fused.hip b/aloception-oss_amd/csrc/fused.hip
--- a/aloception-oss_amd/csrc/fused.hip
+++ b/aloception-oss_amd/csrc/fused.hip
@@ -5,12 +5,6 @@
 
 constexpr int kThreads = 256;
 constexpr int kMaxChunks = 4;
-
-__device__ __forceinline__ float wave_sum(float v) {
-#pragma unroll
-    for (int o = 32; o > 0; o >>= 1) v += __shfl_xor(v, o, 64);
-    return v;
-}
 
 __device__ __forceinline__ void load4(const float* p, float (&v)[4]) {
     const f32x4 x = *reinterpret_cast<const f32x4*>(p);
diff --git a/aloception-oss_amd/csrc/gemm.hip b/aloception-oss_amd/csrc/gemm.hip
--- a/aloception-oss_amd/csrc/gemm.hip
+++ b/aloception-oss_amd/csrc/gemm.hip
@@ -186,8 +186,8 @@
 namespace alo {
 namespace {
 
-constexpr int kFfnRows = 64;
-constexpr int kFfnStride = 256 * 2 + 16;
+constexpr int kFfnRows = kTileRows;
+constexpr int kFfnStride = kTileStride;
 
 struct FfnDims {
     long M;
@@ -210,34 +210,6 @@
     for (int i = tid; i < F; i += 256) b1s[i] = B1 ? bf16_to_f32(B1[i].bits) : 0.f;
     b2s[tid] = B2 ? bf16_to_f32(B2[tid].bits) : 0.f;
 
-    constexpr int KB = 2;
-    constexpr int NBATCH = 16 / KB;
-    auto load_batch = [&](u32x4 (&buf)[2][KB], const bf16_t* frag0, size_t tile_stride, int batch) {
-#pragma unroll
-        for (int t = 0; t < 2; ++t)
-#pragma unroll
-            for (int j = 0; j < KB; ++j)
-                buf[t][j] = *reinterpret_cast<const u32x4*>(frag0 + t * tile_stride + (size_t)(KB * batch + j) * 512);
-        __builtin_amdgcn_sched_barrier(0);
-    };
-    auto mma_batch = [&](f32x16 (&acc)[2][2], const unsigned char* a_lds, const u32x4 (&buf)[2][KB], int batch) {
-        u32x4 af[2][KB];
-#pragma unroll
-        for (int j = 0; j < KB; ++j) {
-            const int s = KB * batch + j;
-            af[0][j] = *reinterpret_cast<const u32x4*>(a_lds + nl * kFfnStride + (16 * s + 8 * kg) * 2);
-            af[1][j] = *reinterpret_cast<const u32x4*>(a_lds + (32 + nl) * kFfnStride + (16 * s + 8 * kg) * 2);
-        }
-#pragma unroll
-        for (int j = 0; j < KB; ++j) {
-            const u32x4 a0 = af[0][j], a1 = af[1][j];
-            acc[0][0] = __builtin_amdgcn_mfma_f32_32x32x16_bf16(as_bf16x8(buf[0][j]), as_bf16x8(a0), acc[0][0], 0, 0, 0);
-            acc[0][1] = __builtin_amdgcn_mfma_f32_32x32x16_bf16(as_bf16x8(buf[1][j]), as_bf16x8(a0), acc[0][1], 0, 0, 0);
-            acc[1][0] = __builtin_amdgcn_mfma_f32_32x32x16_bf16(as_bf16x8(buf[0][j]), as_bf16x8(a1), acc[1][0], 0, 0, 0);
-            acc[1][1] = __builtin_amdgcn_mfma_f32_32x32x16_bf16(as_bf16x8(buf[1][j]), as_bf16x8(a1), acc[1][1], 0, 0, 0);
-        }
-        __builtin_amdgcn_sched_barrier(0);
-    };
     const int fs = F / 16;
     auto w1_frag = [&](int r0) { return W1 + ((size_t)((r0 + 64 * wave) / 32) * 16 * 64 + lane) * 8; };
     auto w2_frag = [&](int r0) { return W2 + (((size_t)(2 * wave) * fs + r0 / 16) * 64 + lane) * 8; };
@@ -245,20 +217,10 @@
     for (int tile = blockIdx.x; tile < dm.tiles; tile += gridDim.x) {
         {
             u32x4 xv[8];
-#pragma unroll
-            for (int j = 0; j < 8; ++j) {
-                const int p = tid + 256 * j;
-                long row = (long)tile * kFfnRows + (p >> 5);
-                row = row < dm.M ? row : dm.M - 1;
-                xv[j] = *reinterpret_cast<const u32x4*>(X + row * 256 + (p & 31) * 8);
-            }
-#pragma unroll
-            for (int j = 0; j < 8; ++j) {
-                const int p = tid + 256 * j;
-                *reinterpret_cast<u32x4*>(xs + (p >> 5) * kFfnStride + (p & 31) * 16) = xv[j];
-            }
-        }
-        u32x4 bufa[2][KB], bufb[2][KB];
+            fetch_tile256(xv, X, (long)tile * kFfnRows, dm.M, tid);
+            park_tile256(xs, xv, tid);
+        }
+        u32x4 bufa[2][kTileKB], bufb[2][kTileKB];
         load_batch(bufa, w1_frag(0), (size_t)16 * 512, 0);
         __syncthreads();
 
@@ -280,52 +242,15 @@
                     for (int i = 0; i < 16; ++i) acc1[a][t][i] = 0.f;
             const bf16_t* w1p = w1_frag(r0);
             const bf16_t* w2p = w2_frag(r0);
-#pragma unroll
-            for (int bt = 0; bt < NBATCH; bt += 2) {
-                load_batch(bufb, w1p, (size_t)16 * 512, bt + 1);
-                mma_batch(acc1, xs, bufa, bt);
-                if (bt + 2 < NBATCH) load_batch(bufa, w1p, (size_t)16 * 512, bt + 2);
-                else load_batch(bufa, w2p, (size_t)fs * 512, 0);
-                mma_batch(acc1, xs, bufb, bt + 1);
-            }
-#pragma unroll
-            for (int t = 0; t < 2; ++t)
-#pragma unroll
-                for (int q = 0; q < 4; ++q) {
-                    const int col = 64 * wave + 32 * t + 8 * q + 4 * kg;
-                    const f32x4 bb = *reinterpret_cast<const f32x4*>(b1s + r0 + col);
-#pragma unroll
-                    for (int a = 0; a < 2; ++a) {
-                        const float v0 = relu_keep_nan(acc1[a][t][4 * q] + bb[0]), v1 = relu_keep_nan(acc1[a][t][4 * q + 1] + bb[1]);
-                        const float v2 = relu_keep_nan(acc1[a][t][4 * q + 2] + bb[2]), v3 = relu_keep_nan(acc1[a][t][4 * q + 3] + bb[3]);
-                        *reinterpret_cast<u32x2*>(hs + (32 * a + nl) * kFfnStride + col * 2) = u32x2{pack_bf16x2(v0, v1), pack_bf16x2(v2, v3)};
-                    }
-                }
+            mma_tile256(acc1, xs, bufa, bufb, w1p, (size_t)16 * 512, w2p, (size_t)fs * 512, nl, kg);
+            stage_tile256<true, true>(hs, acc1, b1s + r0, wave, nl, kg);
             __syncthreads();
 
-#pragma unroll
-            for (int bt = 0; bt < NBATCH; bt += 2) {
-                load_batch(bufb, w2p, (size_t)fs * 512, bt + 1);
-                mma_batch(acc2, hs, bufa, bt);
-                if (bt + 2 < NBATCH) load_batch(bufa, w2p, (size_t)fs * 512, bt + 2);
-                else if (r0 + 256 < F) load_batch(bufa, w1_frag(r0 + 256), (size_t)16 * 512, 0);
-                mma_batch(acc2, hs, bufb, bt + 1);
-            }
+            mma_tile256(acc2, hs, bufa, bufb, w2p, (size_t)fs * 512, r0 + 256 < F ? w1_frag(r0 + 256) : nullptr, (size_t)16 * 512, nl, kg);
             __syncthreads();
         }
 
-#pragma unroll
-        for (int t = 0; t < 2; ++t)
-#pragma unroll
-            for (int q = 0; q < 4; ++q) {
-                const int col = 64 * wave + 32 * t + 8 * q + 4 * kg;
-                const f32x4 bb = *reinterpret_cast<const f32x4*>(b2s + col);
-#pragma unroll
-                for (int a = 0; a < 2; ++a)
-                    *reinterpret_cast<u32x2*>(hs + (32 * a + nl) * kFfnStride + col * 2) =
-                        u32x2{pack_bf16x2(acc2[a][t][4 * q] + bb[0], acc2[a][t][4 * q + 1] + bb[1]),
-                              pack_bf16x2(acc2[a][t][4 * q + 2] + bb[2], acc2[a][t][4 * q + 3] + bb[3])};
-            }
+        stage_tile256<true, false>(hs, acc2, b2s, wave, nl, kg);
         __syncthreads();
 #pragma unroll
         for (int j = 0; j < 8; ++j) {
diff --git a/include/alo_encoder_block.h b/include/alo_encoder_block.h
--- /dev/null
+++ b/include/alo_encoder_block.h
@@ -0,0 +1,22 @@
+#ifndef ALO_ENCODER_BLOCK_H
+#define ALO_ENCODER_BLOCK_H
+
+#include "alo_hotpath.h"
+
+#ifdef __cplusplus
+extern "C" {
+#endif
+
+#define ALO_ENCODER_BLOCK_ABI_VERSION 1
+int alo_encoder_block_abi_version(void);
+
+int alo_encoder_block(const void* attn_out, const void* wo_packed, const void* bo, const void* norm1_w, const void* norm1_b,
+                      const void* src, const void* w1_packed, const void* b1, const void* w2_packed, const void* b2,
+                      const void* norm2_w, const void* norm2_b, void* src_out, const void* pos, const void* padding_mask,
+                      const void* wv_packed, const void* bv, const void* wq_packed, const void* bq, void* value_hm,
+                      void* offsets_logits, int batch, int S, int F, float eps1, float eps2, int dtype, void* stream);
+
+#ifdef __cplusplus
+}
+#endif
+#endif
```
